# haoheliu/AudioLDM2

Hardware: AMD Instinct MI355X
Metric: audio_seconds_per_second (higher is better)
Workload: dtype f32 storage/accumulate; each product = 6 bf16 MFMA partial products of exact 3-part operand splits (fp32-grade); 1 GPU; audioldm2-full: batch 8 prompts/GPU x 1 GPU, 10.24 s @16 kHz, 200 DDIM steps, CFG 3.5, eta 1.0, n_candidates 1; one step = sample_log + VAE decode + HiFi-GAN + D2H of the waveform; synthetic conditioning, random-init weights, host-CPU RNG noise; global_batch=8, parallelism=prompt-sharded replicas x1, weight_broadcast_bytes=0

## Files before the change

audioldm2_amd/csrc/api.hip:

```cpp
#include "common.h"
#include <string.h>

namespace aldm {
static thread_local char g_err[512] = "";
void set_error(const char* fmt, ...) {
    va_list ap;
    va_start(ap, fmt);
    vsnprintf(g_err, sizeof(g_err), fmt, ap);
    va_end(ap);
}
}

extern "C" int aldm_version(void) { return 16; }
extern "C" const char* aldm_last_error(void) { return aldm::g_err; }
```

audioldm2_amd/csrc/igemm.hip:

```cpp
#include "igemm_kernel.h"
#include <algorithm>
#include <atomic>
#include <stdlib.h>

namespace aldm {

int igemm_launch_pre0(int BM, int BN, int kgroups, bool uni, bool w8, dim3 grid, hipStream_t st, const IgemmK& p);
int igemm_launch_pre1(int BM, int BN, int kgroups, bool uni, bool w8, dim3 grid, hipStream_t st, const IgemmK& p);
int igemm_launch_pre2(int BM, int BN, int kgroups, bool uni, bool w8, dim3 grid, hipStream_t st, const IgemmK& p);
int igemm_launch_pre3(int BM, int BN, int kgroups, bool uni, bool w8, dim3 grid, hipStream_t st, const IgemmK& p);
int igemm_launch_pre4(int BM, int BN, int kgroups, bool uni, bool w8, dim3 grid, hipStream_t st, const IgemmK& p);
int igemm_launch_bx_pre0(int BM, int BN, int kgroups, bool uni, bool w8, dim3 grid, hipStream_t st, const IgemmK& p);
int igemm_launch_bx_pre1(int BM, int BN, int kgroups, bool uni, bool w8, dim3 grid, hipStream_t st, const IgemmK& p);
int igemm_launch_bx_pre2(int BM, int BN, int kgroups, bool uni, bool w8, dim3 grid, hipStream_t st, const IgemmK& p);
int igemm_launch_bx_pre3(int BM, int BN, int kgroups, bool uni, bool w8, dim3 grid, hipStream_t st, const IgemmK& p);

int igemm_launch_dma(int BM, int BN, int nst, int parts, bool f16, dim3 grid, hipStream_t st, const IgemmK& p);
bool igemm_dma_config_ok(int BM, int BN, int nst, int parts);
#ifdef ALDM_TEST_HOOKS
extern std::atomic<int> g_debug_drop_product;
#endif
int igemm_launch_dma_ws(int BM, int BN, int nst, int parts, int blocks, hipStream_t st, const IgemmK& p);
bool igemm_dma_ws_config_ok(int BM, int BN, int nst, int parts);
int igemm_dma_ws_blocks_per_cu(int BM, int BN, int nst, int parts);
int igemm_launch_dma_lw(int BM, int BN, int nst, int parts, bool f16, dim3 grid, hipStream_t st, const IgemmK& p);
bool igemm_dma_lw_config_ok(int BM, int BN, int nst, int parts);
int igemm_launch_dma_os(int KT, int nst, int parts, bool f16, dim3 grid, hipStream_t st, const IgemmK& p);
bool igemm_dma_os_config_ok(int KT, int nst, int parts);
int igemm_dma_os_default_stages(int KT, int parts);
int igemm_launch_dma_halo(int BM, int BN, int nstb, int wm, int parts, bool f16, int maxch, dim3 grid, hipStream_t st, const IgemmK& p);
int igemm_dma_halo_maxch(int BM, int BN, int nstb, int wm, int parts, int nch);

__global__ __launch_bounds__(256) void igemm_reduce_kernel(const IgemmK p) {
    const aldm_igemm_desc& d = p.d;
    const int z = blockIdx.z;
    const int N4 = d.N >> 2;
    const int64_t total = (int64_t)p.M * N4;
    const int64_t i = (int64_t)blockIdx.x * 256 + threadIdx.x;
    if (i >= total) return;
    const int m = (int)(i / N4);
    const int n = (int)(i - (int64_t)m * N4) << 2;
    const int64_t slab = (int64_t)p.M * d.N;
    const float* w = d.ws + (int64_t)z * p.splits * slab + (int64_t)m * d.N + n;
    f32x4 v = *reinterpret_cast<const f32x4*>(w);
    int s = 1;
    for (; s + 3 < p.splits; s += 4) {
        const f32x4 a0 = *reinterpret_cast<const f32x4*>(w + (int64_t)s * slab);
        const f32x4 a1 = *reinterpret_cast<const f32x4*>(w + (int64_t)(s + 1) * slab);
        const f32x4 a2 = *reinterpret_cast<const f32x4*>(w + (int64_t)(s + 2) * slab);
        const f32x4 a3 = *reinterpret_cast<const f32x4*>(w + (int64_t)(s + 3) * slab);
        v += a0;
        v += a1;
        v += a2;
        v += a3;
    }
    for (; s < p.splits; ++s) v += *reinterpret_cast<const f32x4*>(w + (int64_t)s * slab);
    const int b = m / p.OHW;
    int64_t orow = m;
    if (d.out_mul > 0) {
        const int qq = m - b * p.OHW;
        const int t = qq * d.out_mul + d.out_off;
        if ((unsigned)t >= (unsigned)d.out_len) return;
        orow = (int64_t)b * d.out_len + t;
    }
    float* outp = d.out ? d.out + (int64_t)z * d.stride_o : nullptr;
    const float* resp = d.res ? d.res + (int64_t)z * d.stride_o : nullptr;
    const int64_t o = orow * d.ldo + n;
    f32x4 r;
#pragma unroll
    for (int j = 0; j < 4; ++j) r[j] = epi_value(d, p.rb_ld, outp, resp, b, o + j, n + j, v[j]);
    if (outp) {
#pragma unroll
        for (int j = 0; j < 4; ++j) outp[o + j] = r[j];
    }
    if (d.out_split) {
        if (d.out_split_act == ALDM_ACT_LRELU) {
#pragma unroll
            for (int j = 0; j < 4; ++j) r[j] = r[j] > 0.0f ? r[j] : r[j] * d.out_split_slope;
        }
        split_store4_out(d, d.out_split, orow, d.out_split_c, n, r);
    }
}

__global__ void pack_weight_kernel(const float* __restrict__ src, float* __restrict__ dst, int N,
                                   int Cin, int KH, int KW, int Kg, int Npad) {
    const int64_t total = (int64_t)Kg * Npad * 4;
    for (int64_t i = blockIdx.x * (int64_t)blockDim.x + threadIdx.x; i < total;
         i += (int64_t)gridDim.x * blockDim.x) {
        const int j = i & 3;
        const int n = (i >> 2) % Npad;
        const int kg = (i >> 2) / Npad;
        const int k = kg * 4 + j;
        float v = 0.f;
        if (n < N && k < KH * KW * Cin) {
            const int tap = k / Cin, ci = k - tap * Cin;
            const int kh = tap / KW, kw = tap - kh * KW;
            v = src[(((int64_t)n * Cin + ci) * KH + kh) * KW + kw];
        }
        dst[i] = v;
    }
}

__global__ void pack_weight_tr_kernel(const float* __restrict__ src, float* __restrict__ dst, int N,
                                      int Cin, int KWfull, int T, int phase, int stride, int Kg,
                                      int Npad) {
    const int64_t total = (int64_t)Kg * Npad * 4;
    for (int64_t i = blockIdx.x * (int64_t)blockDim.x + threadIdx.x; i < total;
         i += (int64_t)gridDim.x * blockDim.x) {
        const int jj = i & 3;
        const int n = (i >> 2) % Npad;
        const int kg = (i >> 2) / Npad;
        const int k = kg * 4 + jj;
        float v = 0.f;
        if (n < N && k < T * Cin) {
            const int kwp = k / Cin, ci = k - kwp * Cin;
            const int j = T - 1 - kwp;
            const int kk = phase + j * stride;
            if (kk < KWfull) v = src[((int64_t)ci * N + n) * KWfull + kk];
        }
        dst[i] = v;
    }
}

__global__ void pack_kn_kernel(const float* __restrict__ src, float* __restrict__ dst, int K, int N,
                               int lds, int Kg, int Npad, int64_t stride_src, int64_t stride_dst) {
    const int64_t total = (int64_t)Kg * Npad * 4;
    src += blockIdx.y * stride_src;
    dst += blockIdx.y * stride_dst;
    for (int64_t i = blockIdx.x * (int64_t)blockDim.x + threadIdx.x; i < total;
         i += (int64_t)gridDim.x * blockDim.x) {
        const int j = i & 3;
        const int n = (i >> 2) % Npad;
        const int kg = (i >> 2) / Npad;
        const int k = kg * 4 + j;
        dst[i] = (n < N && k < K) ? src[(int64_t)k * lds + n] : 0.f;
    }
}

template <int NP>
__global__ void pack_split_kernel(const float* __restrict__ src, uint4* __restrict__ dst, int Kg, int Npad,
                                  int Ko) {
    const int64_t total = (int64_t)Ko * Npad;
    for (int64_t i = blockIdx.x * (int64_t)blockDim.x + threadIdx.x; i < total;
         i += (int64_t)gridDim.x * blockDim.x) {
        const int n = (int)(i % Npad);
        const int ko = (int)(i / Npad);
        u32x2 part[2][3];
#pragma unroll
        for (int h = 0; h < 2; ++h) {
            const int kg = 2 * ko + h;
            f32x4 f = {0.f, 0.f, 0.f, 0.f};
            if (kg < Kg) f = *reinterpret_cast<const f32x4*>(src + ((int64_t)kg * Npad + n) * 4);
            split4_parts(f, part[h], NP);
        }
#pragma unroll
        for (int q = 0; q < NP; ++q) {
            uint4 o;
            o.x = part[0][q][0];
            o.y = part[0][q][1];
            o.z = part[1][q][0];
            o.w = part[1][q][1];
            dst[((int64_t)ko * NP + q) * Npad + n] = o;
        }
    }
}

__global__ void pack_split_f16_kernel(const float* __restrict__ src, uint4* __restrict__ dst, int Kg, int Npad, int Ko, float scale) {
    const int64_t total = (int64_t)Ko * Npad;
    for (int64_t i = blockIdx.x * (int64_t)blockDim.x + threadIdx.x; i < total; i += (int64_t)gridDim.x * blockDim.x) {
        const int n = (int)(i % Npad);
        const int ko = (int)(i / Npad);
        u32x2 part[2][3];
#pragma unroll
        for (int h = 0; h < 2; ++h) {
            const int kg = 2 * ko + h;
            f32x4 f = {0.f, 0.f, 0.f, 0.f};
            if (kg < Kg) f = *reinterpret_cast<const f32x4*>(src + ((int64_t)kg * Npad + n) * 4);
            split4_f16(f, scale, part[h]);
        }
#pragma unroll
        for (int q = 0; q < 2; ++q) {
            uint4 o;
            o.x = part[0][q][0];
            o.y = part[0][q][1];
            o.z = part[1][q][0];
            o.w = part[1][q][1];
            dst[((int64_t)ko * 2 + q) * Npad + n] = o;
        }
    }
}

static int log2_exact(int v) {
    int s = 0;
    while ((1 << s) < v) ++s;
    return (1 << s) == v ? s : -1;
}

}

using namespace aldm;

static thread_local int g_force_bm = 0, g_force_bn = 0, g_force_splits = 0, g_force_kgroups = 0, g_force_stages = 0;

extern "C" void aldm_igemm_force(int bm, int bn, int splits, int kgroups) {
    g_force_bm = bm;
    g_force_bn = bn;
    g_force_splits = splits;
    g_force_kgroups = kgroups;
    g_force_stages = 0;
}
extern "C" void aldm_igemm_force_stages(int stages) { g_force_stages = stages; }

static int default_wave8_mask() {
    static const int m = [] {
        const char* e = getenv("ALDM_IGEMM_W8");
        return e ? atoi(e) : 1;
    }();
    return m;
}
static thread_local int g_wave8_mask = -1;

extern "C" int aldm_igemm_wave8_mask(int mask) {
    g_wave8_mask = mask;
    return mask < 0 ? default_wave8_mask() : mask;
}

static thread_local int g_force_mma = 0;
extern "C" int aldm_igemm_mma(int mode) {
    const int prev = g_force_mma;
    if (mode >= 0 && mode <= 2) g_force_mma = mode;
    return prev;
}

static int pre_mode_of(const aldm_igemm_desc& d) {
    if (d.pre_scale == nullptr && d.pre_act == ALDM_ACT_NONE) return PRE_NONE;
    if (d.pre_scale != nullptr && d.pre_act == ALDM_ACT_NONE) return PRE_AFFINE;
    if (d.pre_scale != nullptr && d.pre_act == ALDM_ACT_SILU) return PRE_AFFINE_SILU;
    if (d.pre_scale == nullptr && d.pre_act == ALDM_ACT_LRELU) return PRE_LRELU;
    return PRE_GENERIC;
}

static int device_cus() {
    static const int n = [] {
        int dev = 0, cus = 0;
        if (hipGetDevice(&dev) != hipSuccess ||
            hipDeviceGetAttribute(&cus, hipDeviceAttributeMultiprocessorCount, dev) != hipSuccess || cus <= 0)
            return 256;
        return cus;
    }();
    return n;
}

static bool dma_ws_eligible(const IgemmK& p, int BM, int BN) {
    const aldm_igemm_desc& d = p.d;
    const bool geglu = d.epi_mode == ALDM_EPI_GEGLU;
    auto al16 = [](const void* q) { return (reinterpret_cast<uintptr_t>(q) & 15) == 0; };
    if (d.out_mul > 0 || d.accumulate || d.batch != 1 || d.act != ALDM_ACT_NONE || d.out_split_act != ALDM_ACT_NONE ||
        d.epi_mode == ALDM_EPI_QKV)
        return false;
    if (p.M % BM != 0 || d.N % BN != 0 || (d.N & 3) != 0 || (d.ldo & 3) != 0) return false;
    if (!al16(d.out) || !al16(d.res) || !al16(d.bias) || !al16(d.rowbias) || !al16(d.out_split)) return false;
    if (d.rowbias && (p.OHW % BM != 0 || (p.rb_ld & 3) != 0)) return false;
    if (geglu && (BN != 128 || d.res || d.rowbias)) return false;
    return true;
}

static bool dma_os_eligible(const IgemmK& p) {
    const aldm_igemm_desc& d = p.d;
    if (d.KH != 1 || d.KW != 1 || d.SH != 1 || d.SW != 1 || d.PH != 0 || d.PW != 0 || d.up_h != 1 || d.up_w != 1) return false;
    if (d.OH != d.H || d.OW != d.W || d.K != p.Cin || d.K % 32 != 0 || d.out_mul > 0 || d.batch > 1) return false;
    if (d.epi_mode == ALDM_EPI_QKV && d.qkv_c % 128 != 0) return false;
    if (d.rowbias || d.accumulate || d.act != ALDM_ACT_NONE) return false;
    auto al16 = [](const void* q) { return (reinterpret_cast<uintptr_t>(q) & 15) == 0; };
    if ((d.N & 3) != 0 || (d.ldo & 3) != 0 || !al16(d.out) || !al16(d.res)) return false;
    return true;
}

static int dma_halo_chunks(const IgemmK& p, int BM) {
    const aldm_igemm_desc& d = p.d;
    if (d.KH != 3 || d.KW != 3 || d.SH != 1 || d.SW != 1 || d.PH != 1 || d.PW != 1 || d.DH != 1 || d.DW != 1) return 0;
    if (d.up_h != 1 || d.up_w != 1 || d.OH != d.H || d.OW != d.W || d.out_mul > 0 || d.batch > 1) return 0;
    if (d.W <= 0 || (d.W & (d.W - 1)) != 0 || BM % d.W != 0 || p.OHW % BM != 0) return 0;
    return ((BM / d.W + 2) * d.W + 15) / 16;
}

static bool tile_supported(int BM, int BN) {
    return (BM == 128 && (BN == 128 || BN == 64 || BN == 32)) || (BM == 64 && (BN == 128 || BN == 64));
}

static int igemm_prepare(const aldm_igemm_desc* dd, IgemmK& p, int& BM, int& BN) {
    ALDM_CHECK(dd != nullptr, "aldm_igemm: null descriptor");
    p.d = *dd;
    aldm_igemm_desc& d = p.d;
    ALDM_CHECK((d.x1 || d.a_split) && d.w && (d.out || d.out_split), "aldm_igemm: null x1/w/out");
    if (!d.x1) d.x1 = reinterpret_cast<const float*>(d.a_split);
    if (d.split_parts == 0) d.split_parts = 3;
    ALDM_CHECK(d.split_parts == 2 || d.split_parts == 3, "aldm_igemm: split_parts must be 0 / 3 or 2");
    if (d.out_split_parts == 0) d.out_split_parts = d.split_parts;
    ALDM_CHECK(d.out_split_parts == 2 || d.out_split_parts == 3, "aldm_igemm: out_split_parts must be 0, 2 or 3");
    ALDM_CHECK(d.a_fmt == ALDM_FMT_BF16 || (d.a_fmt == ALDM_FMT_F16 && d.a_split != nullptr && d.split_parts == 2 && d.acc_scale > 0.0f),
               "aldm_igemm: a_fmt = ALDM_FMT_F16 needs a pre-split operand (a_split), 2-part images and acc_scale > 0");
    if (d.a_fmt == ALDM_FMT_BF16) d.acc_scale = 1.0f;
    ALDM_CHECK(d.out_split_fmt == ALDM_FMT_BF16 ||
                   (d.out_split_fmt == ALDM_FMT_F16 && d.out_split_scale > 0.0f &&
                    (d.epi_mode == ALDM_EPI_QKV ? (d.k_split != nullptr && d.vt_split != nullptr && d.vt_scale > 0.0f) : d.out_split != nullptr)),
               "aldm_igemm: out_split_fmt = ALDM_FMT_F16 needs out_split (QKV: k_split, vt_split and vt_scale) and out_split_scale > 0");
    if (d.out_split_fmt == ALDM_FMT_F16) d.out_split_parts = 2;
    if (!d.x2) d.C2 = 0;
    if (d.pix1 == 0) d.pix1 = d.C1;
    if (d.pix2 == 0) d.pix2 = d.C2;
    if (d.up_h == 0) d.up_h = 1;
    if (d.up_w == 0) d.up_w = 1;
    if (d.batch == 0) d.batch = 1;
    p.Cin = d.C1 + d.C2;
    ALDM_CHECK(d.C1 > 0 && d.C1 % 4 == 0 && d.C2 % 4 == 0,
               "aldm_igemm: C1=%d/C2=%d must be multiples of 4", d.C1, d.C2);
    ALDM_CHECK(d.pix1 % 4 == 0 && d.pix2 % 4 == 0, "aldm_igemm: pixel pitch must be a multiple of 4");
    ALDM_CHECK(d.K == d.KH * d.KW * p.Cin, "aldm_igemm: K=%d != KH*KW*Cin=%d", d.K,
               d.KH * d.KW * p.Cin);
    ALDM_CHECK(d.N > 0 && (d.ldo >= d.N || d.epi_mode == ALDM_EPI_GEGLU || d.epi_mode == ALDM_EPI_QKV),
               "aldm_igemm: bad N=%d ldo=%d", d.N, d.ldo);
    ALDM_CHECK(d.B > 0 && d.H > 0 && d.W > 0 && d.OH > 0 && d.OW > 0, "aldm_igemm: bad extents");
    ALDM_CHECK(d.SH > 0 && d.SW > 0 && d.DH > 0 && d.DW > 0, "aldm_igemm: bad stride/dilation");
    p.shh = log2_exact(d.up_h);
    p.shw = log2_exact(d.up_w);
    ALDM_CHECK(p.shh >= 0 && p.shw >= 0, "aldm_igemm: upsample factors must be powers of two");
    ALDM_CHECK((reinterpret_cast<uintptr_t>(d.x1) & 15) == 0 &&
                   (reinterpret_cast<uintptr_t>(d.w) & 15) == 0 &&
                   (d.x2 == nullptr || (reinterpret_cast<uintptr_t>(d.x2) & 15) == 0),
               "aldm_igemm: operands must be 16-byte aligned");
    if (d.b_mode == ALDM_B_NT) {
        ALDM_CHECK(d.ldb % 4 == 0 && d.ldb >= d.K, "aldm_igemm: NT ldb=%d invalid", d.ldb);
        p.Npad = d.N;
    } else {
        p.Npad = (d.N + 31) / 32 * 32;
        ALDM_CHECK(d.ldb == 0 || d.ldb == p.Npad, "aldm_igemm: packed ldb must equal Npad");
    }
    if (d.out_mul > 0) ALDM_CHECK(d.OH == 1, "aldm_igemm: row remap requires OH == 1");
    ALDM_CHECK((d.pre_scale == nullptr) == (d.pre_shift == nullptr),
               "aldm_igemm: pre_scale/pre_shift must come together");
    ALDM_CHECK(d.pre_scale == nullptr ||
                   ((reinterpret_cast<uintptr_t>(d.pre_scale) | reinterpret_cast<uintptr_t>(d.pre_shift)) & 15) == 0,
               "aldm_igemm: pre_scale/pre_shift must be 16-byte aligned");
    const bool geglu = d.epi_mode == ALDM_EPI_GEGLU;
    const bool qkv = d.epi_mode == ALDM_EPI_QKV;
    ALDM_CHECK(d.epi_mode == ALDM_EPI_PLAIN || geglu || qkv, "aldm_igemm: unknown epi_mode %d", d.epi_mode);
    if (qkv) {
        auto al16 = [](const void* q) { return (reinterpret_cast<uintptr_t>(q) & 15) == 0; };
        ALDM_CHECK(d.a_split && d.qkv_c > 0 && d.qkv_c % 64 == 0 && d.N == 3 * d.qkv_c && d.qkv_rows > 0 && d.qkv_rows % 32 == 0 &&
                       (((int64_t)d.B * d.OH * d.OW) % d.qkv_rows == 0 ||
                        d.qkv_rows == (((int64_t)d.B * d.OH * d.OW + 31) & ~(int64_t)31)) && d.out && d.k_split && d.vt_split && al16(d.out) &&
                       al16(d.k_split) && al16(d.vt_split) && d.ldo >= d.qkv_c && (d.ldo & 3) == 0 && !d.bias && !d.rowbias &&
                       !d.res && !d.out_split && !d.accumulate && d.out_mul == 0 && d.act == ALDM_ACT_NONE && d.alpha == 1.0f &&
                       d.batch <= 1,
                   "aldm_igemm: ALDM_EPI_QKV needs a pre-split operand, N = 3*qkv_c (qkv_c %% 64 == 0), qkv_rows %% 32 == 0 dividing M "
                   "(or M rounded up to 32), "
                   "aligned out / k_split / vt_split and a plain epilogue");
    }
    if (geglu) {
        ALDM_CHECK(d.N % 64 == 0 && d.ldo >= d.N / 2 && d.ldo % 4 == 0 && d.b_mode == ALDM_B_PACKED &&
                       d.out_mul == 0 && !d.res && !d.rowbias && !d.accumulate &&
                       (d.act == ALDM_ACT_NONE || d.act == ALDM_ACT_GELU_TANH) &&
                       (reinterpret_cast<uintptr_t>(d.out) & 15) == 0 && d.stride_o % 4 == 0 &&
                       (d.bias == nullptr || (reinterpret_cast<uintptr_t>(d.bias) & 15) == 0),
                   "aldm_igemm: GEGLU epilogue needs N %% 64 == 0, ldo >= N/2, packed weights, a plain epilogue");
    }
    p.OHW = d.OH * d.OW;
    const int64_t M64 = (int64_t)d.B * p.OHW;
    ALDM_CHECK(M64 < (1ll << 31) - 256, "aldm_igemm: M too large");
    p.M = (int)M64;
    p.HV = d.H * d.up_h;
    p.WV = d.W * d.up_w;
    ALDM_CHECK((int64_t)d.B * d.H * d.W < (1ll << 31), "aldm_igemm: input has too many pixels");
    p.Kg = (d.K + 3) / 4;
    p.rb_ld = d.rowbias_ld > 0 ? d.rowbias_ld : d.N;

    const int nk = (d.K + BK - 1) / BK;
    const int64_t Mz = p.M;
    const int pre = pre_mode_of(d);
    p.dma = 0;
    p.nst = 0;
    p.ws = 0;
    p.ws_blocks = 0;
    p.os_rows = 0;
    ALDM_CHECK(d.out_split_act == ALDM_ACT_NONE || (d.out_split_act == ALDM_ACT_LRELU && d.out_split != nullptr &&
                                                   d.epi_mode == ALDM_EPI_PLAIN),
               "aldm_igemm: out_split_act must be ALDM_ACT_NONE or ALDM_ACT_LRELU with a split-image output of the plain epilogue");
    if (d.out_split) {
        ALDM_CHECK(d.out_split_c > 0 && d.out_split_c % 32 == 0 && d.out_split_c >= (geglu ? d.N / 2 : d.N) &&
                       d.N % 4 == 0 && d.batch == 1 && (reinterpret_cast<uintptr_t>(d.out_split) & 15) == 0 &&
                       ((reinterpret_cast<uintptr_t>(d.out) | reinterpret_cast<uintptr_t>(d.res)) & 15) == 0 &&
                       (d.out == nullptr || (d.ldo & 3) == 0),
                   "aldm_igemm: out_split needs out_split_c %% 32 == 0 and >= N, N %% 4 == 0, batch 1, aligned out/res");
        ALDM_CHECK(d.out != nullptr || !d.accumulate, "aldm_igemm: accumulate needs an fp32 output");
    }
    if (d.a_split) {
        ALDM_CHECK(d.w_split != nullptr && d.b_mode == ALDM_B_PACKED && d.stride_w == 0 && d.batch == 1,
                   "aldm_igemm: a_split needs packed, split weights and batch 1");
        ALDM_CHECK(d.C2 == 0 && d.C1 % 32 == 0 && pre == PRE_NONE,
                   "aldm_igemm: a_split needs one source with C1 %% 32 == 0 and no prologue (C1=%d C2=%d)", d.C1, d.C2);
        ALDM_CHECK(((reinterpret_cast<uintptr_t>(d.a_split) | reinterpret_cast<uintptr_t>(d.w_split)) & 15) == 0,
                   "aldm_igemm: split images must be 16-byte aligned");
        ALDM_CHECK((int64_t)d.B * d.H * d.W * p.Cin * 2 * d.split_parts < (1ll << 40), "aldm_igemm: split image too large");
        const bool can_split = d.N % 4 == 0 && nk >= 8 && !geglu && !qkv;
        const bool have_ws = d.ws != nullptr && (reinterpret_cast<uintptr_t>(d.ws) & 15) == 0;
        auto dma_cost = [&](int bm, int bn, int nst, int sp, int* sp_eff) -> double {
            const int kt = cdiv(nk, sp);
            sp = cdiv(nk, kt);
            *sp_eff = sp;
            const double blocks = (double)cdiv64(Mz, bm) * cdiv(d.N, bn) * sp;
            const int lds = nst * (bm + bn) * 64 * d.split_parts;
            const int o = std::min(2, (160 * 1024) / lds);
            const double tile_c = (bm / 64) * (bn / 64) * 64.0 * (d.split_parts == 3 ? 6 : 3);
            const double dma_c = (bm + bn) * 64.0 * d.split_parts / 56.0;
            const double L = kt * std::max(tile_c, dma_c);
            const double one = kt * std::max(tile_c + 200.0, dma_c) + 6000.0;
            const int64_t nb = (int64_t)((blocks + 255.0) / 256.0);
            const int64_t full = nb / o, last = nb - full * o;
            double T = full * std::max(one, o * L);
            if (last) T += std::max(one, last * L);
            if (sp > 1) T += 10000.0 + (double)(sp + 1) * Mz * d.N * 4.0 / 2000.0;
            return T;
        };
        int splits = 1, nst = 0;
        const bool hint_fits = d.hint_bm > 0 && (!qkv || (d.hint_bn > 0 && d.qkv_c % d.hint_bn == 0)) && (!geglu || d.hint_bn == 128);
        const int f_bm = g_force_bm ? g_force_bm : (hint_fits ? d.hint_bm : 0), f_bn = g_force_bm ? g_force_bn : d.hint_bn;
        const int f_sp = g_force_bm ? g_force_splits : d.hint_splits;
        int f_st = g_force_bm ? g_force_stages : (hint_fits ? d.hint_stages : 0);
        int ws_nst = 0;
        int lw_nst = 0;
        if (f_st >= 300 && f_st < 400) {
            const int KT = d.K / 32;
            int os_nst = f_st - 300;
            if (os_nst == 0) os_nst = igemm_dma_os_default_stages(KT, d.split_parts);
            if (dma_os_eligible(p) && igemm_dma_os_config_ok(KT, os_nst, d.split_parts)) {
                static const int env_rows = [] {
                    const char* e = getenv("ALDM_OS_ROWS");
                    return e ? atoi(e) : 0;
                }();
                const int tn = cdiv(d.N, 128);
                const int stages = cdiv(p.M, 32);
                const int chunks = std::max(1, device_cus() / tn);
                int rows = cdiv(stages, chunks) * 32;
                if (env_rows > 0) rows = cdiv(env_rows, 32) * 32;
                BM = 32;
                BN = 128;
// ... 97 lines not shown
        p.tiles_n = cdiv(d.N, BN);
        p.kt_per_split = cdiv(nk, splits);
        splits = cdiv(nk, p.kt_per_split);
        if (splits > 1 && (!have_ws || d.ws_floats < (int64_t)splits * p.M * d.N)) {
            splits = 1;
            p.kt_per_split = nk;
        }
        p.splits = splits;
        p.kgroups = 1;
        p.bx = 1;
        p.pre = pre;
        p.dma = 1;
        p.nst = nst;
        p.ws = 0;
        p.ws_blocks = 0;
        if (lw_nst > 0) {
            ALDM_CHECK(igemm_dma_lw_config_ok(BM, BN, lw_nst, d.split_parts), "aldm_igemm: no loader-wave DMA kernel for tile %dx%d, %d stages", BM, BN, lw_nst);
            p.ws = 2;
            p.nst = lw_nst;
        }
        if (ws_nst > 0) {
            if (splits == 1 && d.a_fmt == ALDM_FMT_BF16 && d.out_split_parts == d.split_parts && d.out_split_fmt == ALDM_FMT_BF16 &&
                igemm_dma_ws_config_ok(BM, BN, ws_nst, d.split_parts) && dma_ws_eligible(p, BM, BN)) {
                const int ntiles = p.tiles_m * p.tiles_n;
                const int per = cdiv(ntiles, device_cus() * igemm_dma_ws_blocks_per_cu(BM, BN, ws_nst, d.split_parts));
                p.ws = 1;
                p.nst = ws_nst;
                p.ws_blocks = cdiv(ntiles, per);
            } else {
                ALDM_CHECK(!g_force_bm, "aldm_igemm: the persistent DMA kernel cannot run this launch (tile %dx%d, %d stages)", BM,
                           BN, ws_nst);
            }
        }
        return 0;
    }
    const bool bx_ok = d.w_split != nullptr && d.split_parts == 3 && d.b_mode == ALDM_B_PACKED && d.stride_w == 0 && d.batch == 1 &&
                       pre != PRE_GENERIC && (reinterpret_cast<uintptr_t>(d.w_split) & 15) == 0 &&
                       (g_force_mma == 2 || (g_force_mma == 0 && d.hint_mma != 1));
    auto occ_of = [&](int bm, int bn) {
        if (bx_ok && bn != 32) return bm * bn >= 128 * 128 ? 1 : (bm * bn >= 64 * 128 ? 2 : 3);
        return bm * bn >= 128 * 128 ? 2 : ((bm * bn >= 64 * 128 || bn == 32) ? 3 : 4);
    };
    const double pre_w = (d.pre_scale != nullptr || d.pre_act != ALDM_ACT_NONE) ? 1.5 : 1.0;
    auto cost_of = [&](int bm, int bn, int sp, int kg, int* sp_eff) -> double {
        const bool bx = bx_ok && bn != 32;
        const double mf = bx ? 0.375 : 1.0;
        const int kt = cdiv(nk, sp);
        sp = cdiv(nk, kt);
        *sp_eff = sp;
        const double blocks = (double)cdiv64(Mz, bm) * cdiv(d.N, bn) * d.batch * sp;
        const double L = (double)kt * bm * bn / 4.0 * mf;
        const int o = kg == 2 ? (bx ? 1 : 2) : occ_of(bm, bn);
        const double S = (300.0 * (bm / 32) * pre_w + 200.0 * (bn / 32)) *
                         (bx ? (bm * bn >= 128 * 128 && !geglu ? 0.45 : 1.3) : 1.0);
        const double F = 4000.0 + (kg == 2 ? 600.0 : 0.0);
        const int64_t nb = (int64_t)((blocks + 255.0) / 256.0);
        const int64_t full = nb / o, last = nb - full * o;
        const double one = (double)cdiv(kt, kg) * ((double)bm * bn / 4.0 * mf + S) + F;
        double T = full * std::max(one, o * L);
        if (last) T += std::max(one, last * L);
        if (sp > 1) T += 10000.0 + (double)(sp + 1) * Mz * d.N * d.batch * 4.0 / 2000.0;
        return T;
    };
    const bool can_split = d.N % 4 == 0 && nk >= 8 && !geglu;
    const bool have_ws = d.ws != nullptr && (reinterpret_cast<uintptr_t>(d.ws) & 15) == 0;
    int splits = 1, kgroups = 1;
    const int f_bm = g_force_bm ? g_force_bm : d.hint_bm, f_bn = g_force_bm ? g_force_bn : d.hint_bn;
    const int f_sp = g_force_bm ? g_force_splits : d.hint_splits;
    const int f_kg = g_force_bm ? g_force_kgroups : d.hint_kgroups;
    if (f_bm) {
        BM = f_bm;
        BN = f_bn;
        ALDM_CHECK(tile_supported(BM, BN), "aldm_igemm: unsupported forced/hinted tile %dx%d", BM, BN);
        ALDM_CHECK(!geglu || BN == 128, "aldm_igemm: the GEGLU epilogue needs a 128-column tile");
        if (f_sp > 0 && can_split && nk / f_sp >= 1) splits = f_sp;
        if (f_kg == 2) {
            ALDM_CHECK(BM == 64 && BN == 64, "aldm_igemm: two wave groups exist for the 64x64 tile only");
            kgroups = 2;
        }
    } else if (d.N <= 32 && !geglu) {
        BM = 128;
        BN = 32;
    } else {
        static const int cand[4][2] = {{128, 128}, {64, 128}, {128, 64}, {64, 64}};
        static const int sps[8] = {1, 2, 3, 4, 6, 8, 12, 16};
        double best = 1e300;
        BM = 64;
        BN = 64;
        for (int c = 0; c < 4; ++c) {
            const int bm = cand[c][0], bn = cand[c][1];
            if (geglu ? bn != 128 : (bn > 64 && d.N <= 64)) continue;
            for (int si = 0; si < 8; ++si) {
                const int sp = sps[si];
                if (sp > 1 && (!can_split || !have_ws || nk / sp < 3)) break;
                for (int kg = 1; kg <= ((bm == 64 && bn == 64) ? 2 : 1); ++kg) {
                    int spe;
                    const double t = cost_of(bm, bn, sp, kg, &spe);
                    if (spe > 1 && (int64_t)d.batch * spe * Mz * d.N > d.ws_floats) continue;
                    if (kg == 2 && cdiv(nk, spe) < 4) continue;
                    if (t < best) {
                        best = t;
                        BM = bm;
                        BN = bn;
                        splits = spe;
                        kgroups = kg;
                    }
                }
            }
        }
    }
    ALDM_CHECK(!geglu || BN == 128, "aldm_igemm: internal: GEGLU epilogue without a 128-column tile");
    p.tiles_m = cdiv(p.M, BM);
    p.tiles_n = cdiv(d.N, BN);
    if (splits < 1) splits = 1;
    p.kt_per_split = cdiv(nk, splits);
    splits = cdiv(nk, p.kt_per_split);
    if (splits > 1) {
        const int64_t need = (int64_t)d.batch * splits * p.M * d.N;
        if (!have_ws || d.ws_floats < need) {
            splits = 1;
            p.kt_per_split = nk;
        }
    }
    p.splits = splits;
    p.kgroups = kgroups;
    p.bx = bx_ok && BN != 32 ? 1 : 0;
    p.pre = pre;
    return 0;
}

extern "C" int aldm_igemm_plan(const aldm_igemm_desc* dd, int* bm, int* bn, int64_t* flops, int* splits,
                               int* kgroups, int* mma) {
    IgemmK p;
    int BM, BN;
    const int rc = igemm_prepare(dd, p, BM, BN);
    if (rc) return rc;
    if (bm) *bm = BM;
    if (bn) *bn = BN;
    if (flops) *flops = 2ll * p.M * p.d.N * p.d.K * p.d.batch;
    if (splits) *splits = p.splits;
    if (kgroups) *kgroups = p.kgroups;
    if (mma) *mma = p.bx ? ALDM_MMA_BF16X6 : ALDM_MMA_F32;
    return 0;
}

extern "C" int aldm_igemm_plan_stages(const aldm_igemm_desc* dd) {
    IgemmK p;
    int BM, BN;
    if (igemm_prepare(dd, p, BM, BN)) return -1;
    if (p.dma && p.ws == 4) return 400 + (BM == 128 && p.ws_blocks == 4 ? 10 : 0) + p.nst;
    return p.dma ? p.nst + 100 * p.ws : 0;
}

extern "C" int64_t aldm_igemm_ws_floats(const aldm_igemm_desc* dd) {
    if (!dd) return 0;
    aldm_igemm_desc t = *dd;
    t.ws = reinterpret_cast<float*>(uintptr_t(16));
    t.ws_floats = INT64_MAX;
    IgemmK p;
    int BM, BN;
    if (igemm_prepare(&t, p, BM, BN)) return 0;
    return p.splits > 1 ? (int64_t)p.d.batch * p.splits * p.M * p.d.N : 0;
}

extern "C" int aldm_igemm(const aldm_igemm_desc* dd, void* stream) {
    IgemmK p;
    int BM, BN;
    int rc = igemm_prepare(dd, p, BM, BN);
    if (rc) return rc;
    const aldm_igemm_desc& d = p.d;
    dim3 grid((unsigned)(p.tiles_m * p.tiles_n), (unsigned)p.splits, (unsigned)d.batch);
    hipStream_t st = (hipStream_t)stream;
    const int pre = p.pre;
    const bool uni = p.OHW % BM == 0;
    const int env_w8 = g_wave8_mask < 0 ? default_wave8_mask() : g_wave8_mask;
    const bool gn_pre = pre == PRE_AFFINE || pre == PRE_AFFINE_SILU;
    const int tile_bit = (BM == 128 && BN == 128) ? 1 : (BM == 64 && BN == 128) ? 2 : (BM == 128 && BN == 64) ? 4 : 0;
    const bool w8 = p.kgroups == 1 && d.epi_mode != ALDM_EPI_GEGLU && (env_w8 & tile_bit) != 0 &&
                    (p.bx ? tile_bit == 1 : (gn_pre || (tile_bit == 1 && (env_w8 & 8) != 0)));
#ifdef ALDM_TEST_HOOKS
    if (g_debug_drop_product.load(std::memory_order_relaxed))
        ALDM_CHECK(p.dma && p.ws == 0 && BM == 64 && BN == 128 && p.nst == 2 && d.split_parts == 3,
                   "aldm_igemm: aldm_debug_drop_product is set: force the classic DMA-fed 64x128 tile with 2 stages and 3-part images "
                   "(got dma=%d form=%d tile %dx%d, %d stages, %d parts) or clear the switch", p.dma, p.ws, BM, BN, p.nst, d.split_parts);
#endif
    if (p.dma && p.ws == 4) {
        rc = igemm_launch_dma_halo(BM, BN, p.nst, p.ws_blocks, d.split_parts, d.a_fmt == ALDM_FMT_F16, p.os_rows, grid, st, p);
    } else if (p.dma && p.ws == 3) {
        rc = igemm_launch_dma_os(d.K / 32, p.nst, d.split_parts, d.a_fmt == ALDM_FMT_F16, grid, st, p);
    } else if (p.dma && p.ws == 2) {
        rc = igemm_launch_dma_lw(BM, BN, p.nst, d.split_parts, d.a_fmt == ALDM_FMT_F16, grid, st, p);
    } else if (p.dma && p.ws) {
        rc = igemm_launch_dma_ws(BM, BN, p.nst, d.split_parts, p.ws_blocks, st, p);
    } else if (p.dma) {
        rc = igemm_launch_dma(BM, BN, p.nst, d.split_parts, d.a_fmt == ALDM_FMT_F16, grid, st, p);
    } else if (p.bx) {
        switch (pre) {
            case PRE_NONE: rc = igemm_launch_bx_pre0(BM, BN, p.kgroups, uni, w8, grid, st, p); break;
            case PRE_AFFINE: rc = igemm_launch_bx_pre1(BM, BN, p.kgroups, uni, w8, grid, st, p); break;
            case PRE_AFFINE_SILU: rc = igemm_launch_bx_pre2(BM, BN, p.kgroups, uni, w8, grid, st, p); break;
            default: rc = igemm_launch_bx_pre3(BM, BN, p.kgroups, uni, w8, grid, st, p); break;
        }
    } else
    switch (pre) {
        case PRE_NONE: rc = igemm_launch_pre0(BM, BN, p.kgroups, uni, w8, grid, st, p); break;
        case PRE_AFFINE: rc = igemm_launch_pre1(BM, BN, p.kgroups, uni, w8, grid, st, p); break;
        case PRE_AFFINE_SILU: rc = igemm_launch_pre2(BM, BN, p.kgroups, uni, w8, grid, st, p); break;
        case PRE_LRELU: rc = igemm_launch_pre3(BM, BN, p.kgroups, uni, w8, grid, st, p); break;
        default: rc = igemm_launch_pre4(BM, BN, p.kgroups, uni, w8, grid, st, p); break;
    }
    if (rc) {
        set_error("aldm_igemm: no kernel for tile %dx%d", BM, BN);
        return -1;
    }
    if (p.splits > 1) {
        const int64_t total = (int64_t)p.M * (d.N >> 2);
        hipLaunchKernelGGL(igemm_reduce_kernel, dim3((unsigned)cdiv64(total, 256), 1, (unsigned)d.batch),
                           dim3(256), 0, st, p);
    }
    ALDM_LAUNCH_CHECK("aldm_igemm");
    return 0;
}

extern "C" int64_t aldm_split_bytes_parts(int K, int N, int parts) {
    if (K <= 0 || N <= 0 || (parts != 2 && parts != 3)) return 0;
    const int Npad = (N + 31) / 32 * 32;
    const int64_t Ko = 4ll * ((K + 31) / 32);
    return Ko * parts * Npad * 16;
}
extern "C" int64_t aldm_split_bytes(int K, int N) { return aldm_split_bytes_parts(K, N, 3); }

extern "C" int aldm_pack_split_f16(const float* packed, void* dst, int K, int N, float scale, void* stream) {
    ALDM_CHECK(packed && dst && K > 0 && N > 0 && scale > 0.0f, "aldm_pack_split_f16: bad args");
    ALDM_CHECK(((reinterpret_cast<uintptr_t>(packed) | reinterpret_cast<uintptr_t>(dst)) & 15) == 0,
               "aldm_pack_split_f16: operands must be 16-byte aligned");
    const int Npad = (N + 31) / 32 * 32;
    const int Kg = (K + 3) / 4;
    const int Ko = 4 * ((K + 31) / 32);
    const int64_t total = (int64_t)Ko * Npad;
    hipLaunchKernelGGL(pack_split_f16_kernel, dim3((unsigned)std::min<int64_t>(cdiv64(total, 256), 4096)), dim3(256), 0,
                       (hipStream_t)stream, packed, reinterpret_cast<uint4*>(dst), Kg, Npad, Ko, scale);
    ALDM_LAUNCH_CHECK("aldm_pack_split_f16");
    return 0;
}

extern "C" int aldm_pack_split_bf16_parts(const float* packed, void* dst, int K, int N, int parts, void* stream) {
    ALDM_CHECK(packed && dst && K > 0 && N > 0 && (parts == 2 || parts == 3), "aldm_pack_split_bf16: bad args");
    ALDM_CHECK(((reinterpret_cast<uintptr_t>(packed) | reinterpret_cast<uintptr_t>(dst)) & 15) == 0,
               "aldm_pack_split_bf16: operands must be 16-byte aligned");
    const int Npad = (N + 31) / 32 * 32;
    const int Kg = (K + 3) / 4;
    const int Ko = 4 * ((K + 31) / 32);
    const int64_t total = (int64_t)Ko * Npad;
    const int blocks = (int)std::min<int64_t>((total + 255) / 256, 65535);
    if (parts == 3)
        hipLaunchKernelGGL(pack_split_kernel<3>, dim3(blocks), dim3(256), 0, (hipStream_t)stream, packed,
                           reinterpret_cast<uint4*>(dst), Kg, Npad, Ko);
    else
        hipLaunchKernelGGL(pack_split_kernel<2>, dim3(blocks), dim3(256), 0, (hipStream_t)stream, packed,
                           reinterpret_cast<uint4*>(dst), Kg, Npad, Ko);
    ALDM_LAUNCH_CHECK("aldm_pack_split_bf16");
    return 0;
}
extern "C" int aldm_pack_split_bf16(const float* packed, void* dst, int K, int N, void* stream) {
    return aldm_pack_split_bf16_parts(packed, dst, K, N, 3, stream);
}

extern "C" int aldm_pack_weight(const float* src, float* dst, int N, int Cin, int KH, int KW,
                                int transposed, int phase, int stride, void* stream) {
    ALDM_CHECK(src && dst && N > 0 && Cin > 0 && KH > 0 && KW > 0, "aldm_pack_weight: bad args");
    const int Npad = (N + 31) / 32 * 32;
    hipStream_t st = (hipStream_t)stream;
    if (!transposed) {
        const int K = KH * KW * Cin;
        const int Kg = (K + 3) / 4;
        const int64_t total = (int64_t)Kg * Npad * 4;
        const int blocks = (int)std::min<int64_t>(cdiv64(total, 256), 4096);
        hipLaunchKernelGGL(pack_weight_kernel, dim3(blocks), dim3(256), 0, st, src, dst, N, Cin, KH,
                           KW, Kg, Npad);
    } else {
        ALDM_CHECK(KH == 1 && stride > 0 && phase >= 0 && phase < stride,
                   "aldm_pack_weight: bad transposed args");
        const int T = (KW + stride - 1) / stride;
        const int K = T * Cin;
        const int Kg = (K + 3) / 4;
        const int64_t total = (int64_t)Kg * Npad * 4;
        const int blocks = (int)std::min<int64_t>(cdiv64(total, 256), 4096);
        hipLaunchKernelGGL(pack_weight_tr_kernel, dim3(blocks), dim3(256), 0, st, src, dst, N, Cin,
                           KW, T, phase, stride, Kg, Npad);
    }
    ALDM_LAUNCH_CHECK("aldm_pack_weight");
    return 0;
}

extern "C" int aldm_pack_kn(const float* src, float* dst, int K, int N, int lds, int batch,
                            int64_t stride_src, int64_t stride_dst, void* stream) {
    ALDM_CHECK(src && dst && K > 0 && N > 0 && lds >= N && batch > 0, "aldm_pack_kn: bad args");
    const int Npad = (N + 31) / 32 * 32;
    const int Kg = (K + 3) / 4;
    const int64_t total = (int64_t)Kg * Npad * 4;
    const int blocks = (int)std::min<int64_t>(cdiv64(total, 256), 4096);
    hipLaunchKernelGGL(pack_kn_kernel, dim3(blocks, batch), dim3(256), 0, (hipStream_t)stream, src,
                       dst, K, N, lds, Kg, Npad, stride_src, stride_dst);
    ALDM_LAUNCH_CHECK("aldm_pack_kn");
    return 0;
}
```

audioldm2_amd/csrc/igemm_dma.h:

```cpp
#pragma once
#include "igemm_epilogue.h"
#include <type_traits>

namespace aldm {

static __device__ __attribute__((aligned(256))) unsigned g_dma_zero_page[256 + 64];

constexpr int dma_stage_slots(int BM, int BN, int NP) { return (BM + BN) * 4 * NP; }
constexpr int dma_lds_bytes(int BM, int BN, int NST, int NP) { return NST * dma_stage_slots(BM, BN, NP) * 16; }
constexpr int dma_blocks_per_cu(int BM, int BN, int NST, int NP) {
    return (160 * 1024) / dma_lds_bytes(BM, BN, NST, NP) >= 2 ? 2 : 1;
}

template <bool F16>
__device__ __forceinline__ f32x16 mfma_32x32x16(const bf16x8 a, const bf16x8 b, const f32x16 c) {
    if constexpr (F16)
        return __builtin_amdgcn_mfma_f32_32x32x16_f16(__builtin_bit_cast(f16x8, a), __builtin_bit_cast(f16x8, b), c, 0, 0, 0);
    else
        return __builtin_amdgcn_mfma_f32_32x32x16_bf16(a, b, c, 0, 0, 0);
}
template <bool F16, int MT, int NT>
__device__ __forceinline__ void unscale_acc(f32x16 (&acc)[MT][NT], float acc_scale) {
    if constexpr (F16) {
#pragma unroll
        for (int i = 0; i < MT; ++i)
#pragma unroll
            for (int j = 0; j < NT; ++j)
#pragma unroll
                for (int e = 0; e < 16; ++e) acc[i][j][e] *= acc_scale;
    }
}

template <int N>
__device__ __forceinline__ void wait_vmcnt() {
    __builtin_amdgcn_s_waitcnt((N & 15) | (7 << 4) | (0 << 8) | ((N >> 4) << 14));
}

#ifndef ALDM_DMA_TAP_INNER
#define ALDM_DMA_TAP_INNER 0
#endif
#ifndef ALDM_DMA_ABLATE
#define ALDM_DMA_ABLATE 0
#endif

template <int BM, int BN, int NST, int WM = 2, int NP = 3, bool DROP = false, bool F16 = false>
__global__ __launch_bounds__(128 * WM, dma_blocks_per_cu(BM, BN, NST, NP) * (WM / 2))
void igemm_dma_kernel(const IgemmK p) {
    constexpr int WN = 2, NW = WM * WN;
    constexpr int MT = BM / (32 * WM), NT = BN / 64;
    constexpr int STG = dma_stage_slots(BM, BN, NP);
    constexpr int PB = 64 * NP;
    constexpr int RA = BM / (16 * NW);
    constexpr int NB = 4 * NP * (BN / 64) / NW;
    constexpr int D = NP * RA + NB;
    constexpr int NPROD = NP == 3 ? 6 : 3;
    static_assert(NP == 2 || NP == 3, "2 or 3 parts");
    static_assert(!F16 || NP == 2, "fp16 images have two parts");
    static_assert(BM % (16 * NW) == 0 && (4 * NP * (BN / 64)) % NW == 0, "DMA chunks must divide among the waves");
    static_assert(NST >= 2 && NST <= 8 && (NST - 1) * D <= 63, "ring depth / vmcnt range");
    static_assert(NW * 32 * (NT * 32 + 4) * 4 <= NST * STG * 16, "epilogue staging must fit the ring");
    __shared__ u32x4 smem[NST * STG];

    const aldm_igemm_desc& d = p.d;
    const int lane = threadIdx.x & 63;
    const int wave = __builtin_amdgcn_readfirstlane(threadIdx.x >> 6);
    const int wm = wave / WN, wn = wave % WN;
    const int l31 = lane & 31, lh = lane >> 5;

    int tile_m, tile_n;
    {
        const int nwg = gridDim.x;
        const int bid = blockIdx.x;
        const int q = nwg >> 3, r = nwg & 7;
        const int xcd = bid & 7, idx = bid >> 3;
        const int logical = (xcd < r ? xcd * (q + 1) : r * (q + 1) + (xcd - r) * q) + idx;
        tile_n = logical % p.tiles_n;
        tile_m = logical / p.tiles_n;
    }
    const int m0 = tile_m * BM, n0 = tile_n * BN;
    const int split = blockIdx.y;
    const int nk_all = d.K >> 5;
    const int kt0 = split * p.kt_per_split;
    const int kt1 = min(nk_all, kt0 + p.kt_per_split);
#if ALDM_DMA_ABLATE & 32
    const int nk = min(kt1 - kt0, 1);
#else
    const int nk = kt1 - kt0;
#endif

    const char* zero = reinterpret_cast<const char*>(g_dma_zero_page);
    const char* abase = reinterpret_cast<const char*>(d.a_split);
    const char* wbase = reinterpret_cast<const char*>(d.w_split);
    const int cpb = p.Cin >> 5;
    const int taps = d.KH * d.KW;
    const int64_t rowbytes = (int64_t)cpb * PB;

    const int lane_off = ((lane & 3) ^ ((lane >> 4) & 3)) * 16;
    int a_pix[RA], a_h[RA], a_w[RA];
#pragma unroll
    for (int i = 0; i < RA; ++i) {
        const int m = m0 + (wave * RA + i) * 16 + (lane >> 2);
        if (m < p.M) {
            const int b = m / p.OHW;
            const int rem = m - b * p.OHW;
            const int oh = rem / d.OW;
            const int ow = rem - oh * d.OW;
            a_pix[i] = b * d.H;
            a_h[i] = oh * d.SH - d.PH;
            a_w[i] = ow * d.SW - d.PW;
        } else {
            a_pix[i] = 0;
            a_h[i] = -(1 << 28);
            a_w[i] = 0;
        }
    }
    const char* a_ptr[RA];
    int a_step[RA];
    int t_kh, t_kw, t_cb;
    auto set_tap = [&]() {
        const int dh = t_kh * d.DH, dw = t_kw * d.DW;
        const int cboff = t_cb * PB + lane_off;
#pragma unroll
        for (int i = 0; i < RA; ++i) {
            const int ihv = a_h[i] + dh, iwv = a_w[i] + dw;
            const bool ok = (unsigned)ihv < (unsigned)p.HV && (unsigned)iwv < (unsigned)p.WV;
            const int pix = (a_pix[i] + (ihv >> p.shh)) * d.W + (iwv >> p.shw);
            a_ptr[i] = ok ? abase + ((int64_t)pix * rowbytes + cboff) : zero + lane_off;
            a_step[i] = ok ? PB : 0;
        }
    };
    {
        if (ALDM_DMA_TAP_INNER) {
            t_cb = kt0 / taps;
            const int tap = kt0 - t_cb * taps;
            t_kh = tap / d.KW;
            t_kw = tap - t_kh * d.KW;
        } else {
            const int tap = kt0 / cpb;
            t_cb = kt0 - tap * cpb;
            t_kh = tap / d.KW;
            t_kw = tap - t_kh * d.KW;
        }
        set_tap();
    }
    const char* b_ptr[NB];
    int64_t b_tile[NB];
#pragma unroll
    for (int j = 0; j < NB; ++j) {
        const int c = wave * NB + j;
        const int srow = c / (BN / 64), half = c % (BN / 64);
        const int col = n0 + half * 64 + lane;
        const bool ok = col < p.Npad;
        b_tile[j] = ok ? (int64_t)4 * NP * p.Npad * 16 : 0;
        const int tile0 = (t_kh * d.KW + t_kw) * cpb + t_cb;
        b_ptr[j] = ok ? wbase + (((int64_t)tile0 * 4 * NP + srow) * p.Npad + col) * 16 : zero;
    }

    using gptr_t = const __attribute__((address_space(1))) void*;
    using lptr_t = __attribute__((address_space(3))) void*;
    auto issue_dma = [&](int st) {
        u32x4* sa = &smem[st * STG];
#pragma unroll
        for (int i = 0; i < RA; ++i)
#pragma unroll
            for (int q = 0; q < NP; ++q) {
                const char* src = (ALDM_DMA_ABLATE & 1) ? zero + lane * 16 : a_ptr[i] + q * 64;
                __builtin_amdgcn_global_load_lds((gptr_t)src, (lptr_t)(sa + ((wave * RA + i) * NP + q) * 64), 16, 0, 0);
            }
#pragma unroll
        for (int j = 0; j < NB; ++j) {
            const int c = wave * NB + j;
            const int srow = c / (BN / 64), half = c % (BN / 64);
            const char* src = (ALDM_DMA_ABLATE & 2) ? zero + lane * 16 : b_ptr[j];
            __builtin_amdgcn_global_load_lds((gptr_t)src, (lptr_t)(sa + BM * 4 * NP + srow * BN + half * 64), 16, 0, 0);
        }
    };
    auto advance = [&]() {
        if (taps == 1 || !ALDM_DMA_TAP_INNER) {
#pragma unroll
            for (int i = 0; i < RA; ++i) a_ptr[i] += a_step[i];
#pragma unroll
            for (int j = 0; j < NB; ++j) b_ptr[j] += b_tile[j];
            if (++t_cb == cpb && taps > 1) {
                t_cb = 0;
                if (++t_kw == d.KW) {
                    t_kw = 0;
                    ++t_kh;
                }
                set_tap();
            }
            return;
        }
        if (++t_kw == d.KW) {
            t_kw = 0;
            ++t_kh;
        }
        if (t_kh == d.KH) {
            t_kh = 0;
            ++t_cb;
#pragma unroll
            for (int j = 0; j < NB; ++j) b_ptr[j] += b_tile[j] * (1 - (int64_t)(taps - 1) * cpb);
        } else {
#pragma unroll
            for (int j = 0; j < NB; ++j) b_ptr[j] += b_tile[j] * cpb;
        }
        set_tap();
    };
    auto issue = [&](int st) {
        issue_dma(st);
        advance();
    };

    struct Frag {
        bf16x8 a[MT][NP], b[NT][NP];
    };
    const int a_sw = (l31 >> 2) & 3;
    auto read_frags = [&](Frag& f, int st, int step) {
#if ALDM_DMA_ABLATE & 8
        return;
#endif
        const u32x4* sa = &smem[st * STG];
        const int o = 2 * step + lh;
#pragma unroll
        for (int i = 0; i < MT; ++i) {
            const int row = (wm * MT + i) * 32 + l31;
#pragma unroll
            for (int q = 0; q < NP; ++q)
                f.a[i][q] = __builtin_bit_cast(bf16x8, sa[((row >> 4) * NP + q) * 64 + (row & 15) * 4 + (o ^ a_sw)]);
        }
#pragma unroll
        for (int j = 0; j < NT; ++j)
#pragma unroll
            for (int q = 0; q < NP; ++q)
                f.b[j][q] = __builtin_bit_cast(bf16x8, sa[BM * 4 * NP + (o * NP + q) * BN + (wn * NT + j) * 32 + l31]);
    };

    f32x16 acc[MT][NT], sum[MT][NT];
    acc_zero(acc);
    acc_zero(sum);
    auto mma_frags = [&](const Frag& f) {
        constexpr int PA_[6] = {NP == 3 ? 0 : 1, NP == 3 ? 2 : 0, NP == 3 ? 1 : 0, 0, 1, 0};
        constexpr int PB_[6] = {NP == 3 ? 2 : 0, NP == 3 ? 0 : 1, NP == 3 ? 1 : 0, 1, 0, 0};
#if ALDM_DMA_ABLATE & 4
#pragma unroll
        for (int i = 0; i < MT; ++i)
#pragma unroll
            for (int q = 0; q < NP; ++q) asm volatile("" ::"v"(f.a[i][q]));
#pragma unroll
        for (int j = 0; j < NT; ++j)
#pragma unroll
            for (int q = 0; q < NP; ++q) asm volatile("" ::"v"(f.b[j][q]));
        return;
#endif
#pragma unroll
        for (int q = DROP ? 1 : 0; q < NPROD; ++q)
#pragma unroll
            for (int i = 0; i < MT; ++i)
#pragma unroll
                for (int j = 0; j < NT; ++j)
                    acc[i][j] = mfma_32x32x16<F16>(f.a[i][PA_[q]], f.b[j][PB_[q]], acc[i][j]);
    };
    auto wait_tiles = [&](int n) {
        constexpr int MX = NST - 1;
        if (n <= 0) wait_vmcnt<0>();
        else if (n == 1) wait_vmcnt<D>();
        else if (n == 2) wait_vmcnt<(MX >= 2 ? 2 : MX) * D>();
        else if (n == 3) wait_vmcnt<(MX >= 3 ? 3 : MX) * D>();
        else if (n == 4) wait_vmcnt<(MX >= 4 ? 4 : MX) * D>();
        else if (n == 5) wait_vmcnt<(MX >= 5 ? 5 : MX) * D>();
        else wait_vmcnt<(MX >= 6 ? 6 : MX) * D>();
    };

#pragma unroll
    for (int s = 0; s < NST; ++s)
        if (s < nk) issue(s);
    wait_tiles(min(nk, NST) - 1);
    __builtin_amdgcn_s_barrier();
    Frag f0, f1;
#if ALDM_DMA_ABLATE & 8
    for (int q = 0; q < NP; ++q) {
        for (int i = 0; i < MT; ++i) f0.a[i][q] = f1.a[i][q] = __builtin_bit_cast(bf16x8, smem[lane + q]);
        for (int j = 0; j < NT; ++j) f0.b[j][q] = f1.b[j][q] = __builtin_bit_cast(bf16x8, smem[lane + 64 + q]);
    }
#endif
    read_frags(f0, 0, 0);
    int st = 0, t = 0;
    auto body = [&](auto steady) {
        constexpr bool ST = decltype(steady)::value;
        constexpr int NMF = NPROD * MT * NT, NRD = NP * (MT + NT);
        read_frags(f1, st, 1);
        mma_frags(f0);
#pragma unroll
        for (int q = 0; q < NMF; ++q) {
            __builtin_amdgcn_sched_group_barrier(0x008, 1, 0);
            if (q < NRD) __builtin_amdgcn_sched_group_barrier(0x100, 1, 0);
        }
        __builtin_amdgcn_sched_barrier(0);
        const int st1 = st + 1 == NST ? 0 : st + 1;
        if constexpr (ST) wait_vmcnt<(NST - 2) * D>();
        else wait_tiles(min(NST - 2, nk - 2 - t));
        __builtin_amdgcn_s_barrier();
        if constexpr (ST) issue_dma(st);
        read_frags(f0, st1, 0);
        mma_frags(f1);
#pragma unroll
        for (int q = 0; q < NMF; ++q) {
            __builtin_amdgcn_sched_group_barrier(0x008, 1, 1);
            if (ST && q == 0) __builtin_amdgcn_sched_group_barrier(0x020, D, 1);
            if (q < NRD) __builtin_amdgcn_sched_group_barrier(0x100, 1, 1);
        }
        __builtin_amdgcn_sched_barrier(0);
        if constexpr (ST) advance();
        st = st1;
    };
    while (t + NST < nk) {
        for (const int te = min(nk - NST, t + ACC_BLOCK_TILES); t < te; ++t) body(std::true_type{});
        if (t + NST < nk) acc_close_block(acc, sum);
    }
    for (; t + 1 < nk; ++t) body(std::false_type{});
    read_frags(f1, st, 1);
    mma_frags(f0);
    mma_frags(f1);
    acc_total(acc, sum);

    __syncthreads();
#if ALDM_DMA_ABLATE & 16
    if (p.M == -12345) {
#pragma unroll
        for (int i = 0; i < MT; ++i)
#pragma unroll
            for (int j = 0; j < NT; ++j)
#pragma unroll
                for (int e = 0; e < 16; ++e) d.ws[(i * NT + j) * 16 + e + threadIdx.x * 256] = acc[i][j][e];
    }
    return;
#endif
    unscale_acc<F16>(acc, d.acc_scale);
    igemm_epilogue<MT, NT>(p, acc, reinterpret_cast<float*>(&smem[0]), m0, n0, wave, wm, wn, lane, 0, split);
}

}
```

audioldm2_amd/csrc/igemm_dma.hip:

```cpp
#include "igemm_dma.h"
#include <atomic>

namespace aldm {

bool igemm_dma_config_ok(int BM, int BN, int nst, int parts) {
    if (BM == 256 && BN == 128) return parts == 3 ? nst == 2 : (nst == 2 || nst == 3);
    if (BM == 128 && BN == 128) return parts == 3 ? (nst == 2 || nst == 3) : (nst == 2 || nst == 4);
    if ((BM == 64 && BN == 128) || (BM == 128 && BN == 64)) return nst == 2 || nst == 4 || (nst == 6 && parts == 2);
    if (BM == 64 && BN == 64) return nst == 2 || nst == 3 || (nst == 6 && parts == 2);
    return false;
}

#ifdef ALDM_TEST_HOOKS
std::atomic<int> g_debug_drop_product{0};
#endif

int igemm_launch_dma(int BM, int BN, int nst, int parts, bool f16, dim3 grid, hipStream_t st, const IgemmK& p) {
#ifdef ALDM_TEST_HOOKS
    if (g_debug_drop_product.load(std::memory_order_relaxed)) {
        if (!(BM == 64 && BN == 128 && nst == 2 && parts == 3)) return -1;
        hipLaunchKernelGGL((igemm_dma_kernel<64, 128, 2, 2, 3, true>), grid, dim3(256), 0, st, p);
        return 0;
    }
#endif
#define ALDM_DMA(BM_, BN_, NST_, NP_) \
    hipLaunchKernelGGL((igemm_dma_kernel<BM_, BN_, NST_, 2, NP_>), grid, dim3(256), 0, st, p)
#define ALDM_DMA8(BM_, BN_, NST_, NP_) \
    hipLaunchKernelGGL((igemm_dma_kernel<BM_, BN_, NST_, 4, NP_>), grid, dim3(512), 0, st, p)
    if (f16) {
        if (parts != 2) return -1;
#define ALDM_DMA_H(BM_, BN_, NST_) \
    hipLaunchKernelGGL((igemm_dma_kernel<BM_, BN_, NST_, 2, 2, false, true>), grid, dim3(256), 0, st, p)
#define ALDM_DMA8_H(BM_, BN_, NST_) \
    hipLaunchKernelGGL((igemm_dma_kernel<BM_, BN_, NST_, 4, 2, false, true>), grid, dim3(512), 0, st, p)
        if (BM == 256 && BN == 128 && nst == 3) ALDM_DMA8_H(256, 128, 3);
        else if (BM == 256 && BN == 128 && nst == 2) ALDM_DMA8_H(256, 128, 2);
        else if (BM == 128 && BN == 128 && nst == 4) ALDM_DMA_H(128, 128, 4);
        else if (BM == 128 && BN == 128 && nst == 2) ALDM_DMA_H(128, 128, 2);
        else if (BM == 64 && BN == 128 && nst == 6) ALDM_DMA_H(64, 128, 6);
        else if (BM == 64 && BN == 128 && nst == 4) ALDM_DMA_H(64, 128, 4);
        else if (BM == 64 && BN == 128 && nst == 2) ALDM_DMA_H(64, 128, 2);
        else if (BM == 128 && BN == 64 && nst == 6) ALDM_DMA_H(128, 64, 6);
        else if (BM == 128 && BN == 64 && nst == 4) ALDM_DMA_H(128, 64, 4);
        else if (BM == 128 && BN == 64 && nst == 2) ALDM_DMA_H(128, 64, 2);
        else if (BM == 64 && BN == 64 && nst == 6) ALDM_DMA_H(64, 64, 6);
        else if (BM == 64 && BN == 64 && nst == 3) ALDM_DMA_H(64, 64, 3);
        else if (BM == 64 && BN == 64 && nst == 2) ALDM_DMA_H(64, 64, 2);
        else return -1;
#undef ALDM_DMA_H
#undef ALDM_DMA8_H
        return 0;
    }
    if (parts == 3) {
        if (BM == 256 && BN == 128 && nst == 2) ALDM_DMA8(256, 128, 2, 3);
        else if (BM == 128 && BN == 128 && nst == 3) ALDM_DMA(128, 128, 3, 3);
        else if (BM == 128 && BN == 128 && nst == 2) ALDM_DMA(128, 128, 2, 3);
        else if (BM == 64 && BN == 128 && nst == 4) ALDM_DMA(64, 128, 4, 3);
        else if (BM == 64 && BN == 128 && nst == 2) ALDM_DMA(64, 128, 2, 3);
        else if (BM == 128 && BN == 64 && nst == 4) ALDM_DMA(128, 64, 4, 3);
        else if (BM == 128 && BN == 64 && nst == 2) ALDM_DMA(128, 64, 2, 3);
        else if (BM == 64 && BN == 64 && nst == 3) ALDM_DMA(64, 64, 3, 3);
        else if (BM == 64 && BN == 64 && nst == 2) ALDM_DMA(64, 64, 2, 3);
        else return -1;
    } else {
        if (BM == 256 && BN == 128 && nst == 3) ALDM_DMA8(256, 128, 3, 2);
        else if (BM == 256 && BN == 128 && nst == 2) ALDM_DMA8(256, 128, 2, 2);
        else if (BM == 128 && BN == 128 && nst == 4) ALDM_DMA(128, 128, 4, 2);
        else if (BM == 128 && BN == 128 && nst == 2) ALDM_DMA(128, 128, 2, 2);
        else if (BM == 64 && BN == 128 && nst == 6) ALDM_DMA(64, 128, 6, 2);
        else if (BM == 64 && BN == 128 && nst == 4) ALDM_DMA(64, 128, 4, 2);
        else if (BM == 64 && BN == 128 && nst == 2) ALDM_DMA(64, 128, 2, 2);
        else if (BM == 128 && BN == 64 && nst == 6) ALDM_DMA(128, 64, 6, 2);
        else if (BM == 128 && BN == 64 && nst == 4) ALDM_DMA(128, 64, 4, 2);
        else if (BM == 128 && BN == 64 && nst == 2) ALDM_DMA(128, 64, 2, 2);
        else if (BM == 64 && BN == 64 && nst == 6) ALDM_DMA(64, 64, 6, 2);
        else if (BM == 64 && BN == 64 && nst == 3) ALDM_DMA(64, 64, 3, 2);
        else if (BM == 64 && BN == 64 && nst == 2) ALDM_DMA(64, 64, 2, 2);
        else return -1;
    }
#undef ALDM_DMA
#undef ALDM_DMA8
    return 0;
}

template <int ACT, bool AFF>
__global__ __launch_bounds__(256) void split_rows_kernel(const float* __restrict__ x1, const float* __restrict__ x2,
                                                         int C1, int C2, int64_t rows, int P,
                                                         const float* __restrict__ scale,
                                                         const float* __restrict__ shift, char* __restrict__ dst,
                                                         char* __restrict__ dst_raw, int parts, float slope, int raw_parts,
                                                         float f16_scale) {
    const int C = C1 + C2;
    const int C8 = C >> 3;
    const int64_t total = rows * C8;
    for (int64_t i = blockIdx.x * (int64_t)blockDim.x + threadIdx.x; i < total; i += (int64_t)gridDim.x * blockDim.x) {
        const int64_t row = i / C8;
        const int c = (int)(i - row * C8) << 3;
        const float* src = c < C1 ? x1 + row * C1 + c : x2 + row * C2 + (c - C1);
        f32x4 v0 = *reinterpret_cast<const f32x4*>(src);
        f32x4 v1 = *reinterpret_cast<const f32x4*>(src + 4);
        const int64_t off = (row * (C >> 5) + (c >> 5)) * (64 * parts) + (c & 31) * 2;
        u32x2 p0[3], p1[3];
        if (dst_raw) {
            const int64_t roff = (row * (C >> 5) + (c >> 5)) * (64 * raw_parts) + (c & 31) * 2;
            split4_parts(v0, p0, raw_parts);
            split4_parts(v1, p1, raw_parts);
#pragma unroll
            for (int q = 0; q < 3; ++q)
                if (q < raw_parts) *reinterpret_cast<u32x4*>(dst_raw + roff + q * 64) = u32x4{p0[q][0], p0[q][1], p1[q][0], p1[q][1]};
        }
        if constexpr (AFF) {
            const int64_t so = (row / P) * C + c;
            const f32x4 s0 = *reinterpret_cast<const f32x4*>(scale + so), s1 = *reinterpret_cast<const f32x4*>(scale + so + 4);
            const f32x4 h0 = *reinterpret_cast<const f32x4*>(shift + so), h1 = *reinterpret_cast<const f32x4*>(shift + so + 4);
#pragma unroll
            for (int e = 0; e < 4; ++e) {
                v0[e] = __builtin_fmaf(v0[e], s0[e], h0[e]);
                v1[e] = __builtin_fmaf(v1[e], s1[e], h1[e]);
            }
        }
        if constexpr (ACT == ALDM_ACT_SILU) {
#pragma unroll
            for (int e = 0; e < 4; ++e) {
                v0[e] = silu_fast(v0[e]);
                v1[e] = silu_fast(v1[e]);
            }
        }
        if constexpr (ACT == ALDM_ACT_LRELU) {
#pragma unroll
            for (int e = 0; e < 4; ++e) {
                v0[e] = v0[e] > 0.0f ? v0[e] : v0[e] * slope;
                v1[e] = v1[e] > 0.0f ? v1[e] : v1[e] * slope;
            }
        }
        split4_fmt(v0, p0, parts, f16_scale);
        split4_fmt(v1, p1, parts, f16_scale);
#pragma unroll
        for (int q = 0; q < 3; ++q)
            if (q < parts) *reinterpret_cast<u32x4*>(dst + off + q * 64) = u32x4{p0[q][0], p0[q][1], p1[q][0], p1[q][1]};
    }
}

}

using namespace aldm;

#ifdef ALDM_TEST_HOOKS
extern "C" int aldm_debug_drop_product(int on) { return aldm::g_debug_drop_product.exchange(on ? 1 : 0); }
#endif

extern "C" int64_t aldm_split_image_bytes(int64_t rows, int C, int parts) { return rows * (int64_t)(C / 32) * 64 * parts; }

extern "C" int aldm_split_rows_act(const float* x1, const float* x2, int C1, int C2, int64_t rows, int P, const float* scale,
                                   const float* shift, int act, float slope, void* dst, void* dst_raw, int parts, void* stream);
extern "C" int aldm_split_rows_f16(const float* x1, const float* x2, int C1, int C2, int64_t rows, int P, const float* scale,
                                   const float* shift, int act, float slope, void* dst, void* dst_raw, int raw_parts, float f16_scale,
                                   void* stream);

extern "C" int aldm_split_rows(const float* x1, const float* x2, int C1, int C2, int64_t rows, int P, const float* scale,
                               const float* shift, int act, void* dst, void* dst_raw, int parts, void* stream) {
    ALDM_CHECK(act == ALDM_ACT_NONE || act == ALDM_ACT_SILU, "aldm_split_rows: activation %d not supported", act);
    return aldm_split_rows_act(x1, x2, C1, C2, rows, P, scale, shift, act, 0.f, dst, dst_raw, parts, stream);
}

static int split_rows_launch(const float* x1, const float* x2, int C1, int C2, int64_t rows, int P, const float* scale,
                             const float* shift, int act, float slope, void* dst, void* dst_raw, int parts, int raw_parts,
                             float f16_scale, void* stream);

extern "C" int aldm_split_rows_act(const float* x1, const float* x2, int C1, int C2, int64_t rows, int P, const float* scale,
                                   const float* shift, int act, float slope, void* dst, void* dst_raw, int parts, void* stream) {
    return split_rows_launch(x1, x2, C1, C2, rows, P, scale, shift, act, slope, dst, dst_raw, parts, parts, 0.f, stream);
}

extern "C" int aldm_split_rows_f16(const float* x1, const float* x2, int C1, int C2, int64_t rows, int P, const float* scale,
                                   const float* shift, int act, float slope, void* dst, void* dst_raw, int raw_parts, float f16_scale,
                                   void* stream) {
    ALDM_CHECK(f16_scale > 0.0f && (raw_parts == 2 || raw_parts == 3), "aldm_split_rows_f16: need f16_scale > 0 and raw_parts 2 | 3");
// ... 38 lines not shown
```

audioldm2_amd/csrc/igemm_dma_halo.h:

```cpp
#pragma once
#include "igemm_dma.h"

#ifndef ALDM_HALO_ABLATE
#define ALDM_HALO_ABLATE 0
#endif

namespace aldm {

constexpr int halo_lds_slots(int BN, int NSTB, int NP, int MAXCH) {
    return 2 * MAXCH * NP * 64 + NSTB * BN * 4 * NP + NP * 64;
}

template <int BM, int BN, int NSTB, int WM, int NP, int MAXCH, bool F16 = false>
__global__ __launch_bounds__(128 * WM, WM / 2)
void igemm_dma_halo_kernel(const IgemmK p) {
    constexpr int WN = 2, NW = WM * WN;
    constexpr int MT = BM / (32 * WM), NT = BN / 64;
    constexpr int PB = 64 * NP;
    constexpr int PATCH = MAXCH * NP * 64;
    constexpr int BSTG = BN * 4 * NP;
    constexpr int B0 = 2 * PATCH;
    constexpr int Z0 = B0 + NSTB * BSTG;
    constexpr int NB = 4 * NP * (BN / 64) / NW;
    constexpr int D = NB + 1;
    constexpr int ATILES = 11 - NSTB;
    constexpr int NPROD = NP == 3 ? 6 : 3;
    static_assert(NP == 2 || NP == 3, "2 or 3 parts");
    static_assert((4 * NP * (BN / 64)) % NW == 0, "weight pieces must divide among the waves");
    static_assert(NSTB >= 2 && NSTB <= 6 && (NSTB - 1) * D <= 63, "ring depth / vmcnt range");
    static_assert(NW * 32 * (NT * 32 + 4) * 4 <= Z0 * 16, "epilogue staging must fit");
    static_assert((Z0 + NP * 64) * 16 <= 160 * 1024, "LDS budget");
    __shared__ __attribute__((aligned(1024))) u32x4 smem[Z0 + NP * 64];

    const aldm_igemm_desc& d = p.d;
    const int lane = threadIdx.x & 63;
    const int wave = __builtin_amdgcn_readfirstlane(threadIdx.x >> 6);
    const int wm = wave / WN, wn = wave % WN;
    const int l31 = lane & 31, lh = lane >> 5;

    int tile_m, tile_n;
    {
        const int nwg = gridDim.x;
        const int bid = blockIdx.x;
        const int q = nwg >> 3, r = nwg & 7;
        const int xcd = bid & 7, idx = bid >> 3;
        const int logical = (xcd < r ? xcd * (q + 1) : r * (q + 1) + (xcd - r) * q) + idx;
        tile_n = logical % p.tiles_n;
        tile_m = logical / p.tiles_n;
    }
    const int m0 = tile_m * BM, n0 = tile_n * BN;
    const int split = blockIdx.y;
    const int cpb = p.Cin >> 5;
    const int cbps = p.kt_per_split / 9;
    const int cb0 = split * cbps;
    const int ncb = min(cpb, cb0 + cbps) - cb0;
    const int nk = ncb * 9;

    const int W = d.W, lgW = __builtin_ctz((unsigned)W);
    const int img = m0 / p.OHW;
    const int r0 = (m0 - img * p.OHW) >> lgW;
    const int PP = ((BM >> lgW) + 2) << lgW;
    const int NCH = (PP + 15) >> 4;

    const char* zero = reinterpret_cast<const char*>(g_dma_zero_page);
    const char* abase = reinterpret_cast<const char*>(d.a_split);
    const char* wbase = reinterpret_cast<const char*>(d.w_split);
    const int64_t rowbytes = (int64_t)cpb * PB;
    const int lane_off = ((lane & 3) ^ ((lane >> 4) & 3)) * 16;

    using gptr_t = const __attribute__((address_space(1))) void*;
    using lptr_t = __attribute__((address_space(3))) void*;

    const int64_t patch_pix0 = (int64_t)(img * d.H + r0 - 1) * W;
    const char* patch_base0 = abase + (patch_pix0 * rowbytes + (int64_t)cb0 * PB);
    const unsigned rowbytes32 = (unsigned)rowbytes;
    struct Piece {
        const char* src;
        int dst;
    };
    auto prep_patch_piece = [&](int id, int ci, bool live) -> Piece {
        const int j = id / NP, q = id - j * NP;
        const bool valid = live & (j < NCH);
        const int px = j * 16 + (lane >> 2);
        const int irow = r0 - 1 + (px >> lgW);
        const bool ok = valid & (px < PP) & ((unsigned)irow < (unsigned)d.H);
        const unsigned off = (unsigned)px * rowbytes32 + (unsigned)(q * 64 + lane_off);
        const char* real = patch_base0 + (int64_t)((ALDM_HALO_ABLATE & 128) ? 0 : ci) * PB + off;
        const char* zsrc = zero + lane_off;
        Piece pc;
        pc.src = ok ? real : zsrc;
        const int dreal = (ci & 1) * PATCH + (j * NP + q) * 64;
        pc.dst = valid ? dreal : Z0;
        return pc;
    };
    auto issue_piece = [&](const Piece& pc) {
        __builtin_amdgcn_global_load_lds((gptr_t)pc.src, (lptr_t)&smem[pc.dst], 16, 0, 0);
    };
    int av_s = 0, av_c = 1;
    auto prep_a = [&]() {
        return prep_patch_piece(av_s * NW + wave, av_c, (ALDM_HALO_ABLATE & 1) ? false : (av_s < ATILES) & (av_c < ncb));
    };
    auto advance_a = [&]() {
        const bool wrap = av_s == 8;
        av_s = wrap ? 0 : av_s + 1;
        av_c += wrap ? 1 : 0;
    };

    unsigned b_off[NB];
#pragma unroll
    for (int j = 0; j < NB; ++j) {
        const int c = wave * NB + j;
        const int srow = c / (BN / 64), half = c % (BN / 64);
        const int col = min(n0 + half * 64 + lane, p.Npad - 1);
        b_off[j] = (unsigned)((srow * p.Npad + col) * 16);
    }
    const int64_t b_tile = (int64_t)4 * NP * p.Npad * 16;
    const char* b_base = wbase + (int64_t)cb0 * b_tile;
    int bt_tap = 0;
    auto issue_b = [&](int st) {
        u32x4* sb = &smem[B0 + st * BSTG];
#pragma unroll
        for (int j = 0; j < NB; ++j) {
            const int c = wave * NB + j;
            const int srow = c / (BN / 64), half = c % (BN / 64);
            const char* src = (ALDM_HALO_ABLATE & 2) ? zero + lane * 16 : b_base + b_off[j];
            __builtin_amdgcn_global_load_lds((gptr_t)src, (lptr_t)(sb + srow * BN + half * 64), 16, 0, 0);
        }
    };
    auto advance_b = [&]() {
        const bool wrap = bt_tap == 8;
        bt_tap = wrap ? 0 : bt_tap + 1;
        if (!(ALDM_HALO_ABLATE & 64)) b_base += b_tile * (wrap ? 1 - 8 * cpb : cpb);
    };

    struct Frag {
        bf16x8 a[MT][NP], b[NT][NP];
    };
    int pt[MT];
#pragma unroll
    for (int i = 0; i < MT; ++i) pt[i] = (wm * MT + i) * 32 + l31;
    unsigned aaddr[MT];
    unsigned aaddr_n[MT];
    int c_kh = 0, c_kw = 0, c_buf = 0;
    auto set_aaddr_n = [&]() {
        const int toff = c_kh * W + c_kw - 1;
#pragma unroll
        for (int i = 0; i < MT; ++i) {
            const int pp = pt[i] + toff;
            const int cc = (pt[i] & (W - 1)) + c_kw - 1;
            const unsigned off = (unsigned)(pp >> 4) * (NP * 1024) + (unsigned)(pp & 15) * 64 + (unsigned)((((pp >> 2) & 3) ^ lh) << 4);
            const unsigned real = (unsigned)(c_buf * PATCH * 16) + off;
            const unsigned zslot = (unsigned)(Z0 * 16) + (off & 0xF0u);
            aaddr_n[i] = (unsigned)cc < (unsigned)W ? real : zslot;
        }
    };
    auto next_tap = [&]() {
        const bool w1 = c_kw == 2;
        c_kw = w1 ? 0 : c_kw + 1;
        const bool w2 = w1 && c_kh == 2;
        c_kh = w2 ? 0 : (w1 ? c_kh + 1 : c_kh);
        c_buf ^= w2 ? 1 : 0;
        if (!(ALDM_HALO_ABLATE & 32)) set_aaddr_n();
    };
    auto take_aaddr = [&]() {
#pragma unroll
        for (int i = 0; i < MT; ++i) aaddr[i] = aaddr_n[i];
    };
    const char* lds = reinterpret_cast<const char*>(smem);
    auto read_frags = [&](Frag& f, int st, int step) {
#if ALDM_DMA_ABLATE & 8
        return;
#endif
        const int o = 2 * step + lh;
#pragma unroll
        for (int i = 0; i < MT; ++i) {
            const u32x4* pa = reinterpret_cast<const u32x4*>(lds + (aaddr[i] ^ (unsigned)(step << 5)));
#pragma unroll
            for (int q = 0; q < NP; ++q) f.a[i][q] = __builtin_bit_cast(bf16x8, pa[q * 64]);
        }
        const u32x4* sb = &smem[B0 + st * BSTG];
#pragma unroll
        for (int j = 0; j < NT; ++j)
#pragma unroll
            for (int q = 0; q < NP; ++q)
                f.b[j][q] = __builtin_bit_cast(bf16x8, sb[(o * NP + q) * BN + (wn * NT + j) * 32 + l31]);
    };

    f32x16 acc[MT][NT], sum[MT][NT];
    acc_zero(acc);
    acc_zero(sum);
    auto mma_frags = [&](const Frag& f) {
        constexpr int PA_[6] = {NP == 3 ? 0 : 1, NP == 3 ? 2 : 0, NP == 3 ? 1 : 0, 0, 1, 0};
        constexpr int PB_[6] = {NP == 3 ? 2 : 0, NP == 3 ? 0 : 1, NP == 3 ? 1 : 0, 1, 0, 0};
#if ALDM_DMA_ABLATE & 4
#pragma unroll
        for (int i = 0; i < MT; ++i)
#pragma unroll
            for (int q = 0; q < NP; ++q) asm volatile("" ::"v"(f.a[i][q]));
#pragma unroll
        for (int j = 0; j < NT; ++j)
#pragma unroll
            for (int q = 0; q < NP; ++q) asm volatile("" ::"v"(f.b[j][q]));
        return;
#endif
#pragma unroll
        for (int q = 0; q < NPROD; ++q)
#pragma unroll
            for (int i = 0; i < MT; ++i)
#pragma unroll
                for (int j = 0; j < NT; ++j)
                    acc[i][j] = mfma_32x32x16<F16>(f.a[i][PA_[q]], f.b[j][PB_[q]], acc[i][j]);
    };
    auto wait_tiles = [&](int n) {
        constexpr int MX = NSTB - 1;
        if (n <= 0) wait_vmcnt<0>();
        else if (n == 1) wait_vmcnt<D>();
        else if (n == 2) wait_vmcnt<(MX >= 2 ? 2 : MX) * D>();
        else if (n == 3) wait_vmcnt<(MX >= 3 ? 3 : MX) * D>();
        else wait_vmcnt<(MX >= 4 ? 4 : MX) * D>();
    };

    if (wave < NP)
        __builtin_amdgcn_global_load_lds((gptr_t)(zero + lane * 16), (lptr_t)&smem[Z0 + wave * 64], 16, 0, 0);
    for (int id = wave; id < NCH * NP; id += NW) issue_piece(prep_patch_piece(id, 0, true));
    issue_piece(prep_a());
    advance_a();
#pragma unroll
    for (int s = 0; s < NSTB; ++s)
        if (s < nk) {
            issue_b(s);
            advance_b();
        }
    wait_vmcnt<0>();
    __builtin_amdgcn_s_barrier();
    set_aaddr_n();
    take_aaddr();
    Frag f0, f1;
#if ALDM_DMA_ABLATE & 8
    for (int q = 0; q < NP; ++q) {
        for (int i = 0; i < MT; ++i) f0.a[i][q] = f1.a[i][q] = __builtin_bit_cast(bf16x8, smem[lane + q]);
        for (int j = 0; j < NT; ++j) f0.b[j][q] = f1.b[j][q] = __builtin_bit_cast(bf16x8, smem[lane + 64 + q]);
    }
#endif
    read_frags(f0, 0, 0);
    int st = 0, t = 0;
    auto body = [&](auto steady) {
        constexpr bool ST = decltype(steady)::value;
        constexpr int NMF = NPROD * MT * NT, NRD = NP * (MT + NT);
        read_frags(f1, st, 1);
        next_tap();
        Piece pc;
        if constexpr (ST) pc = prep_a();
        mma_frags(f0);
#pragma unroll
        for (int q = 0; q < NMF; ++q) {
            __builtin_amdgcn_sched_group_barrier(0x008, 1, 0);
            if (q < NRD) __builtin_amdgcn_sched_group_barrier(0x100, 1, 0);
            __builtin_amdgcn_sched_group_barrier(0x002, 3, 0);
        }
        __builtin_amdgcn_sched_barrier(0);
        const int st1 = st + 1 == NSTB ? 0 : st + 1;
        if constexpr (ST) wait_vmcnt<(NSTB - 2) * D>();
        else wait_tiles(min(NSTB - 2, nk - 2 - t));
        __builtin_amdgcn_s_barrier();
        if constexpr (ST) {
            issue_b(st);
            issue_piece(pc);
        }
        take_aaddr();
        read_frags(f0, st1, 0);
        mma_frags(f1);
#pragma unroll
        for (int q = 0; q < NMF; ++q) {
            __builtin_amdgcn_sched_group_barrier(0x008, 1, 1);
            if (ST && q == 0) __builtin_amdgcn_sched_group_barrier(0x020, D, 1);
            if (q < NRD) __builtin_amdgcn_sched_group_barrier(0x100, 1, 1);
        }
        __builtin_amdgcn_sched_barrier(0);
        if constexpr (ST) {
            advance_b();
            advance_a();
        }
        st = st1;
    };
    while (t + NSTB < nk) {
        for (const int te = min(nk - NSTB, t + ACC_BLOCK_TILES); t < te; ++t) body(std::true_type{});
        if (t + NSTB < nk) acc_close_block(acc, sum);
    }
    for (; t + 1 < nk; ++t) body(std::false_type{});
    read_frags(f1, st, 1);
    mma_frags(f0);
    mma_frags(f1);
    acc_total(acc, sum);

    __syncthreads();
#if ALDM_DMA_ABLATE & 16
    if (p.M == -12345) {
#pragma unroll
        for (int i = 0; i < MT; ++i)
#pragma unroll
            for (int j = 0; j < NT; ++j)
#pragma unroll
                for (int e = 0; e < 16; ++e) d.ws[(i * NT + j) * 16 + e + threadIdx.x * 256] = acc[i][j][e];
    }
    return;
#endif
    unscale_acc<F16>(acc, d.acc_scale);
    igemm_epilogue<MT, NT>(p, acc, reinterpret_cast<float*>(&smem[0]), m0, n0, wave, wm, wn, lane, 0, split);
}

}
```

audioldm2_amd/csrc/igemm_dma_halo.hip:

```cpp
#include "igemm_dma_halo.h"

namespace aldm {

#define ALDM_HALO_LIST(X)          \
    X(256, 128, 2, 4, 3, 18)       \
    X(128, 128, 3, 2, 3, 10)       \
    X(128, 128, 4, 2, 3, 10)       \
    X(128, 128, 2, 2, 3, 10)       \
    X(128, 128, 2, 4, 3, 10)       \
    X(128, 128, 3, 4, 3, 10)       \
    X(128, 128, 2, 2, 3, 16)       \
    X(128, 128, 2, 4, 3, 16)       \
    X(256, 128, 2, 4, 2, 18)       \
    X(256, 128, 3, 4, 2, 18)       \
    X(128, 128, 3, 2, 2, 10)       \
    X(128, 128, 4, 2, 2, 10)       \
    X(128, 128, 3, 4, 2, 10)       \
    X(128, 128, 3, 2, 2, 16)       \
    X(128, 128, 3, 4, 2, 16)

int igemm_dma_halo_maxch(int BM, int BN, int nstb, int wm, int parts, int nch) {
    int best = 0;
#define X(BM_, BN_, NST_, WM_, NP_, CH_)                                                                   \
    if (BM == BM_ && BN == BN_ && nstb == NST_ && wm == WM_ && parts == NP_ && nch <= CH_ &&             \
        nch * NP_ <= (11 - NST_) * WM_ * 2 && (best == 0 || CH_ < best))                                   \
        best = CH_;
    ALDM_HALO_LIST(X)
#undef X
    return best;
}

int igemm_launch_dma_halo(int BM, int BN, int nstb, int wm, int parts, bool f16, int maxch, dim3 grid, hipStream_t st, const IgemmK& p) {
    if (f16) {
#define X(BM_, BN_, NST_, WM_, NP_, CH_)                                                                                   \
    if constexpr (NP_ == 2) {                                                                                              \
        if (BM == BM_ && BN == BN_ && nstb == NST_ && wm == WM_ && parts == 2 && maxch == CH_) {                           \
            hipLaunchKernelGGL((igemm_dma_halo_kernel<BM_, BN_, NST_, WM_, 2, CH_, true>), grid, dim3(128 * WM_), 0, st, p); \
            return 0;                                                                                                      \
        }                                                                                                                  \
    }
        ALDM_HALO_LIST(X)
#undef X
        return -1;
    }
#define X(BM_, BN_, NST_, WM_, NP_, CH_)                                                                             \
    if (BM == BM_ && BN == BN_ && nstb == NST_ && wm == WM_ && parts == NP_ && maxch == CH_) {                      \
        hipLaunchKernelGGL((igemm_dma_halo_kernel<BM_, BN_, NST_, WM_, NP_, CH_>), grid, dim3(128 * WM_), 0, st, p); \
        return 0;                                                                                                    \
    }
    ALDM_HALO_LIST(X)
#undef X
    return -1;
}

}
```

audioldm2_amd/csrc/igemm_dma_lw.h:

```cpp
#pragma once
#include "igemm_dma.h"

namespace aldm {

template <int BM, int BN, int NST, int WM, int NP, int BPC, bool F16 = false>
__global__ __launch_bounds__(256 * WM, BPC * WM)
void igemm_dma_lw_kernel(const IgemmK p) {
    constexpr int WN = 2, NW = WM * WN;
    constexpr int MT = BM / (32 * WM), NT = BN / 64;
    constexpr int STG = dma_stage_slots(BM, BN, NP);
    constexpr int PB = 64 * NP;
    constexpr int RA = BM / (16 * NW);
    constexpr int NB = 4 * NP * (BN / 64) / NW;
    constexpr int D = NP * RA + NB;
    constexpr int NPROD = NP == 3 ? 6 : 3;
    static_assert(NP == 2 || NP == 3, "2 or 3 parts");
    static_assert(BM % (16 * NW) == 0 && (4 * NP * (BN / 64)) % NW == 0, "DMA chunks must divide among the loader waves");
    static_assert(NST >= 2 && NST <= 8 && (NST - 1) * D <= 63, "ring depth / vmcnt range");
    static_assert(NW * 32 * (NT * 32 + 4) * 4 <= NST * STG * 16, "epilogue staging must fit the ring");
    __shared__ u32x4 smem[NST * STG];

    const aldm_igemm_desc& d = p.d;
    const int lane = threadIdx.x & 63;
    const int wave_all = __builtin_amdgcn_readfirstlane(threadIdx.x >> 6);
    const bool loader = wave_all >= NW;
    const int wave = loader ? wave_all - NW : wave_all;
    const int wm = wave / WN, wn = wave % WN;
    const int l31 = lane & 31, lh = lane >> 5;

    int tile_m, tile_n;
    {
        const int nwg = gridDim.x;
        const int bid = blockIdx.x;
        const int q = nwg >> 3, r = nwg & 7;
        const int xcd = bid & 7, idx = bid >> 3;
        const int logical = (xcd < r ? xcd * (q + 1) : r * (q + 1) + (xcd - r) * q) + idx;
        tile_n = logical % p.tiles_n;
        tile_m = logical / p.tiles_n;
    }
    const int m0 = tile_m * BM, n0 = tile_n * BN;
    const int split = blockIdx.y;
    const int nk_all = d.K >> 5;
    const int kt0 = split * p.kt_per_split;
    const int kt1 = min(nk_all, kt0 + p.kt_per_split);
    const int nk = kt1 - kt0;

    if (loader) {
        const char* zero = reinterpret_cast<const char*>(g_dma_zero_page);
        const char* abase = reinterpret_cast<const char*>(d.a_split);
        const char* wbase = reinterpret_cast<const char*>(d.w_split);
        const int cpb = p.Cin >> 5;
        const int taps = d.KH * d.KW;
        const int64_t rowbytes = (int64_t)cpb * PB;
        const int lane_off = ((lane & 3) ^ ((lane >> 4) & 3)) * 16;
        int a_pix[RA], a_h[RA], a_w[RA];
#pragma unroll
        for (int i = 0; i < RA; ++i) {
            const int m = m0 + (wave * RA + i) * 16 + (lane >> 2);
            if (m < p.M) {
                const int b = m / p.OHW;
                const int rem = m - b * p.OHW;
                const int oh = rem / d.OW;
                const int ow = rem - oh * d.OW;
                a_pix[i] = b * d.H;
                a_h[i] = oh * d.SH - d.PH;
                a_w[i] = ow * d.SW - d.PW;
            } else {
                a_pix[i] = 0;
                a_h[i] = -(1 << 28);
                a_w[i] = 0;
            }
        }
        const char* a_ptr[RA];
        int a_step[RA];
        int t_kh, t_kw, t_cb;
        auto set_tap = [&]() {
            const int dh = t_kh * d.DH, dw = t_kw * d.DW;
            const int cboff = t_cb * PB + lane_off;
#pragma unroll
            for (int i = 0; i < RA; ++i) {
                const int ihv = a_h[i] + dh, iwv = a_w[i] + dw;
                const bool ok = (unsigned)ihv < (unsigned)p.HV && (unsigned)iwv < (unsigned)p.WV;
                const int pix = (a_pix[i] + (ihv >> p.shh)) * d.W + (iwv >> p.shw);
                a_ptr[i] = ok ? abase + ((int64_t)pix * rowbytes + cboff) : zero + lane_off;
                a_step[i] = ok ? PB : 0;
            }
        };
        {
            const int tap = kt0 / cpb;
            t_cb = kt0 - tap * cpb;
            t_kh = tap / d.KW;
            t_kw = tap - t_kh * d.KW;
            set_tap();
        }
        const char* b_ptr[NB];
        int64_t b_tile[NB];
#pragma unroll
        for (int j = 0; j < NB; ++j) {
            const int c = wave * NB + j;
            const int srow = c / (BN / 64), half = c % (BN / 64);
            const int col = n0 + half * 64 + lane;
            const bool ok = col < p.Npad;
            b_tile[j] = ok ? (int64_t)4 * NP * p.Npad * 16 : 0;
            const int tile0 = (t_kh * d.KW + t_kw) * cpb + t_cb;
            b_ptr[j] = ok ? wbase + (((int64_t)tile0 * 4 * NP + srow) * p.Npad + col) * 16 : zero;
        }
        using gptr_t = const __attribute__((address_space(1))) void*;
        using lptr_t = __attribute__((address_space(3))) void*;
        auto issue = [&](int st) {
            u32x4* sa = &smem[st * STG];
#pragma unroll
            for (int i = 0; i < RA; ++i)
#pragma unroll
                for (int q = 0; q < NP; ++q)
                    __builtin_amdgcn_global_load_lds((gptr_t)(a_ptr[i] + q * 64), (lptr_t)(sa + ((wave * RA + i) * NP + q) * 64),
                                                     16, 0, 0);
#pragma unroll
            for (int j = 0; j < NB; ++j) {
                const int c = wave * NB + j;
                const int srow = c / (BN / 64), half = c % (BN / 64);
                __builtin_amdgcn_global_load_lds((gptr_t)b_ptr[j], (lptr_t)(sa + BM * 4 * NP + srow * BN + half * 64), 16, 0, 0);
            }
#pragma unroll
            for (int i = 0; i < RA; ++i) a_ptr[i] += a_step[i];
#pragma unroll
            for (int j = 0; j < NB; ++j) b_ptr[j] += b_tile[j];
            if (++t_cb == cpb && taps > 1) {
                t_cb = 0;
                if (++t_kw == d.KW) {
                    t_kw = 0;
                    ++t_kh;
                }
                set_tap();
            }
        };
        auto wait_tiles = [&](int n) {
            constexpr int MX = NST - 1;
            if (n <= 0) wait_vmcnt<0>();
            else if (n == 1) wait_vmcnt<D>();
            else if (n == 2) wait_vmcnt<(MX >= 2 ? 2 : MX) * D>();
            else if (n == 3) wait_vmcnt<(MX >= 3 ? 3 : MX) * D>();
            else if (n == 4) wait_vmcnt<(MX >= 4 ? 4 : MX) * D>();
            else if (n == 5) wait_vmcnt<(MX >= 5 ? 5 : MX) * D>();
            else wait_vmcnt<(MX >= 6 ? 6 : MX) * D>();
        };
#pragma unroll
        for (int s = 0; s < NST; ++s)
            if (s < nk) issue(s);
        wait_tiles(min(nk, NST) - 1);
        __builtin_amdgcn_s_barrier();
        int st = 0, t = 0;
        for (; t + NST < nk; ++t) {
            wait_vmcnt<(NST - 2) * D>();
            __builtin_amdgcn_s_barrier();
            issue(st);
            st = st + 1 == NST ? 0 : st + 1;
        }
        for (; t + 1 < nk; ++t) {
            wait_tiles(min(NST - 2, nk - 2 - t));
            __builtin_amdgcn_s_barrier();
        }
        __builtin_amdgcn_s_barrier();
        return;
    }

    struct Frag {
        bf16x8 a[MT][NP], b[NT][NP];
    };
    const int a_sw = (l31 >> 2) & 3;
    auto read_frags = [&](Frag& f, int st, int step) {
        const u32x4* sa = &smem[st * STG];
        const int o = 2 * step + lh;
#pragma unroll
        for (int i = 0; i < MT; ++i) {
            const int row = (wm * MT + i) * 32 + l31;
#pragma unroll
            for (int q = 0; q < NP; ++q)
                f.a[i][q] = __builtin_bit_cast(bf16x8, sa[((row >> 4) * NP + q) * 64 + (row & 15) * 4 + (o ^ a_sw)]);
        }
#pragma unroll
        for (int j = 0; j < NT; ++j)
#pragma unroll
            for (int q = 0; q < NP; ++q)
                f.b[j][q] = __builtin_bit_cast(bf16x8, sa[BM * 4 * NP + (o * NP + q) * BN + (wn * NT + j) * 32 + l31]);
    };
    f32x16 acc[MT][NT], sum[MT][NT];
    acc_zero(acc);
    acc_zero(sum);
    auto mma_frags = [&](const Frag& f) {
        constexpr int PA_[6] = {NP == 3 ? 0 : 1, NP == 3 ? 2 : 0, NP == 3 ? 1 : 0, 0, 1, 0};
        constexpr int PB_[6] = {NP == 3 ? 2 : 0, NP == 3 ? 0 : 1, NP == 3 ? 1 : 0, 1, 0, 0};
#pragma unroll
        for (int q = 0; q < NPROD; ++q)
#pragma unroll
            for (int i = 0; i < MT; ++i)
#pragma unroll
                for (int j = 0; j < NT; ++j)
                    acc[i][j] = mfma_32x32x16<F16>(f.a[i][PA_[q]], f.b[j][PB_[q]], acc[i][j]);
    };
    constexpr int NMF = NPROD * MT * NT, NRD = NP * (MT + NT);
    __builtin_amdgcn_s_barrier();
    Frag f0, f1;
    read_frags(f0, 0, 0);
    int st = 0;
    for (int t = 0, te = 0; t + 1 < nk;) {
        if (t) acc_close_block(acc, sum);
        for (te = min(nk - 1, t + ACC_BLOCK_TILES); t < te; ++t) {
            read_frags(f1, st, 1);
            mma_frags(f0);
#pragma unroll
            for (int q = 0; q < NMF; ++q) {
                __builtin_amdgcn_sched_group_barrier(0x008, 1, 0);
                if (q < NRD) __builtin_amdgcn_sched_group_barrier(0x100, 1, 0);
            }
            __builtin_amdgcn_sched_barrier(0);
            const int st1 = st + 1 == NST ? 0 : st + 1;
            __builtin_amdgcn_s_waitcnt((7 << 4) | (3 << 14) | 15);
            __builtin_amdgcn_s_barrier();
            read_frags(f0, st1, 0);
            mma_frags(f1);
#pragma unroll
            for (int q = 0; q < NMF; ++q) {
                __builtin_amdgcn_sched_group_barrier(0x008, 1, 1);
                if (q < NRD) __builtin_amdgcn_sched_group_barrier(0x100, 1, 1);
            }
            __builtin_amdgcn_sched_barrier(0);
            st = st1;
        }
    }
    read_frags(f1, st, 1);
    mma_frags(f0);
    mma_frags(f1);
    acc_total(acc, sum);
    __builtin_amdgcn_s_waitcnt((7 << 4) | (3 << 14) | 15);
    __builtin_amdgcn_s_barrier();
    unscale_acc<F16>(acc, d.acc_scale);
    igemm_epilogue<MT, NT>(p, acc, reinterpret_cast<float*>(&smem[0]), m0, n0, wave, wm, wn, lane, 0, split);
}

}
```

audioldm2_amd/csrc/igemm_dma_lw.hip:

```cpp
#include "igemm_dma_lw.h"
#include <stdlib.h>

namespace aldm {

static int lw_bpc(int BM, int BN, int nst, int parts) {
    return (160 * 1024) / dma_lds_bytes(BM, BN, nst, parts) >= 2 ? 2 : 1;
}

bool igemm_dma_lw_config_ok(int BM, int BN, int nst, int parts) {
    if (parts == 2) {
        if (BM == 128 && BN == 128) return nst == 2 || nst == 4;
        if ((BM == 64 && BN == 128) || (BM == 128 && BN == 64)) return nst == 2 || nst == 3 || nst == 4;
        if (BM == 64 && BN == 64) return nst == 2 || nst == 3 || nst == 4;
        return false;
    }
    if (BM == 128 && BN == 128) return nst == 2 || nst == 3;
    if ((BM == 64 && BN == 128) || (BM == 128 && BN == 64)) return nst == 2 || nst == 4;
    if (BM == 64 && BN == 64) return nst == 2 || nst == 3;
    return false;
}

int igemm_launch_dma_lw(int BM, int BN, int nst, int parts, bool f16, dim3 grid, hipStream_t st, const IgemmK& p) {
    static const int env_bpc = [] {
        const char* e = getenv("ALDM_LW_BPC");
        return e ? atoi(e) : 0;
    }();
#define ALDM_LW_H(BM_, BN_, NST_, WM_)                                                                                  \
    if (f16 && BM == BM_ && BN == BN_ && nst == NST_ && parts == 2) {                                                  \
        constexpr bool two = (160 * 1024) / dma_lds_bytes(BM_, BN_, NST_, 2) >= 2 && BM_ * BN_ < 128 * 128;            \
        if (two && env_bpc != 1)                                                                                       \
            hipLaunchKernelGGL((igemm_dma_lw_kernel<BM_, BN_, NST_, WM_, 2, two ? 2 : 1, true>), grid, dim3(256 * WM_), 0, st, p); \
        else                                                                                                           \
            hipLaunchKernelGGL((igemm_dma_lw_kernel<BM_, BN_, NST_, WM_, 2, 1, true>), grid, dim3(256 * WM_), 0, st, p); \
        return 0;                                                                                                      \
    }
    ALDM_LW_H(128, 128, 2, 2)
    ALDM_LW_H(128, 128, 4, 2)
    ALDM_LW_H(64, 128, 2, 2)
    ALDM_LW_H(64, 128, 3, 2)
    ALDM_LW_H(64, 128, 4, 2)
    ALDM_LW_H(128, 64, 2, 2)
    ALDM_LW_H(128, 64, 3, 2)
    ALDM_LW_H(128, 64, 4, 2)
    ALDM_LW_H(64, 64, 2, 2)
    ALDM_LW_H(64, 64, 3, 2)
    ALDM_LW_H(64, 64, 4, 2)
#undef ALDM_LW_H
    if (f16) return -1;
#define ALDM_LW(BM_, BN_, NST_, WM_, NP_)                                                                              \
    if (BM == BM_ && BN == BN_ && nst == NST_ && parts == NP_) {                                                       \
        constexpr bool two = (160 * 1024) / dma_lds_bytes(BM_, BN_, NST_, NP_) >= 2 && BM_ * BN_ < 128 * 128;          \
        if (two && env_bpc != 1)                                                                                       \
            hipLaunchKernelGGL((igemm_dma_lw_kernel<BM_, BN_, NST_, WM_, NP_, two ? 2 : 1>), grid, dim3(256 * WM_), 0, st, p); \
        else                                                                                                           \
            hipLaunchKernelGGL((igemm_dma_lw_kernel<BM_, BN_, NST_, WM_, NP_, 1>), grid, dim3(256 * WM_), 0, st, p);   \
        return 0;                                                                                                      \
    }
    ALDM_LW(128, 128, 2, 2, 2)
    ALDM_LW(128, 128, 4, 2, 2)
    ALDM_LW(64, 128, 2, 2, 2)
    ALDM_LW(64, 128, 3, 2, 2)
    ALDM_LW(64, 128, 4, 2, 2)
    ALDM_LW(128, 64, 2, 2, 2)
    ALDM_LW(128, 64, 3, 2, 2)
    ALDM_LW(128, 64, 4, 2, 2)
    ALDM_LW(64, 64, 2, 2, 2)
    ALDM_LW(64, 64, 3, 2, 2)
    ALDM_LW(64, 64, 4, 2, 2)
    ALDM_LW(128, 128, 2, 2, 3)
    ALDM_LW(128, 128, 3, 2, 3)
    ALDM_LW(64, 128, 2, 2, 3)
    ALDM_LW(64, 128, 4, 2, 3)
    ALDM_LW(128, 64, 2, 2, 3)
    ALDM_LW(128, 64, 4, 2, 3)
    ALDM_LW(64, 64, 2, 2, 3)
    ALDM_LW(64, 64, 3, 2, 3)
#undef ALDM_LW
    (void)lw_bpc;
    return -1;
}

}
```

audioldm2_amd/csrc/igemm_epilogue.h:

```cpp
#pragma once
#include "common.h"

#ifndef ALDM_DMA_ABLATE
#define ALDM_DMA_ABLATE 0
#endif

namespace aldm {

struct IgemmK {
    aldm_igemm_desc d;
    int Cin, M, OHW, HV, WV, shh, shw, Kg, Npad, tiles_m, tiles_n;
    int splits, kt_per_split;
    int kgroups;
    int rb_ld;
    int bx;
    int pre;
    int dma;
    int nst;
    int ws;
    int ws_blocks;
    int os_rows;
};

enum { PRE_NONE = 0, PRE_AFFINE = 1, PRE_AFFINE_SILU = 2, PRE_LRELU = 3, PRE_GENERIC = 4 };

constexpr int ACC_BLOCK_TILES = 32;
template <int MT, int NT>
__device__ __forceinline__ void acc_zero(f32x16 (&a)[MT][NT]) {
#pragma unroll
    for (int i = 0; i < MT; ++i)
#pragma unroll
        for (int j = 0; j < NT; ++j)
#pragma unroll
            for (int e = 0; e < 16; ++e) a[i][j][e] = 0.f;
}
template <int MT, int NT>
__device__ __forceinline__ void acc_close_block(f32x16 (&acc)[MT][NT], f32x16 (&sum)[MT][NT]) {
#pragma unroll
    for (int i = 0; i < MT; ++i)
#pragma unroll
        for (int j = 0; j < NT; ++j)
#pragma unroll
            for (int e = 0; e < 16; ++e) {
                sum[i][j][e] += acc[i][j][e];
                acc[i][j][e] = 0.f;
            }
}
template <int MT, int NT>
__device__ __forceinline__ void acc_total(f32x16 (&acc)[MT][NT], const f32x16 (&sum)[MT][NT]) {
#pragma unroll
    for (int i = 0; i < MT; ++i)
#pragma unroll
        for (int j = 0; j < NT; ++j)
#pragma unroll
            for (int e = 0; e < 16; ++e) acc[i][j][e] += sum[i][j][e];
}

using bf16x8 = __bf16 __attribute__((ext_vector_type(8)));
using u32x2 = unsigned __attribute__((ext_vector_type(2)));
using u32x4 = unsigned __attribute__((ext_vector_type(4)));
__device__ __forceinline__ unsigned hi16_pair(unsigned a, unsigned b) { return __builtin_amdgcn_perm(b, a, 0x07060302u); }

constexpr int SPLIT_BLOCK_BYTES = 192;

__device__ __forceinline__ unsigned bf16_rn_bits(float x) {
    const unsigned u = __builtin_bit_cast(unsigned, x);
    return (u + 0x7FFFu + ((u >> 16) & 1u)) & 0xFFFF0000u;
}

__device__ __forceinline__ void split4(const f32x4 v, u32x2 (&part)[3]) {
    unsigned u0[4], u1[4], u2[4];
#pragma unroll
    for (int c = 0; c < 4; ++c) {
        const float x = v[c];
        u0[c] = __builtin_bit_cast(unsigned, x);
        const float r1 = x - __builtin_bit_cast(float, u0[c] & 0xFFFF0000u);
        u1[c] = __builtin_bit_cast(unsigned, r1);
        const float r2 = r1 - __builtin_bit_cast(float, u1[c] & 0xFFFF0000u);
        u2[c] = __builtin_bit_cast(unsigned, r2);
    }
    part[0] = u32x2{hi16_pair(u0[0], u0[1]), hi16_pair(u0[2], u0[3])};
    part[1] = u32x2{hi16_pair(u1[0], u1[1]), hi16_pair(u1[2], u1[3])};
    part[2] = u32x2{hi16_pair(u2[0], u2[1]), hi16_pair(u2[2], u2[3])};
}

using bf16x4 = __bf16 __attribute__((ext_vector_type(4)));
__device__ __forceinline__ void split4_rn2(const f32x4 v, u32x2 (&part)[3]) {
    const bf16x4 h = __builtin_convertvector(v, bf16x4);
    const bf16x4 m = __builtin_convertvector(v - __builtin_convertvector(h, f32x4), bf16x4);
    part[0] = __builtin_bit_cast(u32x2, h);
    part[1] = __builtin_bit_cast(u32x2, m);
    part[2] = u32x2{0u, 0u};
}

__device__ __forceinline__ void split4_parts(const f32x4 v, u32x2 (&part)[3], int parts) {
    if (parts == 2) split4_rn2(v, part);
    else split4(v, part);
}

using f16x4 = _Float16 __attribute__((ext_vector_type(4)));
using f16x8 = _Float16 __attribute__((ext_vector_type(8)));
__device__ __forceinline__ void split4_f16(const f32x4 v, float s, u32x2 (&part)[3]) {
    f32x4 x;
#pragma unroll
    for (int e = 0; e < 4; ++e) {
        const float t = v[e] * s;
        x[e] = t != t ? t : __builtin_fminf(__builtin_fmaxf(t, -65504.0f), 65504.0f);
    }
    const f16x4 h = __builtin_convertvector(x, f16x4);
    const f16x4 l = __builtin_convertvector(x - __builtin_convertvector(h, f32x4), f16x4);
    part[0] = __builtin_bit_cast(u32x2, h);
    part[1] = __builtin_bit_cast(u32x2, l);
    part[2] = u32x2{0u, 0u};
}
__device__ __forceinline__ void split4_fmt(const f32x4 v, u32x2 (&part)[3], int parts, float f16_scale) {
    if (f16_scale != 0.f) split4_f16(v, f16_scale, part);
    else split4_parts(v, part, parts);
}

__device__ __forceinline__ void split_store4(void* img, int64_t row, int Cs, int c, const f32x4 v, int parts = 3) {
    u32x2 part[3];
    split4_parts(v, part, parts);
    char* base = reinterpret_cast<char*>(img) + (row * (Cs >> 5) + (c >> 5)) * (64 * parts) + (c & 31) * 2;
#pragma unroll
    for (int q = 0; q < 3; ++q)
        if (q < parts) *reinterpret_cast<u32x2*>(base + q * 64) = part[q];
}

__device__ __forceinline__ void split_store4_f16(void* img, int64_t row, int Cs, int c, const f32x4 v, float scale) {
    u32x2 part[3];
    split4_f16(v, scale, part);
    char* base = reinterpret_cast<char*>(img) + (row * (Cs >> 5) + (c >> 5)) * 128 + (c & 31) * 2;
    *reinterpret_cast<u32x2*>(base) = part[0];
    *reinterpret_cast<u32x2*>(base + 64) = part[1];
}
__device__ __forceinline__ void split_store4_out(const aldm_igemm_desc& d, void* img, int64_t row, int Cs, int c, const f32x4 v) {
    if (d.out_split_fmt == ALDM_FMT_F16) split_store4_f16(img, row, Cs, c, v, d.out_split_scale);
    else split_store4(img, row, Cs, c, v, d.out_split_parts);
}

template <int P>
__device__ __forceinline__ void split_store4_t(void* img, int64_t row, int Cs, int c, const f32x4 v) {
    static_assert(P == 2 || P == 3, "2 or 3 parts");
    u32x2 part[3];
    if constexpr (P == 2) split4_rn2(v, part);
    else split4(v, part);
    char* base = reinterpret_cast<char*>(img) + (row * (Cs >> 5) + (c >> 5)) * (64 * P) + (c & 31) * 2;
#pragma unroll
    for (int q = 0; q < P; ++q) *reinterpret_cast<u32x2*>(base + q * 64) = part[q];
}

__device__ __forceinline__ float epi_value(const aldm_igemm_desc& d, int rb_ld, const float* __restrict__ outp,
                                           const float* __restrict__ resp, int b, int64_t o, int n, float v) {
    if (d.bias) v += d.bias[n];
    if (d.rowbias) v += d.rowbias[(int64_t)b * rb_ld + n];
    v = act_apply(v, d.act, d.act_slope);
    if (resp) v += resp[o];
    v *= d.alpha;
    if (d.accumulate) v += outp[o];
    return v;
}

__device__ __forceinline__ float silu_fast(float v) {
    return v * __frcp_rn(1.0f + __expf(-v));
}

__device__ __forceinline__ void split8_to_parts(const float (&x)[8], u32x4 (&part)[3], int parts) {
    f32x4 a = {x[0], x[1], x[2], x[3]}, b = {x[4], x[5], x[6], x[7]};
    u32x2 pa[3], pb[3];
    split4_parts(a, pa, parts);
    split4_parts(b, pb, parts);
#pragma unroll
    for (int q = 0; q < 3; ++q) part[q] = u32x4{pa[q][0], pa[q][1], pb[q][0], pb[q][1]};
}
// ... 83 lines not shown
            f32x4 bv = {0.f, 0.f, 0.f, 0.f}, bg = {0.f, 0.f, 0.f, 0.f};
            if (d.bias && cok) {
                bv = *reinterpret_cast<const f32x4*>(d.bias + ncol_p);
                bg = *reinterpret_cast<const f32x4*>(d.bias + ncol_p + 32);
            }
            float* go = d.out ? d.out + (int64_t)z * d.stride_o : nullptr;
            const int gate_act = d.act == ALDM_ACT_GELU_TANH ? ALDM_ACT_GELU_TANH : ALDM_ACT_GELU;
#pragma unroll
            for (int i = 0; i < MT; ++i) {
#pragma unroll
                for (int j = 0; j < NT; ++j)
#pragma unroll
                    for (int e = 0; e < 16; ++e)
                        stg[((e & 3) + 8 * (e >> 2) + 4 * lh) * SP + j * 32 + l31] = acc[i][j][e];
#pragma unroll
                for (int it = 0; it < 4; ++it) {
                    const int r = it * 8 + gr;
                    f32x4 xv = *reinterpret_cast<const f32x4*>(&stg[r * SP + gc]) + bv;
                    const f32x4 xg = *reinterpret_cast<const f32x4*>(&stg[r * SP + 32 + gc]) + bg;
#pragma unroll
                    for (int c = 0; c < 4; ++c) xv[c] *= act_apply(xg[c], gate_act, 0.f);
                    const int m = m0 + (wm * MT + i) * 32 + r;
                    if (m < p.M && cok && epi_st) {
                        if (go) *reinterpret_cast<f32x4*>(go + (int64_t)m * d.ldo + ncol_o) = xv;
                        if (simg) split_store4_out(d, simg, m, d.out_split_c, ncol_o, xv);
                    }
                }
            }
            return;
        }
    }
    f32x4 bias4 = {0.f, 0.f, 0.f, 0.f};
    if (!split_out && d.bias) {
#pragma unroll
        for (int c = 0; c < 4; ++c) bias4[c] = d.bias[min(ncol + c, d.N - 1)];
    }
#pragma unroll
    for (int i = 0; i < MT; ++i) {
#pragma unroll
        for (int j = 0; j < NT; ++j)
#pragma unroll
            for (int e = 0; e < 16; ++e)
                stg[((e & 3) + 8 * (e >> 2) + 4 * lh) * SP + j * 32 + l31] = acc[i][j][e];
#pragma unroll
        for (int itc = 0; itc < IT; itc += ITC) {
        f32x4 v[ITC];
        int64_t rowoff[ITC];
        int64_t srow[ITC];
        int rboff[ITC];
        unsigned okmask = 0;
#pragma unroll
        for (int it = 0; it < ITC; ++it) {
            const int r = (itc + it) * RPI + sr;
            v[it] = *reinterpret_cast<const f32x4*>(&stg[r * SP + sc]);
            const int m = m0 + (wm * MT + i) * 32 + r;
            bool ok = m < p.M && ncol < d.N;
            int b = 0;
            int64_t orow = m;
            if (need_b) {
                b = m / p.OHW;
                if (d.out_mul > 0) {
                    const int qq = m - b * p.OHW;
                    const int t = qq * d.out_mul + d.out_off;
                    ok = ok && (unsigned)t < (unsigned)d.out_len;
                    orow = (int64_t)b * d.out_len + t;
                }
            }
            rowoff[it] = ok ? orow * ld_out + (ncol - col_shift) : 0;
            srow[it] = orow;
            rboff[it] = ok ? b * p.rb_ld + ncol : 0;
            okmask |= ((ok && epi_st) ? 1u : 0u) << it;
        }
        if (split_out) {
#pragma unroll
            for (int it = 0; it < ITC; ++it)
                if ((okmask >> it) & 1u) *reinterpret_cast<f32x4*>(outp + rowoff[it]) = v[it];
            continue;
        }
#pragma unroll
        for (int it = 0; it < ITC; ++it) v[it] += bias4;
        if (d.rowbias) {
#pragma unroll
            for (int it = 0; it < ITC; ++it)
#pragma unroll
                for (int c = 0; c < 4; ++c) v[it][c] += d.rowbias[rboff[it] + (ncol + c < d.N ? c : 0)];
        }
        switch (d.act) {
            case ALDM_ACT_NONE: break;
            case ALDM_ACT_SILU:
#pragma unroll
                for (int it = 0; it < ITC; ++it)
#pragma unroll
                    for (int c = 0; c < 4; ++c) v[it][c] = act_apply(v[it][c], ALDM_ACT_SILU, 0.f);
                break;
            case ALDM_ACT_GELU:
#pragma unroll
                for (int it = 0; it < ITC; ++it)
#pragma unroll
                    for (int c = 0; c < 4; ++c) v[it][c] = act_apply(v[it][c], ALDM_ACT_GELU, 0.f);
                break;
            default:
#pragma unroll
                for (int it = 0; it < ITC; ++it)
#pragma unroll
                    for (int c = 0; c < 4; ++c) v[it][c] = act_apply(v[it][c], d.act, d.act_slope);
                break;
        }
        if (vec) {
            if (resp) {
#pragma unroll
                for (int it = 0; it < ITC; ++it) v[it] += *reinterpret_cast<const f32x4*>(resp + rowoff[it]);
            }
#pragma unroll
            for (int it = 0; it < ITC; ++it) v[it] *= d.alpha;
            if (d.accumulate) {
#pragma unroll
                for (int it = 0; it < ITC; ++it) v[it] += *reinterpret_cast<const f32x4*>(outp + rowoff[it]);
            }
            if (outp) {
#pragma unroll
                for (int it = 0; it < ITC; ++it)
                    if ((okmask >> it) & 1u) *reinterpret_cast<f32x4*>(outp + rowoff[it]) = v[it];
            }
            if (simg) {
                if (d.out_split_act == ALDM_ACT_LRELU) {
#pragma unroll
                    for (int it = 0; it < ITC; ++it)
#pragma unroll
                        for (int c = 0; c < 4; ++c) v[it][c] = v[it][c] > 0.0f ? v[it][c] : v[it][c] * d.out_split_slope;
                }
#pragma unroll
                for (int it = 0; it < ITC; ++it)
                    if ((okmask >> it) & 1u) {
                        split_store4_out(d, simg, srow[it], simg_c, ncol - col_shift, v[it]);
                    }
            }
        } else {
#pragma unroll
            for (int it = 0; it < ITC; ++it)
#pragma unroll
                for (int c = 0; c < 4; ++c) {
                    if (!((okmask >> it) & 1u) || ncol + c >= d.N) continue;
                    float x = v[it][c];
                    if (resp) x += resp[rowoff[it] + c];
                    x *= d.alpha;
                    if (d.accumulate) x += outp[rowoff[it] + c];
                    outp[rowoff[it] + c] = x;
                }
        }
        }
    }
}

}
```

audioldm2_amd/lib.py:

```python
from __future__ import annotations

import ctypes as C
import os

_HERE = os.path.dirname(os.path.abspath(__file__))
LIB_PATH = os.environ.get("ALDM_LIB_PATH") or os.path.join(_HERE, "libaldm_hip.so")
ABI_VERSION = 16

ACT_NONE, ACT_SILU, ACT_LRELU, ACT_TANH, ACT_LOGCLAMP, ACT_GELU, ACT_GELU_TANH = range(7)
B_PACKED, B_NT = 0, 1
EPI_PLAIN, EPI_GEGLU, EPI_QKV = 0, 1, 2
GN_CHUNKED, GN_FUSED, GN_FUSED_SPLIT = 0, 1, 2
FMT_BF16, FMT_F16 = 0, 1


class IgemmDesc(C.Structure):

    _fields_ = [
        ("x1", C.c_void_p), ("x2", C.c_void_p),
        ("C1", C.c_int32), ("C2", C.c_int32),
        ("pix1", C.c_int32), ("pix2", C.c_int32),
        ("B", C.c_int32), ("H", C.c_int32), ("W", C.c_int32),
        ("up_h", C.c_int32), ("up_w", C.c_int32),
        ("KH", C.c_int32), ("KW", C.c_int32), ("SH", C.c_int32), ("SW", C.c_int32),
        ("PH", C.c_int32), ("PW", C.c_int32), ("DH", C.c_int32), ("DW", C.c_int32),
        ("OH", C.c_int32), ("OW", C.c_int32),
        ("pre_scale", C.c_void_p), ("pre_shift", C.c_void_p),
        ("pre_act", C.c_int32), ("pre_slope", C.c_float),
        ("w", C.c_void_p),
        ("b_mode", C.c_int32), ("ldb", C.c_int32),
        ("K", C.c_int32), ("N", C.c_int32),
        ("bias", C.c_void_p), ("rowbias", C.c_void_p), ("res", C.c_void_p), ("out", C.c_void_p),
        ("ldo", C.c_int32), ("act", C.c_int32), ("act_slope", C.c_float), ("alpha", C.c_float),
        ("accumulate", C.c_int32),
        ("out_mul", C.c_int32), ("out_off", C.c_int32), ("out_len", C.c_int32),
        ("batch", C.c_int32),
        ("stride_x", C.c_int64), ("stride_w", C.c_int64), ("stride_o", C.c_int64),
        ("rowbias_ld", C.c_int32), ("epi_mode", C.c_int32),
        ("ws", C.c_void_p), ("ws_floats", C.c_int64),
        ("hint_bm", C.c_int32), ("hint_bn", C.c_int32), ("hint_splits", C.c_int32), ("hint_kgroups", C.c_int32),
        ("w_split", C.c_void_p), ("hint_mma", C.c_int32), ("hint_stages", C.c_int32),
        ("a_split", C.c_void_p), ("out_split", C.c_void_p), ("out_split_c", C.c_int32), ("split_parts", C.c_int32),
        ("out_split_act", C.c_int32), ("out_split_slope", C.c_float),
        ("k_split", C.c_void_p), ("vt_split", C.c_void_p), ("qkv_c", C.c_int32), ("qkv_rows", C.c_int32),
        ("a_fmt", C.c_int32), ("acc_scale", C.c_float), ("out_split_parts", C.c_int32),
        ("out_split_fmt", C.c_int32), ("out_split_scale", C.c_float), ("vt_scale", C.c_float),
    ]


_SIGS = {
    "aldm_version": (C.c_int, []),
    "aldm_last_error": (C.c_char_p, []),
    "aldm_igemm": (C.c_int, [C.POINTER(IgemmDesc), C.c_void_p]),
    "aldm_igemm_plan": (C.c_int, [C.POINTER(IgemmDesc), C.POINTER(C.c_int), C.POINTER(C.c_int),
                                  C.POINTER(C.c_int64), C.POINTER(C.c_int), C.POINTER(C.c_int),
                                  C.POINTER(C.c_int)]),
    "aldm_igemm_ws_floats": (C.c_int64, [C.POINTER(IgemmDesc)]),
    "aldm_igemm_plan_stages": (C.c_int, [C.POINTER(IgemmDesc)]),
    "aldm_igemm_force": (None, [C.c_int, C.c_int, C.c_int, C.c_int]),
    "aldm_igemm_force_stages": (None, [C.c_int]),
    "aldm_igemm_wave8_mask": (C.c_int, [C.c_int]),
    "aldm_split_image_bytes": (C.c_int64, [C.c_int64, C.c_int, C.c_int]),
    "aldm_split_rows": (C.c_int, [C.c_void_p, C.c_void_p, C.c_int, C.c_int, C.c_int64, C.c_int, C.c_void_p, C.c_void_p,
                                  C.c_int, C.c_void_p, C.c_void_p, C.c_int, C.c_void_p]),
    "aldm_split_rows_act": (C.c_int, [C.c_void_p, C.c_void_p, C.c_int, C.c_int, C.c_int64, C.c_int, C.c_void_p, C.c_void_p,
                                      C.c_int, C.c_float, C.c_void_p, C.c_void_p, C.c_int, C.c_void_p]),
    "aldm_layernorm_split": (C.c_int, [C.c_void_p, C.c_void_p, C.c_void_p, C.c_int, C.c_int, C.c_void_p, C.c_void_p,
                                       C.c_float, C.c_int, C.c_void_p]),
    "aldm_attention_d32_split": (C.c_int, [C.c_void_p, C.c_void_p, C.c_void_p, C.c_void_p, C.c_void_p, C.c_int, C.c_int,
                                           C.c_int, C.c_int, C.c_int, C.c_int, C.c_int, C.c_int, C.c_int,
                                           C.c_void_p, C.c_float, C.c_void_p]),
    "aldm_split_bytes_parts": (C.c_int64, [C.c_int, C.c_int, C.c_int]),
    "aldm_pack_split_bf16_parts": (C.c_int, [C.c_void_p, C.c_void_p, C.c_int, C.c_int, C.c_int, C.c_void_p]),
    "aldm_pack_split_f16": (C.c_int, [C.c_void_p, C.c_void_p, C.c_int, C.c_int, C.c_float, C.c_void_p]),
    "aldm_split_rows_f16": (C.c_int, [C.c_void_p, C.c_void_p, C.c_int, C.c_int, C.c_int64, C.c_int, C.c_void_p, C.c_void_p,
                                      C.c_int, C.c_float, C.c_void_p, C.c_void_p, C.c_int, C.c_float, C.c_void_p]),
    "aldm_groupnorm_split_f16": (C.c_int, [C.c_void_p, C.c_void_p, C.c_int, C.c_int, C.c_int, C.c_int, C.c_int, C.c_float,
                                           C.c_void_p, C.c_void_p, C.c_int, C.c_void_p, C.c_void_p, C.c_void_p, C.c_void_p,
                                           C.c_void_p, C.c_int, C.c_float, C.c_void_p]),
    "aldm_layernorm_split_f16": (C.c_int, [C.c_void_p, C.c_void_p, C.c_void_p, C.c_int, C.c_int, C.c_void_p, C.c_void_p,
                                           C.c_float, C.c_float, C.c_void_p]),
    "aldm_igemm_mma": (C.c_int, [C.c_int]),
    "aldm_split_bytes": (C.c_int64, [C.c_int, C.c_int]),
    "aldm_pack_split_bf16": (C.c_int, [C.c_void_p, C.c_void_p, C.c_int, C.c_int, C.c_void_p]),
    "aldm_pack_weight": (C.c_int, [C.c_void_p, C.c_void_p, C.c_int, C.c_int, C.c_int, C.c_int,
                                   C.c_int, C.c_int, C.c_int, C.c_void_p]),
    "aldm_pack_kn": (C.c_int, [C.c_void_p, C.c_void_p, C.c_int, C.c_int, C.c_int, C.c_int,
                               C.c_int64, C.c_int64, C.c_void_p]),
    "aldm_groupnorm_stats": (C.c_int, [C.c_void_p, C.c_void_p, C.c_int, C.c_int, C.c_int, C.c_int,
                                       C.c_int, C.c_float, C.c_void_p, C.c_void_p, C.c_void_p,
                                       C.c_void_p, C.c_void_p, C.c_void_p]),
    "aldm_gn_ws_floats": (C.c_int64, [C.c_int, C.c_int, C.c_int, C.c_int]),
    "aldm_groupnorm_plan": (C.c_int, [C.c_int] * 6 + [C.POINTER(C.c_int)] * 9),
    "aldm_groupnorm_split": (C.c_int, [C.c_void_p, C.c_void_p, C.c_int, C.c_int, C.c_int, C.c_int, C.c_int, C.c_float,
                                       C.c_void_p, C.c_void_p, C.c_int, C.c_void_p, C.c_void_p, C.c_void_p, C.c_void_p,
                                       C.c_void_p, C.c_int, C.c_void_p]),
    "aldm_layernorm": (C.c_int, [C.c_void_p, C.c_void_p, C.c_int, C.c_int, C.c_void_p, C.c_void_p,
                                 C.c_float, C.c_void_p]),
    "aldm_attention_mma": (C.c_int, [C.c_int]),
    "aldm_attention_sched": (C.c_int, [C.c_int]),
    "aldm_attention_query_tiles": (C.c_int, [C.c_int, C.c_int, C.c_int]),
    "aldm_attention_d32_presplit_f16": (C.c_int, [C.c_void_p, C.c_void_p, C.c_void_p, C.c_void_p, C.c_void_p, C.c_int, C.c_float,
                                                  C.c_int, C.c_int, C.c_int, C.c_int, C.c_int, C.c_int, C.c_float, C.c_float,
                                                  C.c_float, C.c_float, C.c_void_p]),
    "aldm_attention_d32_presplit": (C.c_int, [C.c_void_p, C.c_void_p, C.c_void_p, C.c_void_p, C.c_void_p, C.c_int, C.c_int,
                                              C.c_int, C.c_int, C.c_int, C.c_int, C.c_int, C.c_float, C.c_void_p]),
    "aldm_vt_regroup": (C.c_int, [C.c_void_p, C.c_void_p, C.c_int, C.c_int, C.c_int, C.c_int, C.c_void_p]),
    "aldm_attention_d32": (C.c_int, [C.c_void_p, C.c_void_p, C.c_void_p, C.c_void_p, C.c_int,
                                     C.c_int, C.c_int, C.c_int, C.c_int, C.c_int, C.c_int, C.c_int,
                                     C.c_void_p, C.c_float, C.c_void_p]),
    "aldm_rel_attention": (C.c_int, [C.c_void_p, C.c_void_p, C.c_void_p, C.c_void_p, C.c_int, C.c_int, C.c_int, C.c_int,
                                     C.c_int, C.c_int, C.c_int, C.c_int, C.c_void_p, C.c_void_p, C.c_int, C.c_void_p,
                                     C.c_void_p]),
    "aldm_rowscale_add": (C.c_int, [C.c_void_p, C.c_void_p, C.c_void_p, C.c_void_p, C.c_int64, C.c_int, C.c_int, C.c_void_p]),
    "aldm_rmsnorm": (C.c_int, [C.c_void_p, C.c_void_p, C.c_int, C.c_int, C.c_void_p, C.c_float, C.c_void_p]),
    "aldm_softmax_rows_bias": (C.c_int, [C.c_void_p, C.c_void_p, C.c_int, C.c_int, C.c_int, C.c_int, C.c_float, C.c_void_p,
                                         C.c_void_p, C.c_void_p]),
    "aldm_resample_sinc": (C.c_int, [C.c_void_p, C.c_void_p, C.c_void_p, C.c_int, C.c_int, C.c_int, C.c_int, C.c_int, C.c_int,
                                     C.c_int, C.c_void_p]),
    "aldm_power_spec": (C.c_int, [C.c_void_p, C.c_void_p, C.c_int64, C.c_int, C.c_int, C.c_int, C.c_void_p]),
    "aldm_col_affine": (C.c_int, [C.c_void_p, C.c_void_p, C.c_void_p, C.c_void_p, C.c_int64, C.c_int, C.c_void_p]),
    "aldm_bicubic_patchify": (C.c_int, [C.c_void_p, C.c_void_p, C.c_int, C.c_int, C.c_int, C.c_int, C.c_int, C.c_void_p]),
    "aldm_token_mean": (C.c_int, [C.c_void_p, C.c_void_p, C.c_int, C.c_int, C.c_int, C.c_void_p]),
    "aldm_row_cosine": (C.c_int, [C.c_void_p, C.c_void_p, C.c_void_p, C.c_int, C.c_int, C.c_float, C.c_void_p]),
    "aldm_decode_linear": (C.c_int, [C.c_void_p, C.c_int, C.c_int, C.c_int, C.c_void_p, C.c_int, C.c_void_p, C.c_void_p,
                                     C.c_void_p, C.c_float, C.c_int, C.c_void_p, C.c_int, C.c_void_p, C.c_int, C.c_void_p]),
    "aldm_decode_attention": (C.c_int, [C.c_void_p, C.c_int, C.c_void_p, C.c_void_p, C.c_void_p, C.c_void_p, C.c_int, C.c_int,
                                        C.c_int, C.c_float, C.c_void_p, C.c_int, C.c_void_p]),
    "aldm_decode_gemv_slices": (C.c_int, [C.c_int, C.c_int]),
    "aldm_decode_gemv": (C.c_int, [C.c_void_p, C.c_int, C.c_int, C.c_int64, C.c_void_p, C.c_int, C.c_int, C.c_int, C.c_void_p,
                                   C.c_int, C.c_void_p, C.c_void_p]),
    "aldm_decode_reduce_ln": (C.c_int, [C.c_void_p, C.c_int, C.c_int64, C.c_int, C.c_void_p, C.c_void_p, C.c_void_p, C.c_int,
                                        C.c_int, C.c_int, C.c_void_p, C.c_int, C.c_void_p, C.c_void_p, C.c_float, C.c_void_p,
                                        C.c_int, C.c_void_p, C.c_int, C.c_void_p]),
    "aldm_decode_attention_parts": (C.c_int, [C.c_void_p, C.c_int, C.c_int, C.c_int64, C.c_void_p, C.c_void_p, C.c_void_p,
                                              C.c_void_p, C.c_void_p, C.c_int, C.c_int, C.c_int, C.c_float, C.c_void_p, C.c_int,
                                              C.c_void_p]),
    "aldm_softmax_rows_masked": (C.c_int, [C.c_void_p, C.c_void_p, C.c_int, C.c_int, C.c_int, C.c_int, C.c_float,
                                           C.c_void_p, C.c_int, C.c_void_p]),
    "aldm_softmax_rows": (C.c_int, [C.c_void_p, C.c_void_p, C.c_int64, C.c_int, C.c_float,
                                    C.c_void_p]),
    "aldm_geglu": (C.c_int, [C.c_void_p, C.c_void_p, C.c_int64, C.c_int, C.c_void_p]),
    "aldm_timestep_embedding": (C.c_int, [C.c_void_p, C.c_void_p, C.c_int, C.c_int, C.c_float,
                                          C.c_void_p]),
    "aldm_nchw_to_nhwc": (C.c_int, [C.c_void_p, C.c_void_p, C.c_int, C.c_int, C.c_int, C.c_int,
                                    C.c_void_p]),
    "aldm_nhwc_to_nchw": (C.c_int, [C.c_void_p, C.c_void_p, C.c_int, C.c_int, C.c_int, C.c_void_p]),
    "aldm_ddim_step": (C.c_int, [C.c_void_p, C.c_void_p, C.c_void_p, C.c_void_p, C.c_void_p,
                                 C.c_void_p, C.c_int64, C.c_void_p]),
    "aldm_ddim_step_indexed": (C.c_int, [C.c_void_p, C.c_void_p, C.c_void_p, C.c_void_p, C.c_void_p, C.c_void_p, C.c_int64,
                                         C.c_int, C.c_void_p]),
    "aldm_plms_first_step": (C.c_int, [C.c_void_p, C.c_void_p, C.c_void_p, C.c_void_p, C.c_void_p, C.c_void_p, C.c_void_p,
                                       C.c_int64, C.c_void_p]),
    "aldm_plms_step_indexed": (C.c_int, [C.c_void_p, C.c_void_p, C.c_void_p, C.c_void_p, C.c_void_p, C.c_void_p, C.c_int64,
                                         C.c_int, C.c_void_p]),
    "aldm_dpmpp_step_indexed": (C.c_int, [C.c_void_p, C.c_void_p, C.c_void_p, C.c_void_p, C.c_void_p, C.c_int64, C.c_int,
                                          C.c_void_p]),
    "aldm_cfg_rescale_indexed": (C.c_int, [C.c_void_p, C.c_void_p, C.c_void_p, C.c_void_p, C.c_int, C.c_int64, C.c_int,
                                           C.c_void_p]),
    "aldm_step_advance": (C.c_int, [C.c_void_p, C.c_void_p, C.c_void_p, C.c_int, C.c_int, C.c_void_p]),
    "aldm_ddpm_step": (C.c_int, [C.c_void_p, C.c_void_p, C.c_void_p, C.c_void_p, C.c_void_p, C.c_int64,
                                 C.c_void_p]),
    "aldm_inpaint_blend": (C.c_int, [C.c_void_p, C.c_void_p, C.c_void_p, C.c_void_p, C.c_void_p,
                                     C.c_int64, C.c_void_p]),
    "aldm_posterior_qsample": (C.c_int, [C.c_void_p, C.c_void_p, C.c_void_p, C.c_void_p, C.c_void_p, C.c_void_p, C.c_int,
                                         C.c_int, C.c_int, C.c_int64, C.c_void_p]),
    "aldm_axpby": (C.c_int, [C.c_void_p, C.c_void_p, C.c_void_p, C.c_float, C.c_float, C.c_int64,
                             C.c_void_p]),
    "aldm_reflect_pad_1d": (C.c_int, [C.c_void_p, C.c_void_p, C.c_int, C.c_int, C.c_int, C.c_int,
                                      C.c_void_p]),
    "aldm_mag_phase": (C.c_int, [C.c_void_p, C.c_void_p, C.c_void_p, C.c_int64, C.c_int, C.c_int,
                                 C.c_int, C.c_void_p]),
    "aldm_row_l2norm": (C.c_int, [C.c_void_p, C.c_void_p, C.c_int64, C.c_int, C.c_int, C.c_void_p]),
}

EXPORTED_SYMBOLS = tuple(_SIGS.keys())
TEST_HOOK_SIGS = {"aldm_debug_drop_product": (C.c_int, [C.c_int])}
TESTHOOKS_LIB_PATH = os.path.join(_HERE, "libaldm_hip_testhooks.so")

_lib = None


def source_hash(family: str = "all") -> str:
    import glob
    import hashlib
    h = hashlib.sha256()
    files = sorted(glob.glob(os.path.join(_HERE, "csrc", "*.hip")) + glob.glob(os.path.join(_HERE, "csrc", "*.h")) +
                   glob.glob(os.path.join(os.path.dirname(_HERE), "include", "*.h")))
    if family == "igemm":
        files = [f for f in files if os.path.basename(f).startswith("igemm") or os.path.basename(f) in ("common.h", "aldm_hip.h")]
    elif family != "all":
        raise ValueError(f"source_hash: unknown family {family!r}")
    for f in files:
        h.update(os.path.basename(f).encode())
        with open(f, "rb") as fh:
            h.update(fh.read())
    return h.hexdigest()[:16]


def tuning_hash() -> str:
    import glob
    import hashlib
    h = hashlib.sha256()
    for f in sorted(glob.glob(os.path.join(_HERE, "tuning", "*.json"))):
        h.update(os.path.basename(f).encode())
        with open(f, "rb") as fh:
            h.update(fh.read())
    return h.hexdigest()[:16]


def load():
# ... 31 lines not shown
```

audioldm2_amd/ops.py:

```python
from __future__ import annotations

import ctypes as C
import json
import os
from dataclasses import dataclass
from typing import List, Optional, Sequence, Tuple

import torch

from . import lib as _l
from .lib import (ACT_GELU, ACT_GELU_TANH, ACT_LOGCLAMP, ACT_LRELU, ACT_NONE, ACT_SILU, ACT_TANH, B_NT, B_PACKED,
                  IgemmDesc)


def _stream() -> int:
    return torch.cuda.current_stream().cuda_stream


def _p(t: Optional[torch.Tensor]):
    return None if t is None else t.data_ptr()


def _chk(t: torch.Tensor, name: str):
    if not (t.is_cuda and t.dtype == torch.float32 and t.is_contiguous()):
# ... 271 lines not shown
    _l.check(_l.load().aldm_split_rows_act(x.data_ptr(), _p(x2), C1, C2, rows, P, _p(sc), _p(sh), act, slope, dst.data_ptr(),
                                           None if raw is None else raw.data_ptr(), dst.parts, _stream()), "split_rows")
    return (dst, raw) if want_raw else dst


PROFILE = None
ATTN_PROFILE = None


_ws = {}
_ws_retired = []
WS_SLOT = 0


def _workspace(lib, d: IgemmDesc, device) -> None:
    need = lib.aldm_igemm_ws_floats(C.byref(d))
    if need <= 0:
        return
    key = (device.index if device.index is not None else torch.cuda.current_device(), WS_SLOT)
    buf = _ws.get(key)
    if buf is None or buf.numel() < need:
        if torch.cuda.is_current_stream_capturing():
            return
        if buf is not None:
            _ws_retired.append(buf)
        buf = torch.empty(max(need, 8 << 20), device=device, dtype=torch.float32)
        _ws[key] = buf
    d.ws = buf.data_ptr()
    d.ws_floats = buf.numel()


_TUNE_FIELDS = ("B", "H", "W", "C1", "C2", "pix1", "up_h", "up_w", "KH", "KW", "SH", "SW", "PH", "PW", "DH", "DW",
                "OH", "OW", "N", "b_mode", "batch", "epi_mode", "out_mul")
_TUNED = None
TUNE_LOG = None


def tune_key(d: IgemmDesc) -> str:
    return ",".join(str(getattr(d, f)) for f in _TUNE_FIELDS) + f",{_pre_mode(d)}" + \
        (("," + ("dma2" if d.split_parts == 2 else "dma")) if d.a_split else "")


def _tuned_table(bx=False):
    global _TUNED
    if _TUNED is None:
        _TUNED = {False: {}, True: {}, "dma": {}, "dma2": {}}
        if os.environ.get("ALDM_NO_TUNING", "0") != "1":
            for mode, name in ((False, "mi355x_igemm.json"), (True, "mi355x_igemm_bf16x6.json"),
                               ("dma", "mi355x_igemm_dma.json"), ("dma2", "mi355x_igemm_dma_bf16x3.json")):
                path = os.path.join(os.environ.get("ALDM_TUNING_DIR", ""), name)
                if not (os.environ.get("ALDM_TUNING_DIR") and os.path.exists(path)):
                    path = os.path.join(os.path.dirname(os.path.abspath(__file__)), "tuning", name)
                if os.path.exists(path):
                    with open(path) as f:
                        _TUNED[mode] = {k: v[:5] if mode is True else v[:4] for k, v in json.load(f)["entries"].items()}
    return _TUNED[bx]


def _set_split_operand(d: IgemmDesc, x: "SplitT", pw: "Packed", so: Optional["SplitT"] = None) -> None:
    d.a_split = x.data_ptr()
    d.split_parts = x.parts
    if x.fmt == "f16":
        d.a_fmt = _l.FMT_F16
        d.w_split = pw.split16_ptr()
        d.acc_scale = 1.0 / (x.scale * pw.w_scale)
        d.out_split_parts = so.parts if so is not None else 3
    else:
        d.w_split = pw.split_ptr(x.parts)
        if so is not None:
            assert so.parts == x.parts and so.fmt == "bf16"


def _igemm(d: IgemmDesc, what: str, device=None):
    lib = _l.load()
    if d.a_split and d.epi_mode == _l.EPI_QKV:
        d.epi_mode = _l.EPI_PLAIN
        key = tune_key(d)
        d.epi_mode = _l.EPI_QKV
    else:
        key = tune_key(d)
    key_t = key
    if TUNE_LOG is not None:
        TUNE_LOG.append(key)
    if d.a_split:
        hint = _tuned_table("dma2" if d.split_parts == 2 else "dma").get(key_t)
        if hint is not None:
            d.hint_bm, d.hint_bn, d.hint_splits, d.hint_stages = hint[:4]
    else:
        hint = _tuned_table(bool(d.w_split)).get(key)
        if hint is not None:
            d.hint_bm, d.hint_bn, d.hint_splits, d.hint_kgroups = hint[:4]
            d.hint_mma = hint[4] if len(hint) > 4 else 0
    _workspace(lib, d, device if device is not None else torch.device("cuda", torch.cuda.current_device()))
    if PROFILE is None:
        _l.check(lib.aldm_igemm(C.byref(d), _stream()), what)
        return
    bm, bn, fl, sp, kg, mma = C.c_int(), C.c_int(), C.c_int64(), C.c_int(), C.c_int(), C.c_int()
    _l.check(lib.aldm_igemm_plan(C.byref(d), C.byref(bm), C.byref(bn), C.byref(fl), C.byref(sp), C.byref(kg),
                                 C.byref(mma)), what)
    e0 = torch.cuda.Event(enable_timing=True)
    e1 = torch.cuda.Event(enable_timing=True)
    e0.record()
    _l.check(lib.aldm_igemm(C.byref(d), _stream()), what)
    e1.record()
    shape = (d.B * d.OH * d.OW, d.N, d.K, d.KH * d.KW, d.C2, int(bool(d.pre_scale)), d.pre_act, d.batch,
             sp.value * 10 + kg.value, int(bool(d.a_split)), int(bool(d.out)), int(bool(d.out_split)), d.split_parts or 3,
             int(d.epi_mode == _l.EPI_GEGLU), int(bool(d.res)))
    PROFILE.append((what, bm.value, bn.value, fl.value, e0, e1, shape,
                    _kernel_name(d, bm.value, bn.value, kg.value, bool(mma.value))))


def _pre_mode(d: IgemmDesc) -> int:
    if not d.pre_scale and d.pre_act == ACT_NONE:
        return 0
    if d.pre_scale and d.pre_act == ACT_NONE:
        return 1
    if d.pre_scale and d.pre_act == ACT_SILU:
        return 2
    if not d.pre_scale and d.pre_act == ACT_LRELU:
        return 3
    return 4


def _kernel_name(d: IgemmDesc, bm: int, bn: int, kg: int = 1, bx: bool = False) -> str:
    if d.a_split:
        nst = _l.load().aldm_igemm_plan_stages(C.byref(d))
        if nst >= 400:
            w8 = (nst - 400) // 10
            return f"igemm_dma_halo_kernel<{bm}, {bn}, {(nst - 400) % 10}, {4 if (bm == 256 or w8) else 2}, {d.split_parts or 3}>"
        if nst >= 300:
            epi = 1 if d.epi_mode == _l.EPI_GEGLU else (2 if d.epi_mode == _l.EPI_QKV else 0)
            return f"igemm_dma_os_kernel<{d.K // 32}, {nst - 300}, {d.split_parts or 3}, {epi}>"
        if nst >= 200:
            return f"igemm_dma_lw_kernel<{bm}, {bn}, {nst - 200}, {4 if bm == 256 else 2}, {d.split_parts or 3}>"
        if nst >= 100:
            return f"igemm_dma_ws_kernel<{bm}, {bn}, {nst - 100}, {d.split_parts or 3}>"
        return f"igemm_dma_kernel<{bm}, {bn}, {nst}, {4 if bm == 256 else 2}, {d.split_parts or 3}>"
    pre = _pre_mode(d)
    wm, wn = (4, 1) if bn == 32 else (2, 2)
    w8 = _wave8_mask if _wave8_mask >= 0 else int(os.environ.get("ALDM_IGEMM_W8", "1"))
    bit = {(128, 128): 1, (64, 128): 2, (128, 64): 4}.get((bm, bn), 0)
    if kg == 1 and d.epi_mode != _l.EPI_GEGLU and (w8 & bit) and (
            bit == 1 if bx else (pre in (1, 2) or (bit == 1 and (w8 & 8)))):
        wm, wn = (4, 2) if bit == 4 else (2, 4)
    if bx and (bm, bn) == (128, 128) and d.epi_mode == _l.EPI_GEGLU and pre == 0:
        wm, wn = 4, 2
    uni = "true" if pre in (1, 2) and (d.OH * d.OW) % bm == 0 else "false"
    return f"igemm_kernel<{bm}, {bn}, {wm}, {wn}, {pre}, {kg}, {uni}, {'true' if bx else 'false'}>"


def igemm_force(bm: int = 0, bn: int = 0, splits: int = 0, kgroups: int = 0, stages: int = 0) -> None:
    _l.load().aldm_igemm_force(bm, bn, splits, kgroups)
    _l.load().aldm_igemm_force_stages(stages)


def attention_mma(mode: int) -> int:
    return _l.load().aldm_attention_mma(mode)


def attention_sched(sched: int) -> int:
    return _l.load().aldm_attention_sched(sched)


def attention_query_tiles(B: int, heads: int, Lq: int) -> int:
    return _l.load().aldm_attention_query_tiles(B, heads, Lq)


def debug_drop_product(on: bool) -> bool:
    fn = getattr(_l.load(), "aldm_debug_drop_product", None)
    if fn is None:
        raise RuntimeError("aldm_debug_drop_product is a test hook of libaldm_hip_testhooks.so; the release library does not "
                           f"export it (run with ALDM_LIB_PATH={_l.TESTHOOKS_LIB_PATH})")
    return bool(fn(1 if on else 0))


def igemm_mma(mode: int) -> int:
    return _l.load().aldm_igemm_mma(mode)


_wave8_mask = -1


def igemm_wave8(mask: int = -1) -> int:
    global _wave8_mask
    _wave8_mask = mask
    return _l.load().aldm_igemm_wave8_mask(mask)


def _npad(n: int) -> int:
    return (n + 31) // 32 * 32


def pack_conv(weight: torch.Tensor, bias: Optional[torch.Tensor] = None) -> Packed:
    w = weight.detach().to(device="cuda", dtype=torch.float32).contiguous()
    if w.dim() == 2:
        N, Cin, KH, KW = w.shape[0], w.shape[1], 1, 1
    elif w.dim() == 3:
        N, Cin, KH, KW = w.shape[0], w.shape[1], 1, w.shape[2]
    else:
        N, Cin, KH, KW = w.shape
    K = KH * KW * Cin
    dst = torch.empty(((K + 3) // 4) * _npad(N) * 4, device="cuda", dtype=torch.float32)
    lib = _l.load()
    _l.check(lib.aldm_pack_weight(w.data_ptr(), dst.data_ptr(), N, Cin, KH, KW, 0, 0, 1, _stream()),
             "pack_weight")
    b = None if bias is None else bias.detach().to(device="cuda", dtype=torch.float32).contiguous()
    return Packed(dst, N, Cin, KH, KW, b)


def pack_geglu(weight: torch.Tensor, bias: Optional[torch.Tensor]) -> Packed:
    two_inner = weight.shape[0]
    inner = two_inner // 2
    assert weight.dim() == 2 and two_inner % 64 == 0
    g = torch.arange(inner // 32).view(-1, 1, 1)
    j = torch.arange(2).view(1, -1, 1)
    l = torch.arange(32).view(1, 1, -1)
    perm = (j * inner + g * 32 + l).reshape(-1).to(weight.device)
    pw = pack_conv(weight.detach()[perm], None if bias is None else bias.detach()[perm])
    pw.geglu = True
    return pw


def linear_geglu(x, pw: Packed, split_out: Optional[str] = None, gate_act: int = ACT_NONE,
                 out: Optional[torch.Tensor] = None):
    is_split = isinstance(x, SplitT)
    if not is_split:
        _chk(x, "linear_geglu.x")
    shp = x.shape
    M = (x.rows if is_split else x.numel() // shp[-1])
    assert shp[-1] == pw.Cin and pw.KH == 1 and pw.KW == 1 and pw.N % 64 == 0
    oshape = (*shp[:-1], pw.N // 2)
    if split_out == "only":
        assert out is None
    elif out is None:
        out = torch.empty(oshape, device=x.device, dtype=torch.float32)
    else:
        _chk(out, "linear_geglu.out")
        assert out.numel() == M * (pw.N // 2), (out.shape, oshape)
        out = out.view(oshape)
    so = None
    if split_out:
        if is_split and x.fmt == "f16" and x.rn > 0.0 and f16_mode() and F16_FF_OUT:
            if pw.geglu:
                bound, typ = pw.geglu_bound(x.rn, x.rt)
            else:
                bound, typ = pw.out_bound(x.rn) ** 2, 0.0
            if typ <= 0.0 or bound <= typ * 2.0 ** F16_GEGLU_MAX_SLACK_LOG2:
                so = SplitT.empty(oshape, x.device, f16_scale=_pow2_scale(bound))
        if so is None:
            so = SplitT.empty(oshape, x.device)
    d = IgemmDesc()
    if is_split:
        _set_split_operand(d, x, pw, so if (so is None or so.fmt == "bf16") else None)
        if so is not None and so.fmt == "f16":
            d.out_split_fmt = _l.FMT_F16; d.out_split_scale = so.scale
    else:
        d.x1 = x.data_ptr(); d.split_parts = 3
        d.w_split = pw.split_ptr(3)
    if so is not None and not is_split:
        d.split_parts = so.parts
    d.C1 = pw.Cin; d.B = 1; d.H = 1; d.W = M; d.up_h = d.up_w = 1
    d.KH = d.KW = d.SH = d.SW = d.DH = d.DW = 1
    d.OH = 1; d.OW = M
    d.w = pw.data.data_ptr(); d.b_mode = B_PACKED; d.K = pw.K; d.N = pw.N
    d.bias = _p(pw.bias); d.out = _p(out); d.ldo = pw.N // 2; d.alpha = 1.0
    if so is not None:
        d.out_split = so.data_ptr(); d.out_split_c = pw.N // 2
    d.epi_mode = _l.EPI_GEGLU; d.batch = 1
    d.act = gate_act
    _igemm(d, "igemm(geglu)")
    return so if split_out == "only" else ((out, so) if split_out else out)


def linear_qkv(x: "SplitT", pw: Packed, heads: int, rows_per_sample: int):
    assert isinstance(x, SplitT) and pw.KH == 1 and pw.KW == 1 and pw.bias is None
    Cq = heads * 32
    assert pw.N == 3 * Cq and x.shape[-1] == pw.Cin
    M = x.rows
    assert M % rows_per_sample == 0
    Bn = M // rows_per_sample
    ragged = rows_per_sample % 32 != 0
    f16_kv = x.fmt == "f16" and x.rn > 0.0 and f16_mode() and F16_ATTN
    P = 2 if f16_kv else (3 if x.fmt == "f16" else x.parts)
    dev = x.device
    q = torch.empty((*x.shape[:-1], Cq), device=dev, dtype=torch.float32)
    if ragged:
        k_img = torch.empty((M + 31, heads, P, 32), device=dev, dtype=torch.int16)[:M]
        vt_img = torch.empty((Bn, heads, -(-rows_per_sample // 32), P, 32, 32), device=dev, dtype=torch.int16)
        vt_raw = torch.empty((heads, -(-M // 32), P, 32, 32), device=dev, dtype=torch.int16)
    else:
        k_img = torch.empty((M, heads, P, 32), device=dev, dtype=torch.int16)
        vt_img = torch.empty((Bn, heads, rows_per_sample // 32, P, 32, 32), device=dev, dtype=torch.int16)
    d = IgemmDesc()
    _set_split_operand(d, x, pw)
    d.out_split_parts = P
    if f16_kv:
        bound = pw.out_bound(x.rn)
        kv_scale = _pow2_scale(bound)
        q_scale = _pow2_scale(bound * (32 ** -0.5) * 1.4426950408889634)
        d.out_split_fmt = _l.FMT_F16; d.out_split_scale = kv_scale; d.vt_scale = kv_scale
        k_img._aldm_f16 = vt_img._aldm_f16 = (q_scale, kv_scale, kv_scale)
    d.C1 = pw.Cin; d.B = 1; d.H = 1; d.W = M; d.up_h = d.up_w = 1
    d.KH = d.KW = d.SH = d.SW = d.DH = d.DW = 1
    d.OH = 1; d.OW = M
    d.w = pw.data.data_ptr(); d.b_mode = B_PACKED; d.K = pw.K; d.N = pw.N
    d.out = q.data_ptr(); d.ldo = Cq; d.alpha = 1.0
# ... 833 lines not shown
```

include/aldm_hip.h:

```cpp
#ifndef ALDM_HIP_H
#define ALDM_HIP_H

#include <stdint.h>

#ifdef __cplusplus
extern "C" {
#endif

int aldm_version(void);
const char* aldm_last_error(void);

enum {
    ALDM_ACT_NONE = 0,
    ALDM_ACT_SILU = 1,
    ALDM_ACT_LRELU = 2,
    ALDM_ACT_TANH = 3,
    ALDM_ACT_LOGCLAMP = 4,
    ALDM_ACT_GELU = 5,
    ALDM_ACT_GELU_TANH = 6
};

enum { ALDM_EPI_PLAIN = 0, ALDM_EPI_GEGLU = 1, ALDM_EPI_QKV = 2 };

enum {
    ALDM_B_PACKED = 0,
    ALDM_B_NT = 1
};

enum { ALDM_MMA_F32 = 0, ALDM_MMA_BF16X6 = 1 };

typedef struct aldm_igemm_desc {
    const float* x1;
    const float* x2;
    int32_t C1, C2;
    int32_t pix1, pix2;
    int32_t B, H, W;
    int32_t up_h, up_w;
    int32_t KH, KW, SH, SW, PH, PW, DH, DW;
    int32_t OH, OW;
    const float* pre_scale;
    const float* pre_shift;
    int32_t pre_act;
    float pre_slope;
    const float* w;
    int32_t b_mode;
    int32_t ldb;
    int32_t K, N;
    const float* bias;
    const float* rowbias;
    const float* res;
    float* out;
    int32_t ldo;
    int32_t act;
    float act_slope;
    float alpha;
    int32_t accumulate;
    int32_t out_mul, out_off, out_len;
    int32_t batch;
    int64_t stride_x, stride_w, stride_o;
    int32_t rowbias_ld;
    int32_t epi_mode;
    float* ws;
    int64_t ws_floats;
    int32_t hint_bm, hint_bn, hint_splits;
    int32_t hint_kgroups;
    const void* w_split;
    int32_t hint_mma;
    int32_t hint_stages;
    const void* a_split;
    void* out_split;
    int32_t out_split_c;
    int32_t split_parts;
    int32_t out_split_act;
    float out_split_slope;
    void* k_split;
    void* vt_split;
    int32_t qkv_c;
    int32_t qkv_rows;
    int32_t a_fmt;
    float acc_scale;
    int32_t out_split_parts;
    int32_t out_split_fmt;
    float out_split_scale;
    float vt_scale;
} aldm_igemm_desc;

int aldm_igemm(const aldm_igemm_desc* d, void* stream);
int64_t aldm_igemm_ws_floats(const aldm_igemm_desc* d);
enum { ALDM_FMT_BF16 = 0, ALDM_FMT_F16 = 1 };
int aldm_igemm_plan(const aldm_igemm_desc* d, int* bm, int* bn, int64_t* flops, int* splits, int* kgroups,
                    int* mma);
int aldm_igemm_plan_stages(const aldm_igemm_desc* d);
void aldm_igemm_force(int bm, int bn, int splits, int kgroups);
void aldm_igemm_force_stages(int stages);
int aldm_igemm_wave8_mask(int mask);
int aldm_igemm_mma(int mode);
#ifdef ALDM_TEST_HOOKS
int aldm_debug_drop_product(int on);
#endif
int64_t aldm_split_bytes(int K, int N);
int aldm_pack_split_bf16(const float* packed, void* dst, int K, int N, void* stream);
int64_t aldm_split_bytes_parts(int K, int N, int parts);
int aldm_pack_split_bf16_parts(const float* packed, void* dst, int K, int N, int parts, void* stream);
int aldm_pack_split_f16(const float* packed, void* dst, int K, int N, float scale, void* stream);

int64_t aldm_split_image_bytes(int64_t rows, int C, int parts);
int aldm_split_rows(const float* x1, const float* x2, int C1, int C2, int64_t rows, int P, const float* scale,
                    const float* shift, int act, void* dst, void* dst_raw, int parts, void* stream);
int aldm_split_rows_act(const float* x1, const float* x2, int C1, int C2, int64_t rows, int P, const float* scale,
                        const float* shift, int act, float slope, void* dst, void* dst_raw, int parts, void* stream);
int aldm_split_rows_f16(const float* x1, const float* x2, int C1, int C2, int64_t rows, int P, const float* scale,
                        const float* shift, int act, float slope, void* dst, void* dst_raw, int raw_parts, float f16_scale,
                        void* stream);

int aldm_pack_weight(const float* src, float* dst, int N, int Cin, int KH, int KW,
                     int transposed, int phase, int stride, void* stream);
int aldm_pack_kn(const float* src, float* dst, int K, int N, int lds, int batch,
                 int64_t stride_src, int64_t stride_dst, void* stream);

int aldm_groupnorm_stats(const float* x1, const float* x2, int B, int P, int C1, int C2,
                         int G, float eps, const float* gamma, const float* beta,
                         float* scale, float* shift, float* ws, void* stream);
int64_t aldm_gn_ws_floats(int B, int P, int C, int G);
enum { ALDM_GN_CHUNKED = 0, ALDM_GN_FUSED = 1, ALDM_GN_FUSED_SPLIT = 2 };
int aldm_groupnorm_plan(int B, int P, int C1, int C2, int G, int want_split, int* form, int* group_slices,
                        int* groups_per_block, int* chunks, int* chunk_px, int* cols, int* rows, int* passes,
                        int* active_threads);
int aldm_groupnorm_split(const float* x1, const float* x2, int B, int P, int C1, int C2, int G, float eps,
                         const float* gamma, const float* beta, int act, float* scale, float* shift, float* ws,
                         void* dst, void* dst_raw, int parts, void* stream);
int aldm_groupnorm_split_f16(const float* x1, const float* x2, int B, int P, int C1, int C2, int G, float eps,
                             const float* gamma, const float* beta, int act, float* scale, float* shift, float* ws,
                             void* dst, void* dst_raw, int raw_parts, float f16_scale, void* stream);
int aldm_layernorm(const float* x, float* y, int M, int C, const float* gamma,
                   const float* beta, float eps, void* stream);
int aldm_layernorm_split(const float* x, float* y, void* y_split, int M, int C, const float* gamma,
                         const float* beta, float eps, int parts, void* stream);
int aldm_layernorm_split_f16(const float* x, float* y, void* y_split, int M, int C, const float* gamma,
                             const float* beta, float eps, float f16_scale, void* stream);

int aldm_attention_d32(const float* q, const float* k, const float* v, float* out,
                       int B, int heads, int Lq, int Lk, int ldq, int ldk, int ldv, int ldo,
                       const float* mask, float scale, void* stream);
int aldm_attention_d32_split(const float* q, const float* k, const float* v, float* out, void* out_split,
                             int parts, int B, int heads, int Lq, int Lk, int ldq, int ldk, int ldv, int ldo,
                             const float* mask, float scale, void* stream);
int aldm_attention_d32_presplit(const float* q, const void* k_split, const void* vt_split, float* out, void* out_split,
                                int parts, int B, int heads, int Lq, int Lk, int ldq, int ldo, float scale, void* stream);
int aldm_vt_regroup(const void* src, void* dst, int B, int L, int heads, int parts, void* stream);
int aldm_attention_mma(int mode);
int aldm_attention_sched(int sched);
int aldm_attention_query_tiles(int B, int heads, int Lq);
int aldm_attention_d32_presplit_f16(const float* q, const void* k_split, const void* vt_split, float* out, void* out_split,
                                    int out_parts, float out_scale, int B, int heads, int Lq, int Lk, int ldq, int ldo,
                                    float scale, float q_scale, float k_scale, float v_scale, void* stream);
int aldm_rel_attention(const float* q, const float* k, const float* v, float* out, int B, int heads, int T, int d,
                       int ldq, int ldk, int ldv, int ldo, const float* emb_k, const float* emb_v, int window,
                       const float* mask, void* stream);
int aldm_rowscale_add(const float* x, const float* s, const float* res, float* y, int64_t rows, int C, int divide,
                      void* stream);
int aldm_rmsnorm(const float* x, float* y, int M, int C, const float* weight, float eps, void* stream);
int aldm_softmax_rows_bias(const float* x, float* y, int B, int heads, int q_rows, int N, float scale, const float* bias,
                           const float* keymask, void* stream);
int aldm_softmax_rows(const float* x, float* y, int64_t M, int N, float scale, void* stream);
int aldm_softmax_rows_masked(const float* x, float* y, int B, int heads, int q_rows, int N, float scale,
                             const float* keymask, int q_pos0, void* stream);

int aldm_decode_linear(const float* x, int ldx, int M, int K, const float* w_kn, int N, const float* bias,
                       const float* ln_gamma, const float* ln_beta, float ln_eps, int act, const float* res, int ldr,
                       float* y, int ldy, void* stream);
int aldm_decode_attention(const float* qkv, int ldq, const int64_t* pos, float* k_cache, float* v_cache, const float* keymask,
                          int B, int heads, int n_tot, float scale, float* out, int ldo, void* stream);
int aldm_decode_gemv_slices(int K, int N);
int aldm_decode_gemv(const float* x, int ldx, int xparts, int64_t xstride, const float* xbias, int xact, int M, int K,
                     const float* w_kn, int N, float* ypart, void* stream);
int aldm_decode_reduce_ln(const float* part, int nparts, int64_t pstride, int ldp, const float* bias, const int64_t* bias_row,
                          const float* res, int ldr, int M, int N, float* h_out, int ldh, const float* ln_gamma,
                          const float* ln_beta, float ln_eps, float* xn, int ldn, float* xn2, int ldn2, void* stream);
int aldm_decode_attention_parts(const float* qkv_part, int ldq, int qparts, int64_t qstride, const float* qbias,
                                const int64_t* pos, float* k_cache, float* v_cache, const float* keymask, int B, int heads,
                                int n_tot, float scale, float* out, int ldo, void* stream);

int aldm_geglu(const float* x, float* y, int64_t M, int C, void* stream);
int aldm_timestep_embedding(const float* t, float* out, int B, int dim, float max_period,
                            void* stream);
int aldm_nchw_to_nhwc(const float* x, float* y, int B, int C, int HW, int rep, void* stream);
int aldm_nhwc_to_nchw(const float* x, float* y, int B, int C, int HW, void* stream);
int aldm_ddim_step(const float* x, const float* eps, const float* noise, const float* coef,
                   float* x_prev, float* pred_x0, int64_t n, void* stream);
int aldm_ddim_step_indexed(float* x, const float* eps, const float* noise_tab, const float* coef_tab,
                           const int* step_idx, float* pred_x0, int64_t n, int coef_ld, void* stream);
int aldm_plms_first_step(const float* x, const float* e_t, const float* e_next, const float* coef_row, float* x_out,
                         float* pred_x0, float* hist, int64_t n, void* stream);
int aldm_plms_step_indexed(float* x, const float* eps, float* hist, const float* coef_tab, const int* step_idx,
                           float* pred_x0, int64_t n, int coef_ld, void* stream);
int aldm_dpmpp_step_indexed(float* x, const float* eps, float* x0_buf, const float* coef_tab, const int* step_idx, int64_t n,
                            int coef_ld, void* stream);
int aldm_cfg_rescale_indexed(const float* eps, float* out, const float* coef_tab, const int* step_idx, int B, int64_t n_s,
                             int coef_ld, void* stream);
int aldm_step_advance(int* step_idx, const float* t_tab, float* t_cur, int nt, int steps, void* stream);
int aldm_ddpm_step(const float* x, const float* eps, const float* noise, const float* coef,
                   float* x_prev, int64_t n, void* stream);
int aldm_inpaint_blend(const float* x0, const float* qnoise, const float* mask, const float* coef,
                       float* x, int64_t n, void* stream);
int aldm_posterior_qsample(const float* moments_cl, const float* n_post, const float* n_enc, const float* coef, float* z,
                           float* x_t, int B0, int n_gen, int C, int64_t hw, void* stream);
int aldm_axpby(const float* a, const float* b, float* y, float alpha, float beta, int64_t n,
               void* stream);
int aldm_reflect_pad_1d(const float* x, float* y, int B, int T, int pad, int ld_out,
                        void* stream);
int aldm_mag_phase(const float* spec, float* mag, float* phase, int64_t M, int F, int ld_spec,
                   int ld_mag, void* stream);

int aldm_row_l2norm(const float* x, float* out, int64_t M, int F, int ld, void* stream);

int aldm_resample_sinc(const float* x, const float* kernel, float* y, int B, int T, int Tout, int down, int up, int taps,
                       int width, void* stream);
int aldm_power_spec(const float* spec, float* out, int64_t M, int F, int ld_spec, int ld_out, void* stream);
int aldm_col_affine(const float* x, const float* scale, const float* shift, float* y, int64_t rows, int C, void* stream);
int aldm_bicubic_patchify(const float* x, float* out, int B, int T, int mel, int S, int p, void* stream);
int aldm_token_mean(const float* x, float* y, int B, int L, int C, void* stream);
int aldm_row_cosine(const float* a, const float* b, float* out, int M, int C, float eps, void* stream);

#ifdef __cplusplus
}
#endif
#endif
```

Baseline: 18.65 audio-s/s.

## Add specialized epilogue forms with prefetched bias/residual to DMA igemm kernels

Adds compile-time epilogue variants (plain, rowbias, residual) for the DMA, LW and halo igemm kernels. They apply only to the common case of no activation, alpha 1, single split and aligned pointers. Bias, residual and rowbias vectors are loaded into registers before the main K loop so their latency overlaps compute, and the epilogue becomes a simpler vectorized path than the generic one. The cost is extra register pressure from holding the prefetched values, more kernel instantiations, and planner logic that decides which form applies. It is on by default and can be turned off with an environment variable.

```diff
diff --git a/audioldm2_amd/csrc/api.hip b/audioldm2_amd/csrc/api.hip
--- a/audioldm2_amd/csrc/api.hip
+++ b/audioldm2_amd/csrc/api.hip
@@ -11,5 +11,5 @@
 }
 }
 
-extern "C" int aldm_version(void) { return 16; }
+extern "C" int aldm_version(void) { return 17; }
 extern "C" const char* aldm_last_error(void) { return aldm::g_err; }
diff --git a/audioldm2_amd/csrc/igemm.hip b/audioldm2_amd/csrc/igemm.hip
--- a/audioldm2_amd/csrc/igemm.hip
+++ b/audioldm2_amd/csrc/igemm.hip
@@ -30,6 +30,9 @@
 int igemm_dma_os_default_stages(int KT, int parts);
 int igemm_launch_dma_halo(int BM, int BN, int nstb, int wm, int parts, bool f16, int maxch, dim3 grid, hipStream_t st, const IgemmK& p);
 int igemm_dma_halo_maxch(int BM, int BN, int nstb, int wm, int parts, int nch);
+bool igemm_dma_form_ok(int BM, int BN, int nst, int parts);
+bool igemm_dma_lw_form_ok(int BM, int BN, int nst, int parts);
+bool igemm_dma_halo_form_ok(int BM, int BN, int nstb, int wm, int parts, int maxch);
 
 __global__ __launch_bounds__(256) void igemm_reduce_kernel(const IgemmK p) {
     const aldm_igemm_desc& d = p.d;
@@ -232,6 +235,44 @@
     return prev;
 }
 
+static std::atomic<int> g_epi_forms{-1};
+static int epi_forms_on() {
+    static const int env_on = [] {
+        const char* e = getenv("ALDM_EPI_FORMS");
+        return (e && e[0] == '0' && e[1] == 0) ? 0 : 1;
+    }();
+    const int v = g_epi_forms.load(std::memory_order_relaxed);
+    return v < 0 ? env_on : v;
+}
+extern "C" int aldm_igemm_epilogue_forms(int on) {
+    const int prev = epi_forms_on();
+    g_epi_forms.store(on == 0 || on == 1 ? on : -1, std::memory_order_relaxed);
+    return prev;
+}
+
+static int plan_epilogue_form(const IgemmK& p, int BM, int BN) {
+    const aldm_igemm_desc& d = p.d;
+    if (!epi_forms_on() || !p.dma || d.a_fmt != ALDM_FMT_BF16) return ALDM_EPI_FORM_GENERIC;
+    const bool inst = p.ws == 0   ? igemm_dma_form_ok(BM, BN, p.nst, d.split_parts)
+                      : p.ws == 2 ? igemm_dma_lw_form_ok(BM, BN, p.nst, d.split_parts)
+                      : p.ws == 4 ? igemm_dma_halo_form_ok(BM, BN, p.nst, p.ws_blocks, d.split_parts, p.os_rows)
+                                  : false;
+    if (!inst) return ALDM_EPI_FORM_GENERIC;
+    if (d.epi_mode != ALDM_EPI_PLAIN || p.splits != 1 || d.act != ALDM_ACT_NONE || d.alpha != 1.0f || d.accumulate ||
+        d.out_mul > 0 || d.batch != 1)
+        return ALDM_EPI_FORM_GENERIC;
+    auto al16 = [](const void* q) { return (reinterpret_cast<uintptr_t>(q) & 15) == 0; };
+    if ((d.N & 3) != 0 || (d.ldo & 3) != 0 || (d.stride_o & 3) != 0 || !al16(d.out) || !al16(d.res) || !al16(d.bias) ||
+        !al16(d.rowbias) || (d.rowbias && (p.rb_ld & 3) != 0))
+        return ALDM_EPI_FORM_GENERIC;
+    if (d.out_split && (d.out_split_fmt != ALDM_FMT_BF16 || d.out_split_parts != d.split_parts)) return ALDM_EPI_FORM_GENERIC;
+#ifdef ALDM_TEST_HOOKS
+    if (g_debug_drop_product.load(std::memory_order_relaxed)) return ALDM_EPI_FORM_GENERIC;
+#endif
+    if (d.res && d.rowbias) return ALDM_EPI_FORM_GENERIC;
+    return d.res ? ALDM_EPI_FORM_RES : (d.rowbias ? ALDM_EPI_FORM_ROWBIAS : ALDM_EPI_FORM_PLAIN);
+}
+
 static int pre_mode_of(const aldm_igemm_desc& d) {
     if (d.pre_scale == nullptr && d.pre_act == ALDM_ACT_NONE) return PRE_NONE;
     if (d.pre_scale != nullptr && d.pre_act == ALDM_ACT_NONE) return PRE_AFFINE;
@@ -292,6 +333,7 @@
     ALDM_CHECK(dd != nullptr, "aldm_igemm: null descriptor");
     p.d = *dd;
     aldm_igemm_desc& d = p.d;
+    p.epi_form = ALDM_EPI_FORM_GENERIC;
     ALDM_CHECK((d.x1 || d.a_split) && d.w && (d.out || d.out_split), "aldm_igemm: null x1/w/out");
     if (!d.x1) d.x1 = reinterpret_cast<const float*>(d.a_split);
     if (d.split_parts == 0) d.split_parts = 3;
@@ -695,6 +737,13 @@
     return p.dma ? p.nst + 100 * p.ws : 0;
 }
 
+extern "C" int aldm_igemm_plan_epilogue(const aldm_igemm_desc* dd) {
+    IgemmK p;
+    int BM, BN;
+    if (igemm_prepare(dd, p, BM, BN)) return -1;
+    return plan_epilogue_form(p, BM, BN);
+}
+
 extern "C" int64_t aldm_igemm_ws_floats(const aldm_igemm_desc* dd) {
     if (!dd) return 0;
     aldm_igemm_desc t = *dd;
@@ -711,6 +760,7 @@
     int BM, BN;
     int rc = igemm_prepare(dd, p, BM, BN);
     if (rc) return rc;
+    p.epi_form = plan_epilogue_form(p, BM, BN);
     const aldm_igemm_desc& d = p.d;
     dim3 grid((unsigned)(p.tiles_m * p.tiles_n), (unsigned)p.splits, (unsigned)d.batch);
     hipStream_t st = (hipStream_t)stream;
diff --git a/audioldm2_amd/csrc/igemm_dma.h b/audioldm2_amd/csrc/igemm_dma.h
--- a/audioldm2_amd/csrc/igemm_dma.h
+++ b/audioldm2_amd/csrc/igemm_dma.h
@@ -43,7 +43,7 @@
 #define ALDM_DMA_ABLATE 0
 #endif
 
-template <int BM, int BN, int NST, int WM = 2, int NP = 3, bool DROP = false, bool F16 = false>
+template <int BM, int BN, int NST, int WM = 2, int NP = 3, bool DROP = false, bool F16 = false, int FORM = ALDM_EPI_FORM_GENERIC>
 __global__ __launch_bounds__(128 * WM, dma_blocks_per_cu(BM, BN, NST, NP) * (WM / 2))
 void igemm_dma_kernel(const IgemmK p) {
     constexpr int WN = 2, NW = WM * WN;
@@ -56,6 +56,7 @@
     constexpr int NPROD = NP == 3 ? 6 : 3;
     static_assert(NP == 2 || NP == 3, "2 or 3 parts");
     static_assert(!F16 || NP == 2, "fp16 images have two parts");
+    static_assert(!F16 || FORM == ALDM_EPI_FORM_GENERIC, "the epilogue forms write bf16 images");
     static_assert(BM % (16 * NW) == 0 && (4 * NP * (BN / 64)) % NW == 0, "DMA chunks must divide among the waves");
     static_assert(NST >= 2 && NST <= 8 && (NST - 1) * D <= 63, "ring depth / vmcnt range");
     static_assert(NW * 32 * (NT * 32 + 4) * 4 <= NST * STG * 16, "epilogue staging must fit the ring");
@@ -271,6 +272,8 @@
         else wait_vmcnt<(MX >= 6 ? 6 : MX) * D>();
     };
 
+    EpiPre<MT, NT, FORM> epre;
+    if constexpr (FORM != ALDM_EPI_FORM_GENERIC) epi_form_prefetch(p, epre, m0, n0, wm, wn, lane);
 #pragma unroll
     for (int s = 0; s < NST; ++s)
         if (s < nk) issue(s);
@@ -336,7 +339,10 @@
     return;
 #endif
     unscale_acc<F16>(acc, d.acc_scale);
-    igemm_epilogue<MT, NT>(p, acc, reinterpret_cast<float*>(&smem[0]), m0, n0, wave, wm, wn, lane, 0, split);
-}
-
-}
+    if constexpr (FORM != ALDM_EPI_FORM_GENERIC)
+        igemm_epilogue_form<MT, NT, NP, FORM>(p, acc, epre, reinterpret_cast<float*>(&smem[0]), m0, n0, wave, wm, wn, lane);
+    else
+        igemm_epilogue<MT, NT>(p, acc, reinterpret_cast<float*>(&smem[0]), m0, n0, wave, wm, wn, lane, 0, split);
+}
+
+}
diff --git a/audioldm2_amd/csrc/igemm_dma.hip b/audioldm2_amd/csrc/igemm_dma.hip
--- a/audioldm2_amd/csrc/igemm_dma.hip
+++ b/audioldm2_amd/csrc/igemm_dma.hip
@@ -15,6 +15,8 @@
 std::atomic<int> g_debug_drop_product{0};
 #endif
 
+int igemm_launch_dma_form(int BM, int BN, int nst, int form, dim3 grid, hipStream_t st, const IgemmK& p);
+
 int igemm_launch_dma(int BM, int BN, int nst, int parts, bool f16, dim3 grid, hipStream_t st, const IgemmK& p) {
 #ifdef ALDM_TEST_HOOKS
     if (g_debug_drop_product.load(std::memory_order_relaxed)) {
@@ -23,6 +25,7 @@
         return 0;
     }
 #endif
+    if (p.epi_form != ALDM_EPI_FORM_GENERIC) return igemm_launch_dma_form(BM, BN, nst, p.epi_form, grid, st, p);
 #define ALDM_DMA(BM_, BN_, NST_, NP_) \
     hipLaunchKernelGGL((igemm_dma_kernel<BM_, BN_, NST_, 2, NP_>), grid, dim3(256), 0, st, p)
 #define ALDM_DMA8(BM_, BN_, NST_, NP_) \
diff --git a/audioldm2_amd/csrc/igemm_dma_forms.hip b/audioldm2_amd/csrc/igemm_dma_forms.hip
--- /dev/null
+++ b/audioldm2_amd/csrc/igemm_dma_forms.hip
@@ -0,0 +1,38 @@
+#include "igemm_dma.h"
+
+namespace aldm {
+
+bool igemm_dma_form_ok(int BM, int BN, int nst, int parts) {
+    if (parts != 3) return false;
+    if ((BM == 64 && BN == 128) || (BM == 128 && BN == 64)) return nst == 2 || nst == 4;
+    if (BM == 64 && BN == 64) return nst == 2 || nst == 3;
+    return false;
+}
+
+template <int BM, int BN, int NST>
+static int launch_forms(int form, dim3 grid, hipStream_t st, const IgemmK& p) {
+    switch (form) {
+        case ALDM_EPI_FORM_PLAIN:
+            hipLaunchKernelGGL((igemm_dma_kernel<BM, BN, NST, 2, 3, false, false, ALDM_EPI_FORM_PLAIN>), grid, dim3(256), 0, st, p);
+            return 0;
+        case ALDM_EPI_FORM_ROWBIAS:
+            hipLaunchKernelGGL((igemm_dma_kernel<BM, BN, NST, 2, 3, false, false, ALDM_EPI_FORM_ROWBIAS>), grid, dim3(256), 0, st, p);
+            return 0;
+        case ALDM_EPI_FORM_RES:
+            hipLaunchKernelGGL((igemm_dma_kernel<BM, BN, NST, 2, 3, false, false, ALDM_EPI_FORM_RES>), grid, dim3(256), 0, st, p);
+            return 0;
+    }
+    return -1;
+}
+
+int igemm_launch_dma_form(int BM, int BN, int nst, int form, dim3 grid, hipStream_t st, const IgemmK& p) {
+    if (BM == 64 && BN == 64 && nst == 2) return launch_forms<64, 64, 2>(form, grid, st, p);
+    if (BM == 64 && BN == 64 && nst == 3) return launch_forms<64, 64, 3>(form, grid, st, p);
+    if (BM == 128 && BN == 64 && nst == 2) return launch_forms<128, 64, 2>(form, grid, st, p);
+    if (BM == 128 && BN == 64 && nst == 4) return launch_forms<128, 64, 4>(form, grid, st, p);
+    if (BM == 64 && BN == 128 && nst == 2) return launch_forms<64, 128, 2>(form, grid, st, p);
+    if (BM == 64 && BN == 128 && nst == 4) return launch_forms<64, 128, 4>(form, grid, st, p);
+    return -1;
+}
+
+}
diff --git a/audioldm2_amd/csrc/igemm_dma_halo.h b/audioldm2_amd/csrc/igemm_dma_halo.h
--- a/audioldm2_amd/csrc/igemm_dma_halo.h
+++ b/audioldm2_amd/csrc/igemm_dma_halo.h
@@ -11,7 +11,7 @@
     return 2 * MAXCH * NP * 64 + NSTB * BN * 4 * NP + NP * 64;
 }
 
-template <int BM, int BN, int NSTB, int WM, int NP, int MAXCH, bool F16 = false>
+template <int BM, int BN, int NSTB, int WM, int NP, int MAXCH, bool F16 = false, int FORM = ALDM_EPI_FORM_GENERIC>
 __global__ __launch_bounds__(128 * WM, WM / 2)
 void igemm_dma_halo_kernel(const IgemmK p) {
     constexpr int WN = 2, NW = WM * WN;
@@ -26,6 +26,7 @@
     constexpr int ATILES = 11 - NSTB;
     constexpr int NPROD = NP == 3 ? 6 : 3;
     static_assert(NP == 2 || NP == 3, "2 or 3 parts");
+    static_assert(!F16 || FORM == ALDM_EPI_FORM_GENERIC, "the epilogue forms write bf16 images");
     static_assert((4 * NP * (BN / 64)) % NW == 0, "weight pieces must divide among the waves");
     static_assert(NSTB >= 2 && NSTB <= 6 && (NSTB - 1) * D <= 63, "ring depth / vmcnt range");
     static_assert(NW * 32 * (NT * 32 + 4) * 4 <= Z0 * 16, "epilogue staging must fit");
@@ -220,6 +221,8 @@
         else wait_vmcnt<(MX >= 4 ? 4 : MX) * D>();
     };
 
+    EpiPre<MT, NT, FORM> epre;
+    if constexpr (FORM != ALDM_EPI_FORM_GENERIC) epi_form_prefetch(p, epre, m0, n0, wm, wn, lane);
     if (wave < NP)
         __builtin_amdgcn_global_load_lds((gptr_t)(zero + lane * 16), (lptr_t)&smem[Z0 + wave * 64], 16, 0, 0);
     for (int id = wave; id < NCH * NP; id += NW) issue_piece(prep_patch_piece(id, 0, true));
@@ -306,7 +309,10 @@
     return;
 #endif
     unscale_acc<F16>(acc, d.acc_scale);
-    igemm_epilogue<MT, NT>(p, acc, reinterpret_cast<float*>(&smem[0]), m0, n0, wave, wm, wn, lane, 0, split);
+    if constexpr (FORM != ALDM_EPI_FORM_GENERIC)
+        igemm_epilogue_form<MT, NT, NP, FORM>(p, acc, epre, reinterpret_cast<float*>(&smem[0]), m0, n0, wave, wm, wn, lane);
+    else
+        igemm_epilogue<MT, NT>(p, acc, reinterpret_cast<float*>(&smem[0]), m0, n0, wave, wm, wn, lane, 0, split);
 }
 
 }
diff --git a/audioldm2_amd/csrc/igemm_dma_halo.hip b/audioldm2_amd/csrc/igemm_dma_halo.hip
--- a/audioldm2_amd/csrc/igemm_dma_halo.hip
+++ b/audioldm2_amd/csrc/igemm_dma_halo.hip
@@ -30,7 +30,10 @@
     return best;
 }
 
+int igemm_launch_dma_halo_form(int BM, int BN, int nstb, int wm, int maxch, int form, dim3 grid, hipStream_t st, const IgemmK& p);
+
 int igemm_launch_dma_halo(int BM, int BN, int nstb, int wm, int parts, bool f16, int maxch, dim3 grid, hipStream_t st, const IgemmK& p) {
+    if (p.epi_form != ALDM_EPI_FORM_GENERIC) return igemm_launch_dma_halo_form(BM, BN, nstb, wm, maxch, p.epi_form, grid, st, p);
     if (f16) {
 #define X(BM_, BN_, NST_, WM_, NP_, CH_)                                                                                   \
     if constexpr (NP_ == 2) {                                                                                              \
diff --git a/audioldm2_amd/csrc/igemm_dma_halo_forms.hip b/audioldm2_amd/csrc/igemm_dma_halo_forms.hip
--- /dev/null
+++ b/audioldm2_amd/csrc/igemm_dma_halo_forms.hip
@@ -0,0 +1,33 @@
+#include "igemm_dma_halo.h"
+
+namespace aldm {
+
+bool igemm_dma_halo_form_ok(int BM, int BN, int nstb, int wm, int parts, int maxch) {
+    if (parts != 3 || BM != 128 || BN != 128 || maxch != 10) return false;
+    return (nstb == 4 && wm == 2) || (nstb == 2 && wm == 4);
+}
+
+template <int NSTB, int WM>
+static int launch_forms(int form, dim3 grid, hipStream_t st, const IgemmK& p) {
+    switch (form) {
+        case ALDM_EPI_FORM_PLAIN:
+            hipLaunchKernelGGL((igemm_dma_halo_kernel<128, 128, NSTB, WM, 3, 10, false, ALDM_EPI_FORM_PLAIN>), grid, dim3(128 * WM), 0, st, p);
+            return 0;
+        case ALDM_EPI_FORM_ROWBIAS:
+            hipLaunchKernelGGL((igemm_dma_halo_kernel<128, 128, NSTB, WM, 3, 10, false, ALDM_EPI_FORM_ROWBIAS>), grid, dim3(128 * WM), 0, st, p);
+            return 0;
+        case ALDM_EPI_FORM_RES:
+            hipLaunchKernelGGL((igemm_dma_halo_kernel<128, 128, NSTB, WM, 3, 10, false, ALDM_EPI_FORM_RES>), grid, dim3(128 * WM), 0, st, p);
+            return 0;
+    }
+    return -1;
+}
+
+int igemm_launch_dma_halo_form(int BM, int BN, int nstb, int wm, int maxch, int form, dim3 grid, hipStream_t st, const IgemmK& p) {
+    if (BM != 128 || BN != 128 || maxch != 10) return -1;
+    if (nstb == 4 && wm == 2) return launch_forms<4, 2>(form, grid, st, p);
+    if (nstb == 2 && wm == 4) return launch_forms<2, 4>(form, grid, st, p);
+    return -1;
+}
+
+}
diff --git a/audioldm2_amd/csrc/igemm_dma_lw.h b/audioldm2_amd/csrc/igemm_dma_lw.h
--- a/audioldm2_amd/csrc/igemm_dma_lw.h
+++ b/audioldm2_amd/csrc/igemm_dma_lw.h
@@ -3,7 +3,7 @@
 
 namespace aldm {
 
-template <int BM, int BN, int NST, int WM, int NP, int BPC, bool F16 = false>
+template <int BM, int BN, int NST, int WM, int NP, int BPC, bool F16 = false, int FORM = ALDM_EPI_FORM_GENERIC>
 __global__ __launch_bounds__(256 * WM, BPC * WM)
 void igemm_dma_lw_kernel(const IgemmK p) {
     constexpr int WN = 2, NW = WM * WN;
@@ -15,6 +15,7 @@
     constexpr int D = NP * RA + NB;
     constexpr int NPROD = NP == 3 ? 6 : 3;
     static_assert(NP == 2 || NP == 3, "2 or 3 parts");
+    static_assert(!F16 || FORM == ALDM_EPI_FORM_GENERIC, "the epilogue forms write bf16 images");
     static_assert(BM % (16 * NW) == 0 && (4 * NP * (BN / 64)) % NW == 0, "DMA chunks must divide among the loader waves");
     static_assert(NST >= 2 && NST <= 8 && (NST - 1) * D <= 63, "ring depth / vmcnt range");
     static_assert(NW * 32 * (NT * 32 + 4) * 4 <= NST * STG * 16, "epilogue staging must fit the ring");
@@ -199,6 +200,8 @@
                     acc[i][j] = mfma_32x32x16<F16>(f.a[i][PA_[q]], f.b[j][PB_[q]], acc[i][j]);
     };
     constexpr int NMF = NPROD * MT * NT, NRD = NP * (MT + NT);
+    EpiPre<MT, NT, FORM> epre;
+    if constexpr (FORM != ALDM_EPI_FORM_GENERIC) epi_form_prefetch(p, epre, m0, n0, wm, wn, lane);
     __builtin_amdgcn_s_barrier();
     Frag f0, f1;
     read_frags(f0, 0, 0);
@@ -235,7 +238,10 @@
     __builtin_amdgcn_s_waitcnt((7 << 4) | (3 << 14) | 15);
     __builtin_amdgcn_s_barrier();
     unscale_acc<F16>(acc, d.acc_scale);
-    igemm_epilogue<MT, NT>(p, acc, reinterpret_cast<float*>(&smem[0]), m0, n0, wave, wm, wn, lane, 0, split);
+    if constexpr (FORM != ALDM_EPI_FORM_GENERIC)
+        igemm_epilogue_form<MT, NT, NP, FORM>(p, acc, epre, reinterpret_cast<float*>(&smem[0]), m0, n0, wave, wm, wn, lane);
+    else
+        igemm_epilogue<MT, NT>(p, acc, reinterpret_cast<float*>(&smem[0]), m0, n0, wave, wm, wn, lane, 0, split);
 }
 
 }
diff --git a/audioldm2_amd/csrc/igemm_dma_lw.hip b/audioldm2_amd/csrc/igemm_dma_lw.hip
--- a/audioldm2_amd/csrc/igemm_dma_lw.hip
+++ b/audioldm2_amd/csrc/igemm_dma_lw.hip
@@ -20,11 +20,19 @@
     return false;
 }
 
-int igemm_launch_dma_lw(int BM, int BN, int nst, int parts, bool f16, dim3 grid, hipStream_t st, const IgemmK& p) {
+int igemm_dma_lw_env_bpc() {
     static const int env_bpc = [] {
         const char* e = getenv("ALDM_LW_BPC");
         return e ? atoi(e) : 0;
     }();
+    return env_bpc;
+}
+
+int igemm_launch_dma_lw_form(int BM, int BN, int nst, int form, dim3 grid, hipStream_t st, const IgemmK& p);
+
+int igemm_launch_dma_lw(int BM, int BN, int nst, int parts, bool f16, dim3 grid, hipStream_t st, const IgemmK& p) {
+    const int env_bpc = igemm_dma_lw_env_bpc();
+    if (p.epi_form != ALDM_EPI_FORM_GENERIC) return igemm_launch_dma_lw_form(BM, BN, nst, p.epi_form, grid, st, p);
 #define ALDM_LW_H(BM_, BN_, NST_, WM_)                                                                                  \
     if (f16 && BM == BM_ && BN == BN_ && nst == NST_ && parts == 2) {                                                  \
         constexpr bool two = (160 * 1024) / dma_lds_bytes(BM_, BN_, NST_, 2) >= 2 && BM_ * BN_ < 128 * 128;            \
diff --git a/audioldm2_amd/csrc/igemm_dma_lw_forms.hip b/audioldm2_amd/csrc/igemm_dma_lw_forms.hip
--- /dev/null
+++ b/audioldm2_amd/csrc/igemm_dma_lw_forms.hip
@@ -0,0 +1,41 @@
+#include "igemm_dma_lw.h"
+
+namespace aldm {
+
+int igemm_dma_lw_env_bpc();
+
+bool igemm_dma_lw_form_ok(int BM, int BN, int nst, int parts) {
+    if (parts != 3 || igemm_dma_lw_env_bpc() == 1) return false;
+    if (BM == 64 && BN == 128) return nst == 2 || nst == 4;
+    if (BM == 128 && BN == 64) return nst == 4;
+    if (BM == 64 && BN == 64) return nst == 2 || nst == 3;
+    return false;
+}
+
+template <int BM, int BN, int NST>
+static int launch_forms(int form, dim3 grid, hipStream_t st, const IgemmK& p) {
+    constexpr int BPC = (160 * 1024) / dma_lds_bytes(BM, BN, NST, 3) >= 2 ? 2 : 1;
+    switch (form) {
+        case ALDM_EPI_FORM_PLAIN:
+            hipLaunchKernelGGL((igemm_dma_lw_kernel<BM, BN, NST, 2, 3, BPC, false, ALDM_EPI_FORM_PLAIN>), grid, dim3(512), 0, st, p);
+            return 0;
+        case ALDM_EPI_FORM_ROWBIAS:
+            hipLaunchKernelGGL((igemm_dma_lw_kernel<BM, BN, NST, 2, 3, BPC, false, ALDM_EPI_FORM_ROWBIAS>), grid, dim3(512), 0, st, p);
+            return 0;
+        case ALDM_EPI_FORM_RES:
+            hipLaunchKernelGGL((igemm_dma_lw_kernel<BM, BN, NST, 2, 3, BPC, false, ALDM_EPI_FORM_RES>), grid, dim3(512), 0, st, p);
+            return 0;
+    }
+    return -1;
+}
+
+int igemm_launch_dma_lw_form(int BM, int BN, int nst, int form, dim3 grid, hipStream_t st, const IgemmK& p) {
+    if (BM == 64 && BN == 64 && nst == 2) return launch_forms<64, 64, 2>(form, grid, st, p);
+    if (BM == 64 && BN == 64 && nst == 3) return launch_forms<64, 64, 3>(form, grid, st, p);
+    if (BM == 128 && BN == 64 && nst == 4) return launch_forms<128, 64, 4>(form, grid, st, p);
+    if (BM == 64 && BN == 128 && nst == 2) return launch_forms<64, 128, 2>(form, grid, st, p);
+    if (BM == 64 && BN == 128 && nst == 4) return launch_forms<64, 128, 4>(form, grid, st, p);
+    return -1;
+}
+
+}
diff --git a/audioldm2_amd/csrc/igemm_epilogue.h b/audioldm2_amd/csrc/igemm_epilogue.h
--- a/audioldm2_amd/csrc/igemm_epilogue.h
+++ b/audioldm2_amd/csrc/igemm_epilogue.h
@@ -20,6 +20,7 @@
     int ws;
     int ws_blocks;
     int os_rows;
+    int epi_form;
 };
 
 enum { PRE_NONE = 0, PRE_AFFINE = 1, PRE_AFFINE_SILU = 2, PRE_LRELU = 3, PRE_GENERIC = 4 };
@@ -409,4 +410,111 @@
     }
 }
 
-}
+template <int NT>
+struct EpiGeom {
+    static constexpr int C4 = NT * 8;
+    static constexpr int RPI = 64 / C4;
+    static constexpr int IT = 32 / RPI;
+};
+template <int MT, int NT, int FORM>
+struct EpiPre {
+    static constexpr bool OPT = FORM == ALDM_EPI_FORM_RES || FORM == ALDM_EPI_FORM_ROWBIAS;
+    f32x4 bias4;
+    f32x4 opt[OPT ? MT : 1][OPT ? EpiGeom<NT>::IT : 1];
+};
+
+template <int MT, int NT, int FORM>
+__device__ __forceinline__ void epi_form_prefetch(const IgemmK& p, EpiPre<MT, NT, FORM>& q, int m0, int n0, int wm, int wn, int lane) {
+    using G = EpiGeom<NT>;
+    const aldm_igemm_desc& d = p.d;
+    const int sr = lane / G::C4;
+    const int ncol = n0 + wn * NT * 32 + (lane % G::C4) * 4;
+    const bool cok = ncol < d.N;
+    q.bias4 = f32x4{0.f, 0.f, 0.f, 0.f};
+    if (d.bias) q.bias4 = *reinterpret_cast<const f32x4*>(d.bias + (cok ? ncol : 0));
+    if constexpr (EpiPre<MT, NT, FORM>::OPT) {
+#pragma unroll
+        for (int i = 0; i < MT; ++i)
+#pragma unroll
+            for (int it = 0; it < G::IT; ++it) {
+                const int m = m0 + (wm * MT + i) * 32 + it * G::RPI + sr;
+                const bool ok = m < p.M && cok;
+                if constexpr (FORM == ALDM_EPI_FORM_RES)
+                    q.opt[i][it] = *reinterpret_cast<const f32x4*>(d.res + (ok ? (int64_t)m * d.ldo + ncol : 0));
+                else
+                    q.opt[i][it] = *reinterpret_cast<const f32x4*>(d.rowbias + (ok ? (m / p.OHW) * p.rb_ld + ncol : 0));
+            }
+    }
+}
+
+template <int MT, int NT, int NP, int FORM, int PAD = 4>
+__device__ __forceinline__ void igemm_epilogue_form(const IgemmK& p, f32x16 (&acc)[MT][NT], const EpiPre<MT, NT, FORM>& q, float* lds,
+                                                    int m0, int n0, int wave, int wm, int wn, int lane) {
+    using G = EpiGeom<NT>;
+    const aldm_igemm_desc& d = p.d;
+    const bool epi_st = (ALDM_DMA_ABLATE & 64) ? p.M == -12345 : true;
+    constexpr int SP = NT * 32 + PAD;
+    constexpr int ITC = G::IT < 4 ? G::IT : 4;
+    const int l31 = lane & 31;
+    const int lh = lane >> 5;
+    float* stg = lds + wave * (32 * SP);
+    const int sr = lane / G::C4;
+    const int sc = (lane % G::C4) * 4;
+    const int ncol = n0 + wn * NT * 32 + sc;
+    float* const outp = d.out;
+    void* const simg = d.out_split;
+    const bool lrelu_img = d.out_split_act == ALDM_ACT_LRELU;
+    asm volatile("" ::"v"(q.bias4));
+    if constexpr (EpiPre<MT, NT, FORM>::OPT) {
+#pragma unroll
+        for (int i = 0; i < MT; ++i)
+#pragma unroll
+            for (int it = 0; it < G::IT; ++it) asm volatile("" ::"v"(q.opt[i][it]));
+    }
+#pragma unroll
+    for (int i = 0; i < MT; ++i) {
+#pragma unroll
+        for (int j = 0; j < NT; ++j)
+#pragma unroll
+            for (int e = 0; e < 16; ++e)
+                stg[((e & 3) + 8 * (e >> 2) + 4 * lh) * SP + j * 32 + l31] = acc[i][j][e];
+#pragma unroll
+        for (int itc = 0; itc < G::IT; itc += ITC) {
+            f32x4 v[ITC];
+            int64_t rowoff[ITC];
+            unsigned okmask = 0;
+#pragma unroll
+            for (int it = 0; it < ITC; ++it) {
+                const int r = (itc + it) * G::RPI + sr;
+                v[it] = *reinterpret_cast<const f32x4*>(&stg[r * SP + sc]);
+                const int m = m0 + (wm * MT + i) * 32 + r;
+                const bool ok = m < p.M && ncol < d.N;
+                rowoff[it] = m;
+                okmask |= ((ok && epi_st) ? 1u : 0u) << it;
+            }
+#pragma unroll
+            for (int it = 0; it < ITC; ++it) {
+                v[it] += q.bias4;
+                if constexpr (EpiPre<MT, NT, FORM>::OPT) v[it] += q.opt[i][itc + it];
+            }
+            if (outp) {
+#pragma unroll
+                for (int it = 0; it < ITC; ++it)
+                    if ((okmask >> it) & 1u) *reinterpret_cast<f32x4*>(outp + rowoff[it] * d.ldo + ncol) = v[it];
+            }
+            if (simg) {
+                if (lrelu_img) {
+#pragma unroll
+                    for (int it = 0; it < ITC; ++it)
+#pragma unroll
+                        for (int c = 0; c < 4; ++c) v[it][c] = v[it][c] > 0.0f ? v[it][c] : v[it][c] * d.out_split_slope;
+                }
+#pragma unroll
+                for (int it = 0; it < ITC; ++it)
+                    if ((okmask >> it) & 1u) split_store4_t<NP>(simg, rowoff[it], d.out_split_c, ncol, v[it]);
+            }
+        }
+    }
+}
+
+}
diff --git a/audioldm2_amd/lib.py b/audioldm2_amd/lib.py
--- a/audioldm2_amd/lib.py
+++ b/audioldm2_amd/lib.py
@@ -5,13 +5,14 @@
 
 _HERE = os.path.dirname(os.path.abspath(__file__))
 LIB_PATH = os.environ.get("ALDM_LIB_PATH") or os.path.join(_HERE, "libaldm_hip.so")
-ABI_VERSION = 16
+ABI_VERSION = 17
 
 ACT_NONE, ACT_SILU, ACT_LRELU, ACT_TANH, ACT_LOGCLAMP, ACT_GELU, ACT_GELU_TANH = range(7)
 B_PACKED, B_NT = 0, 1
 EPI_PLAIN, EPI_GEGLU, EPI_QKV = 0, 1, 2
 GN_CHUNKED, GN_FUSED, GN_FUSED_SPLIT = 0, 1, 2
 FMT_BF16, FMT_F16 = 0, 1
+EPI_FORM_GENERIC, EPI_FORM_PLAIN, EPI_FORM_ROWBIAS, EPI_FORM_RES = range(4)
 
 
 class IgemmDesc(C.Structure):
@@ -57,6 +58,8 @@
                                   C.POINTER(C.c_int)]),
     "aldm_igemm_ws_floats": (C.c_int64, [C.POINTER(IgemmDesc)]),
     "aldm_igemm_plan_stages": (C.c_int, [C.POINTER(IgemmDesc)]),
+    "aldm_igemm_plan_epilogue": (C.c_int, [C.POINTER(IgemmDesc)]),
+    "aldm_igemm_epilogue_forms": (C.c_int, [C.c_int]),
     "aldm_igemm_force": (None, [C.c_int, C.c_int, C.c_int, C.c_int]),
     "aldm_igemm_force_stages": (None, [C.c_int]),
     "aldm_igemm_wave8_mask": (C.c_int, [C.c_int]),
diff --git a/audioldm2_amd/ops.py b/audioldm2_amd/ops.py
--- a/audioldm2_amd/ops.py
+++ b/audioldm2_amd/ops.py
@@ -447,6 +447,10 @@
 def igemm_force(bm: int = 0, bn: int = 0, splits: int = 0, kgroups: int = 0, stages: int = 0) -> None:
     _l.load().aldm_igemm_force(bm, bn, splits, kgroups)
     _l.load().aldm_igemm_force_stages(stages)
+
+
+def igemm_epilogue_forms(on: int = -1) -> int:
+    return _l.load().aldm_igemm_epilogue_forms(on)
 
 
 def attention_mma(mode: int) -> int:
diff --git a/include/aldm_hip.h b/include/aldm_hip.h
--- a/include/aldm_hip.h
+++ b/include/aldm_hip.h
@@ -91,6 +91,9 @@
 int aldm_igemm_plan(const aldm_igemm_desc* d, int* bm, int* bn, int64_t* flops, int* splits, int* kgroups,
                     int* mma);
 int aldm_igemm_plan_stages(const aldm_igemm_desc* d);
+enum { ALDM_EPI_FORM_GENERIC = 0, ALDM_EPI_FORM_PLAIN = 1, ALDM_EPI_FORM_ROWBIAS = 2, ALDM_EPI_FORM_RES = 3 };
+int aldm_igemm_plan_epilogue(const aldm_igemm_desc* d);
+int aldm_igemm_epilogue_forms(int on);
 void aldm_igemm_force(int bm, int bn, int splits, int kgroups);
 void aldm_igemm_force_stages(int stages);
 int aldm_igemm_wave8_mask(int mask);
```

Result: faster. 18.88 audio-s/s (median of 6 runs) (+1.3%).
